# iebeid/ProtGram-DirectGCN

Hardware: AMD Instinct MI355X
Metric: edges/sec propagated, DirectGCN fwd on 4-gram graph, 1/2/4/8 MI355X (higher is better)
Workload: dtype f32; 1 GPU; directgcn_fwd_B(20,4); graph=complete n-gram de Bruijn B(20,4), num_nodes=160000, transitions=3200000, nnz_per_adjacency=6559580, feat_dim=128, layers=2, classes=20, propagation=precomputed-weights, entry=trainer COO (edge_index_*/edge_weight_* -> csr_from_coo), parallelism=single

## Files before the change

### include/pg_directgcn.h

```cpp
#ifndef PG_DIRECTGCN_H
#define PG_DIRECTGCN_H

#include <stdint.h>

#ifdef __cplusplus
extern "C" {
#endif

#define PG_ABI_VERSION 4

#define PG_OK 0
#define PG_ERR_ARG (-1)
#define PG_ERR_HIP (-2)
#define PG_ERR_UNSUPPORTED (-3)

typedef struct pg_edge3 {
    int32_t col;
    float w_in;
    float w_out;
    float w_und;
} pg_edge3_t;

typedef struct pg_edgeraw {
    int32_t col;
    float a_fwd;
    float a_bwd;
    float m_und;
} pg_edgeraw_t;

typedef struct pg_edge1 {
    int32_t col;
    float w;
} pg_edge1_t;


#define PG_FLAG_NO_XCD_REMAP (1u << 0)
#define PG_FLAG_EDGE_LDS (1u << 1)
#define PG_FLAG_UNROLL4 (1u << 2)
#define PG_FLAG_BCAST_RECORDS (1u << 7)
#define PG_FLAG_NGRAMT_WIDE (1u << 8)
#define PG_FLAG_NGRAMT_HALVES (1u << 4)
#define PG_FLAG_NGRAMT_NARROW (1u << 3)
#define PG_FLAG_DENSE_PREGATED (1u << 14)
#define PG_FLAG_DENSE_TILED (1u << 15)
#define PG_FLAG_DENSE_X3 (1u << 16)
#define PG_FLAG_WGRAD_BF16_TILED (1u << 11)
#define PG_FLAG_DGRAD_BF16_TILED (1u << 10)
#define PG_FLAG_DGRAD_BF16_RESIDENT (1u << 9)
#define PG_FLAG_WGRAD_F32MFMA (1u << 18)
#define PG_FLAG_DGRAD_F32MFMA (1u << 17)
#define PG_FLAG_NO_NGRAM (1u << 20)
#define PG_FLAG_NGRAM_BLOCK4 (1u << 21)
#define PG_FLAG_MID_NO_PAIRS (1u << 22)
#define PG_FLAG_MID_LOADER_SYNC (1u << 19)
#define PG_FLAG_DENSE_NO_IL (1u << 13)
#define PG_FLAG_DENSE_A_CACHED (1u << 12)
#define PG_FLAG_DENSE_LDS_EPILOGUE (1u << 29)
#define PG_FLAG_SCATTER_CPW_SHIFT 24
#define PG_FLAG_MID_TRANSPOSED (1u << 23)


const char* pg_last_error(void);
int pg_abi_version(void);

int pg_spmm3_f32(int64_t n_rows, const int64_t* rowptr, const int32_t* row_order, const pg_edge3_t* edges,
                 const float* X, int64_t ldx, int64_t F,
                 float* Z, int64_t ldz, uint32_t flags, void* stream);


int pg_spmm3_fusednorm_f32(int64_t n_rows, const int64_t* rowptr, const int32_t* row_order,
                           const pg_edgeraw_t* edges,
                           const float* node_norm, float eps,
                           const float* X, int64_t ldx, int64_t F,
                           float* Z, int64_t ldz, uint32_t flags, void* stream);

int pg_edges_normalize_f32(int64_t n_rows, const int64_t* rowptr, const pg_edgeraw_t* raw,
                           const float* node_norm, float eps, pg_edge3_t* out, void* stream);

int pg_spmm3t_f32(int64_t n_rows, const int64_t* rowptr, const int32_t* row_order, const pg_edge3_t* edges,
                  const float* G, int64_t ldg, int64_t F,
                  float* dX, int64_t lddx, int accumulate, uint32_t flags, void* stream);

int pg_spmm1_f32(int64_t n_rows, const int64_t* rowptr, const int32_t* row_order, const pg_edge1_t* edges,
                 const float* X, int64_t ldx, int64_t F,
                 float* Y, int64_t ldy, int accumulate, uint32_t flags, void* stream);

#define PG_GATES_VECTOR 0
#define PG_GATES_SCALAR 1

typedef struct pg_layer_args {
    int64_t M, F_in, F_out;
    const float* Z; int64_t ldz;
    const float* W_main_in; const float* W_main_out; const float* W_undirected; const float* W_shared;
    const float* b_main_in; const float* b_dir_shared_in;
    const float* b_main_out; const float* b_dir_shared_out;
    const float* b_undirected; const float* b_undirected_shared;
    int32_t gate_mode;
    const float* C_in; const float* C_out; const float* C_directed; const float* C_undirected; const float* C_all;
    const int64_t* rows;
    const float* constant; int64_t ld_const;
    const float* res_x; int64_t ld_res;
    const float* W_res; const float* b_res;
    int32_t act; float slope;
    float* Y; int64_t ldy;
    float drop_p; const int64_t* drop_seed;
} pg_layer_args_t;

int64_t pg_directgcn_packed_floats(int64_t F_in, int64_t F_out, int has_res_proj);

int pg_directgcn_pack_f32(const pg_layer_args_t* args, float* packed, void* stream);

int pg_directgcn_dense_f32(const pg_layer_args_t* args, const float* packed, uint32_t flags, void* stream);

int pg_directgcn_dense_ngram_rows_f32(const pg_layer_args_t* args, const float* packed, int64_t Kn1, int64_t m0,
                                      int32_t map_res, int32_t map_y, uint32_t flags, void* stream);

int pg_spmm3_gated_f32(int64_t n_rows, const int64_t* rowptr, const int32_t* row_order, const pg_edge3_t* edges,
                       const float* X, int64_t ldx, int64_t F, const pg_layer_args_t* gates,
                       float* Z, int64_t ldz, uint32_t flags, void* stream);

int64_t pg_ngram_plan_floats(int K, int n, int64_t n_rows);
int pg_ngram_plan_f32(int K, int n, int64_t n_rows, const int64_t* rowptr, const pg_edge3_t* edges, float* plan,
                      int64_t plan_floats, int* bad, void* stream);
int pg_spmm3_ngram_f32(int K, int n, int64_t n_rows, const float* plan, const float* X, int64_t ldx, int64_t F,
                       const pg_layer_args_t* gates, float* Z, int64_t ldz, uint32_t flags, void* stream);
int pg_spmm3t_ngram_f32(int K, int n, int64_t n_rows, const float* plan, const float* G, int64_t ldg, int64_t F,
                        float* dX, int64_t lddx, int accumulate, uint32_t flags, void* stream);
int pg_spmm3t_ngram_bf16(int K, int n, int64_t n_rows, const float* plan, const uint16_t* G, int64_t ldg, int64_t F,
                         uint16_t* dX, int64_t lddx, int accumulate, uint32_t flags, void* stream);
int pg_spmm3t_ngram_add_bf16(int K, int n, int64_t n_rows, const float* plan, const uint16_t* G, int64_t ldg,
                             int64_t F, const uint16_t* C, int64_t ldc, uint16_t* dX, int64_t lddx, uint32_t flags,
                             void* stream);

int64_t pg_ngram_mplan_floats(int K, int n, int64_t n_rows);
int pg_ngram_mplan_f32(int K, int n, int64_t n_rows, const int64_t* rowptr, const pg_edge3_t* edges, float* plan,
                       int64_t plan_floats, int* bad, void* stream);
int pg_spmm3_ngram_mid_f32(int K, int n, int64_t n_rows, const float* plan, const float* X, int64_t ldx, int64_t F,
                           const pg_layer_args_t* gates, float* Z, int64_t ldz, uint32_t flags, void* stream);
int pg_spmm3_ngram_mid_rows_f32(int K, int n, int64_t n_rows, const float* plan, const float* X, int64_t ldx, int64_t F,
                                int64_t m_begin, int64_t m_end, float* Z, int64_t ldz, uint32_t flags, void* stream);
int pg_spmm3_ngram_mid_bf16(int K, int n, int64_t n_rows, const float* plan, const uint16_t* X, int64_t ldx, int64_t F,
                            uint16_t* Z, int64_t ldz, uint32_t flags, void* stream);
int pg_spmm3_ngram_mid_rows_bf16(int K, int n, int64_t n_rows, const float* plan, const uint16_t* X, int64_t ldx,
                                 int64_t F, int64_t m_begin, int64_t m_end, uint16_t* Z, int64_t ldz, uint32_t flags,
                                 void* stream);
int pg_ngram_mplan_map_f32(int K, int n, int64_t n_nodes, const int64_t* rowptr, const pg_edge3_t* edges,
                           const int32_t* ginv, float* plan, int64_t plan_floats, uint8_t* resid, void* stream);
int pg_spmm3_ngram_mid_map_f32(int K, int n, const float* plan, const int32_t* gmap, const float* X, int64_t ldx,
                               int64_t F, float* Z, int64_t ldz, uint32_t flags, void* stream);
int pg_spmm3_resid_f32(int64_t n_list, const int64_t* rowptr, const int32_t* rows, const pg_edge3_t* edges,
                       const float* X, int64_t ldx, int64_t F, float* Z, int64_t ldz, uint32_t flags, void* stream);
int pg_spmm3t_ngram_mid_offdiag_f32(int K, int n, int64_t n_rows, const float* plan, const float* G, int64_t ldg,
                                    int64_t F, float* dX, int64_t lddx, int accumulate, uint32_t flags, void* stream);
int pg_spmm3t_ngram_mid_bf16(int K, int n, int64_t n_rows, const float* plan, const uint16_t* G, int64_t ldg, int64_t F,
                             uint16_t* dX, int64_t lddx, int accumulate, uint32_t flags, void* stream);

int pg_ngram_scatter_plan(int K, int n, const float* mplan, int64_t m0, int64_t n_mid, float* splan, void* stream);
int pg_spmm3t_ngram_scatter_f32(const float* splan, int64_t n_mid, const float* G, int64_t ldg, int64_t F, float* T,
                                int64_t ldt, uint32_t flags, void* stream);
int pg_spmm3t_ngram_scatter_bf16(const float* splan, int64_t n_mid, const uint16_t* G, int64_t ldg, int64_t F,
                                 float* T, int64_t ldt, uint32_t flags, void* stream);

int pg_rows_gather(const void* src, int64_t ld_src, const int64_t* idx, int64_t n, int64_t row_bytes, void* dst,
                   int64_t ld_dst, void* stream);
int pg_rows_scatter(const void* src, int64_t ld_src, const int64_t* idx, int64_t n, int64_t row_bytes, void* dst,
                    int64_t ld_dst, void* stream);
int pg_rows_gather_sum(const float* A, int64_t lda, const void* B, int64_t ldb, int b_bf16, const int64_t* rowptr,
                       const int32_t* idx, int64_t n_out, int64_t F, void* out, int64_t ldo, int out_bf16,
                       void* stream);

typedef struct pg_layer_grad_args {
    const float* dY; int64_t lddy;
    float* dpre; int64_t ldp;
    float* dZ; int64_t lddz;
    float* dres; int64_t lddres;
    float* dgate;
    float* gates;
    float* dW;
    float* work; int64_t work_floats;
    float* dpre_f32; int64_t ldp_f32;
} pg_layer_grad_args_t;

int64_t pg_directgcn_dense_bwd_workspace(const pg_layer_args_t* args);
int pg_directgcn_dense_bwd_f32(const pg_layer_args_t* args, const float* packed, const pg_layer_grad_args_t* grads,
                               uint32_t flags, void* stream);

int pg_directgcn_dense_bwd_span_f32(const pg_layer_args_t* args, const float* packed, const pg_layer_grad_args_t* grads,
                                    const float* wdiag, float* E, int64_t lde, int e_res, uint32_t flags, void* stream);


int pg_f32_to_bf16(int64_t n, const float* in, uint16_t* out, void* stream);

int pg_spmm3_bf16(int64_t n_rows, const int64_t* rowptr, const int32_t* row_order, const pg_edge3_t* edges,
                  const uint16_t* X, int64_t ldx, int64_t F, uint16_t* Z, int64_t ldz, uint32_t flags, void* stream);

int pg_spmm3t_bf16(int64_t n_rows, const int64_t* rowptr, const int32_t* row_order, const pg_edge3_t* edges,
                   const uint16_t* G, int64_t ldg, int64_t F, uint16_t* dX, int64_t lddx, uint32_t flags,
                   void* stream);

int pg_directgcn_dense_bf16(const pg_layer_args_t* args, const float* packed, const uint16_t* packed_bf16,
                            uint32_t flags, void* stream);

int pg_directgcn_dense_bwd_bf16(const pg_layer_args_t* args, const float* packed, const uint16_t* packed_bf16,
                                const pg_layer_grad_args_t* grads, uint32_t flags, void* stream);

int pg_directgcn_head_bf16(int64_t M, int64_t F, int64_t H, int64_t C, const uint16_t* h, int64_t ldh,
                           const float* W1, const float* b1, const float* W2, const float* b2, float eps,
                           float* logp, int64_t ldp, float* emb, int64_t lde, void* stream);

int pg_ngram_keys(int64_t nseq, const int64_t* offsets, const uint8_t* bytes, const int32_t* lut, int n,
                  int64_t K, int64_t* keys, int64_t* next_keys, void* stream);

int pg_ngram_letter_masks(int64_t n_nodes, const int64_t* node_keys, int n, int64_t K, const int32_t* code_bit,
                          uint32_t* masks, void* stream);

int pg_reach_hop_u32(int64_t n_rows, const int64_t* rowptr, const int64_t* col, const uint32_t* reach_in,
                     uint32_t* reach_out, int hop, int n_bits, uint8_t* dist, int64_t ldd, const uint8_t* target,
                     int64_t* labels, void* stream);

int pg_ngram_window_ids(int64_t nseq, const int64_t* offsets, const uint8_t* bytes, const int32_t* lut, int n,
                        int64_t K, const int64_t* node_keys, int64_t N, const int32_t* table, int32_t* ids,
                        void* stream);

int64_t pg_pool_distinct_max_nodes(void);
int pg_pool_rows_f32(const float* E, int64_t lde, int64_t N, int64_t F, const int64_t* rowptr, const int32_t* ids,
                     const int64_t* order, int64_t P, int distinct, float* out, int64_t ldo, int32_t* counts,
                     uint32_t flags, void* stream);

int64_t pg_pca_moments_workspace(int64_t P, int64_t F);
int pg_pca_moments_f64(const float* X, int64_t ldx, int64_t P, int64_t F, const int32_t* counts, const float* shift,
                       double* out, double* work, int64_t work_doubles, void* stream);

int pg_pca_project(const float* X, int64_t ldx, int64_t P, int64_t F, const int32_t* counts, const float* center,
                   const float* W, int64_t k, void* out, int64_t ldo, int out_dtype, void* stream);

typedef struct pg_tensor_desc {
    const float* x;
    float* y;
    int64_t numel;
} pg_tensor_desc_t;

int64_t pg_multi_chunks(int64_t numel);

int pg_multi_sqsum_f32(int ntens, const pg_tensor_desc_t* descs, const int64_t* chunk_ptr, int64_t nchunks,
                       float* partial, float* out, void* stream);

int pg_multi_axpy_f32(int ntens, const pg_tensor_desc_t* descs, const int64_t* chunk_ptr, int64_t nchunks,
                      float alpha, const float* alpha_scale, void* stream);

typedef struct pg_adam_desc {
    float* p;
    const void* g;
    float* m;
    float* v;
    int64_t numel;
    int64_t gtype;
} pg_adam_desc_t;

int pg_adam_f32(int ntens, const pg_adam_desc_t* descs, const int64_t* chunk_ptr, int64_t nchunks, double lr,
                double beta1, double beta2, double eps, double weight_decay, float* step, const float* grad_scale,
                const float* found_inf, float* sq_partial, const double* hyper, void* stream);

typedef struct pg_adam_rows_desc {
    float* p;
    const void* g;
    float* m;
    float* v;
    int64_t numel;
    int64_t gtype;
    const int32_t* pos;
    int64_t width;
} pg_adam_rows_desc_t;

int pg_adam_rows_f32(int ntens, const pg_adam_rows_desc_t* descs, const int64_t* chunk_ptr, int64_t nchunks, double lr,
                     double beta1, double beta2, double eps, double weight_decay, float* step, const float* grad_scale,
                     const float* found_inf, float* sq_partial, const double* hyper, void* stream);
int pg_multi_sum_f32(int64_t n, const float* x, float* out, void* stream);

int64_t pg_head_train_workspace(int64_t M, int64_t F, int64_t H, int64_t C);
int pg_head_train_f32(int64_t M, int64_t F, int64_t H, int64_t C, const float* h, int64_t ldh, const float* W1,
                      const float* b1, const float* W2, const float* b2, const int64_t* y, float loss_weight,
                      float drop_p, const int64_t* seed, const float* grad_scale, float* dh, int64_t lddh,
                      float* grads, float* loss, float* work, int64_t work_floats, void* stream);

int64_t pg_head_train_bf16_workspace(int64_t M, int64_t F, int64_t H, int64_t C);
int pg_head_train_bf16(int64_t M, int64_t F, int64_t H, int64_t C, const uint16_t* h, int64_t ldh, const float* W1,
                       const float* b1, const float* W2, const float* b2, const int64_t* y, float loss_weight,
                       float drop_p, const int64_t* seed, const float* grad_scale, uint16_t* dh, int64_t lddh,
                       float* grads, float* loss, float* work, int64_t work_floats, void* stream);

int64_t pg_gemm_at_b_workspace(int64_t M, int64_t P, int64_t N);
int pg_gemm_at_b_f32(int64_t M, int64_t P, int64_t N, const float* A, int64_t lda, const float* B, int64_t ldb,
                     float* out, float* work, int64_t work_floats, void* stream);

int pg_dense_grads_layout_f32(int64_t F_out, int64_t F_in, int32_t S, const float* dB, const float* dbsum, float* out,
                              void* stream);

int pg_directgcn_head_f32(int64_t M, int64_t F, int64_t H, int64_t C, const float* h, int64_t ldh,
                          const float* W1, const float* b1, const float* W2, const float* b2, float eps,
                          float* logp, int64_t ldp, float* emb, int64_t lde, void* stream);

#ifdef __cplusplus
}
#endif

#endif
```

### protgram-directgcn_amd/_lib.py

```python
from __future__ import annotations

import ctypes
import os

_HERE = os.path.dirname(os.path.abspath(__file__))
_LIB_PATH = os.environ.get("PG_DIRECTGCN_LIB", os.path.join(_HERE, "libpgdgcn.so"))

PG_OK = 0
PG_FLAG_NO_XCD_REMAP = 1 << 0
PG_FLAG_EDGE_LDS = 1 << 1
PG_FLAG_UNROLL4 = 1 << 2
PG_FLAG_BCAST_RECORDS = 1 << 7
PG_FLAG_NGRAMT_WIDE = 1 << 8
PG_FLAG_NGRAMT_NARROW = 1 << 3
PG_FLAG_NGRAMT_HALVES = 1 << 4
PG_FLAG_DENSE_PREGATED = 1 << 14
PG_FLAG_DENSE_TILED = 1 << 15
PG_FLAG_DENSE_X3 = 1 << 16
PG_FLAG_WGRAD_F32MFMA = 1 << 18
PG_FLAG_WGRAD_BF16_TILED = 1 << 11
PG_FLAG_DGRAD_BF16_TILED = 1 << 10
PG_FLAG_DGRAD_BF16_RESIDENT = 1 << 9
PG_FLAG_DGRAD_F32MFMA = 1 << 17
PG_FLAG_NO_NGRAM = 1 << 20
PG_FLAG_NGRAM_BLOCK4 = 1 << 21
PG_FLAG_MID_NO_PAIRS = 1 << 22
PG_FLAG_MID_LOADER_SYNC = 1 << 19
PG_FLAG_MID_TRANSPOSED = 1 << 23
PG_FLAG_SCATTER_CPW_SHIFT = 24
PG_FLAG_DENSE_A_CACHED = 1 << 12
PG_FLAG_DENSE_NO_IL = 1 << 13
PG_FLAG_DENSE_LDS_EPILOGUE = 1 << 29

c_i64, c_i32, c_u32, c_f32, c_vp = ctypes.c_int64, ctypes.c_int32, ctypes.c_uint32, ctypes.c_float, ctypes.c_void_p


PG_OK, PG_ERR_ARG, PG_ERR_HIP, PG_ERR_UNSUPPORTED = 0, -1, -2, -3


class NativeLibraryError(RuntimeError):
    pass


class LayerArgs(ctypes.Structure):
    _fields_ = [("M", c_i64), ("F_in", c_i64), ("F_out", c_i64),
                ("Z", c_vp), ("ldz", c_i64),
                ("W_main_in", c_vp), ("W_main_out", c_vp), ("W_undirected", c_vp), ("W_shared", c_vp),
                ("b_main_in", c_vp), ("b_dir_shared_in", c_vp),
                ("b_main_out", c_vp), ("b_dir_shared_out", c_vp),
                ("b_undirected", c_vp), ("b_undirected_shared", c_vp),
                ("gate_mode", c_i32),
                ("C_in", c_vp), ("C_out", c_vp), ("C_directed", c_vp), ("C_undirected", c_vp), ("C_all", c_vp),
                ("rows", c_vp),
                ("constant", c_vp), ("ld_const", c_i64),
                ("res_x", c_vp), ("ld_res", c_i64),
                ("W_res", c_vp), ("b_res", c_vp),
                ("act", c_i32), ("slope", c_f32),
                ("Y", c_vp), ("ldy", c_i64),
                ("drop_p", c_f32), ("drop_seed", c_vp)]


class LayerGradArgs(ctypes.Structure):
    _fields_ = [("dY", c_vp), ("lddy", c_i64), ("dpre", c_vp), ("ldp", c_i64), ("dZ", c_vp), ("lddz", c_i64),
                ("dres", c_vp), ("lddres", c_i64), ("dgate", c_vp), ("gates", c_vp), ("dW", c_vp),
                ("work", c_vp), ("work_floats", c_i64), ("dpre_f32", c_vp), ("ldp_f32", c_i64)]


SIGNATURES = {
    "pg_last_error": (ctypes.c_char_p, []),
    "pg_abi_version": (ctypes.c_int, []),
    "pg_spmm3_f32": (ctypes.c_int, [c_i64, c_vp, c_vp, c_vp, c_vp, c_i64, c_i64, c_vp, c_i64, c_u32, c_vp]),
    "pg_spmm3_gated_f32": (ctypes.c_int, [c_i64, c_vp, c_vp, c_vp, c_vp, c_i64, c_i64, ctypes.POINTER(LayerArgs), c_vp,
                                          c_i64, c_u32, c_vp]),
    "pg_spmm3_fusednorm_f32": (ctypes.c_int, [c_i64, c_vp, c_vp, c_vp, c_vp, c_f32, c_vp, c_i64, c_i64, c_vp, c_i64,
                                              c_u32, c_vp]),
    "pg_edges_normalize_f32": (ctypes.c_int, [c_i64, c_vp, c_vp, c_vp, c_f32, c_vp, c_vp]),
    "pg_ngram_plan_floats": (c_i64, [ctypes.c_int, ctypes.c_int, c_i64]),
    "pg_ngram_plan_f32": (ctypes.c_int, [ctypes.c_int, ctypes.c_int, c_i64, c_vp, c_vp, c_vp, c_i64, c_vp, c_vp]),
    "pg_spmm3_ngram_f32": (ctypes.c_int, [ctypes.c_int, ctypes.c_int, c_i64, c_vp, c_vp, c_i64, c_i64,
                                          ctypes.POINTER(LayerArgs), c_vp, c_i64, c_u32, c_vp]),
    "pg_ngram_mplan_floats": (c_i64, [ctypes.c_int, ctypes.c_int, c_i64]),
    "pg_ngram_mplan_f32": (ctypes.c_int, [ctypes.c_int, ctypes.c_int, c_i64, c_vp, c_vp, c_vp, c_i64, c_vp, c_vp]),
    "pg_spmm3_ngram_mid_f32": (ctypes.c_int, [ctypes.c_int, ctypes.c_int, c_i64, c_vp, c_vp, c_i64, c_i64,
                                              ctypes.POINTER(LayerArgs), c_vp, c_i64, c_u32, c_vp]),
    "pg_spmm3_ngram_mid_rows_f32": (ctypes.c_int, [ctypes.c_int, ctypes.c_int, c_i64, c_vp, c_vp, c_i64, c_i64, c_i64,
                                                   c_i64, c_vp, c_i64, c_u32, c_vp]),
    "pg_spmm3_ngram_mid_bf16": (ctypes.c_int, [ctypes.c_int, ctypes.c_int, c_i64, c_vp, c_vp, c_i64, c_i64, c_vp,
                                               c_i64, c_u32, c_vp]),
    "pg_spmm3_ngram_mid_rows_bf16": (ctypes.c_int, [ctypes.c_int, ctypes.c_int, c_i64, c_vp, c_vp, c_i64, c_i64, c_i64,
                                                    c_i64, c_vp, c_i64, c_u32, c_vp]),
    "pg_ngram_mplan_map_f32": (ctypes.c_int, [ctypes.c_int, ctypes.c_int, c_i64, c_vp, c_vp, c_vp, c_vp, c_i64, c_vp,
                                              c_vp]),
    "pg_spmm3_ngram_mid_map_f32": (ctypes.c_int, [ctypes.c_int, ctypes.c_int, c_vp, c_vp, c_vp, c_i64, c_i64, c_vp,
                                                  c_i64, c_u32, c_vp]),
    "pg_spmm3_resid_f32": (ctypes.c_int, [c_i64, c_vp, c_vp, c_vp, c_vp, c_i64, c_i64, c_vp, c_i64, c_u32, c_vp]),
    "pg_rows_gather": (ctypes.c_int, [c_vp, c_i64, c_vp, c_i64, c_i64, c_vp, c_i64, c_vp]),
    "pg_rows_scatter": (ctypes.c_int, [c_vp, c_i64, c_vp, c_i64, c_i64, c_vp, c_i64, c_vp]),
    "pg_rows_gather_sum": (ctypes.c_int, [c_vp, c_i64, c_vp, c_i64, ctypes.c_int, c_vp, c_vp, c_i64, c_i64, c_vp,
                                          c_i64, ctypes.c_int, c_vp]),
    "pg_ngram_scatter_plan": (ctypes.c_int, [ctypes.c_int, ctypes.c_int, c_vp, c_i64, c_i64, c_vp, c_vp]),
    "pg_spmm3t_ngram_scatter_f32": (ctypes.c_int, [c_vp, c_i64, c_vp, c_i64, c_i64, c_vp, c_i64, c_u32, c_vp]),
    "pg_spmm3t_ngram_scatter_bf16": (ctypes.c_int, [c_vp, c_i64, c_vp, c_i64, c_i64, c_vp, c_i64, c_u32, c_vp]),
    "pg_spmm3t_ngram_f32": (ctypes.c_int, [ctypes.c_int, ctypes.c_int, c_i64, c_vp, c_vp, c_i64, c_i64, c_vp, c_i64,
                                           ctypes.c_int, c_u32, c_vp]),
    "pg_spmm3t_ngram_mid_offdiag_f32": (ctypes.c_int, [ctypes.c_int, ctypes.c_int, c_i64, c_vp, c_vp, c_i64, c_i64,
                                                       c_vp, c_i64, ctypes.c_int, c_u32, c_vp]),
    "pg_spmm3t_ngram_mid_bf16": (ctypes.c_int, [ctypes.c_int, ctypes.c_int, c_i64, c_vp, c_vp, c_i64, c_i64, c_vp, c_i64,
                                                ctypes.c_int, c_u32, c_vp]),
    "pg_spmm3t_ngram_bf16": (ctypes.c_int, [ctypes.c_int, ctypes.c_int, c_i64, c_vp, c_vp, c_i64, c_i64, c_vp, c_i64,
                                            ctypes.c_int, c_u32, c_vp]),
    "pg_spmm3t_ngram_add_bf16": (ctypes.c_int, [ctypes.c_int, ctypes.c_int, c_i64, c_vp, c_vp, c_i64, c_i64, c_vp,
                                                c_i64, c_vp, c_i64, c_u32, c_vp]),
    "pg_spmm3t_f32": (ctypes.c_int, [c_i64, c_vp, c_vp, c_vp, c_vp, c_i64, c_i64, c_vp, c_i64, ctypes.c_int, c_u32,
                                     c_vp]),
    "pg_spmm1_f32": (ctypes.c_int, [c_i64, c_vp, c_vp, c_vp, c_vp, c_i64, c_i64, c_vp, c_i64, ctypes.c_int, c_u32,
                                    c_vp]),
    "pg_directgcn_packed_floats": (c_i64, [c_i64, c_i64, ctypes.c_int]),
    "pg_directgcn_pack_f32": (ctypes.c_int, [ctypes.POINTER(LayerArgs), c_vp, c_vp]),
    "pg_directgcn_dense_f32": (ctypes.c_int, [ctypes.POINTER(LayerArgs), c_vp, c_u32, c_vp]),
    "pg_directgcn_dense_ngram_rows_f32": (ctypes.c_int, [ctypes.POINTER(LayerArgs), c_vp, c_i64, c_i64, c_i32, c_i32,
                                                         c_u32, c_vp]),
    "pg_directgcn_dense_bwd_workspace": (c_i64, [ctypes.POINTER(LayerArgs)]),
    "pg_directgcn_dense_bwd_f32": (ctypes.c_int, [ctypes.POINTER(LayerArgs), c_vp, ctypes.POINTER(LayerGradArgs),
                                                  c_u32, c_vp]),
    "pg_directgcn_dense_bwd_span_f32": (ctypes.c_int, [ctypes.POINTER(LayerArgs), c_vp, ctypes.POINTER(LayerGradArgs),
                                                       c_vp, c_vp, c_i64, c_i32, c_u32, c_vp]),
    "pg_f32_to_bf16": (ctypes.c_int, [c_i64, c_vp, c_vp, c_vp]),
    "pg_spmm3_bf16": (ctypes.c_int, [c_i64, c_vp, c_vp, c_vp, c_vp, c_i64, c_i64, c_vp, c_i64, c_u32, c_vp]),
    "pg_spmm3t_bf16": (ctypes.c_int, [c_i64, c_vp, c_vp, c_vp, c_vp, c_i64, c_i64, c_vp, c_i64, c_u32, c_vp]),
    "pg_directgcn_dense_bf16": (ctypes.c_int, [ctypes.POINTER(LayerArgs), c_vp, c_vp, c_u32, c_vp]),
    "pg_directgcn_dense_bwd_bf16": (ctypes.c_int, [ctypes.POINTER(LayerArgs), c_vp, c_vp, ctypes.POINTER(LayerGradArgs),
                                                   c_u32, c_vp]),
    "pg_directgcn_head_bf16": (ctypes.c_int, [c_i64, c_i64, c_i64, c_i64, c_vp, c_i64, c_vp, c_vp, c_vp, c_vp, c_f32,
                                              c_vp, c_i64, c_vp, c_i64, c_vp]),
    "pg_ngram_keys": (ctypes.c_int, [c_i64, c_vp, c_vp, c_vp, ctypes.c_int, c_i64, c_vp, c_vp, c_vp]),
    "pg_ngram_window_ids": (ctypes.c_int, [c_i64, c_vp, c_vp, c_vp, ctypes.c_int, c_i64, c_vp, c_i64, c_vp, c_vp, c_vp]),
    "pg_ngram_letter_masks": (ctypes.c_int, [c_i64, c_vp, ctypes.c_int, c_i64, c_vp, c_vp, c_vp]),
    "pg_reach_hop_u32": (ctypes.c_int, [c_i64, c_vp, c_vp, c_vp, c_vp, ctypes.c_int, ctypes.c_int, c_vp, c_i64, c_vp,
                                        c_vp, c_vp]),
    "pg_pool_distinct_max_nodes": (c_i64, []),
    "pg_pool_rows_f32": (ctypes.c_int, [c_vp, c_i64, c_i64, c_i64, c_vp, c_vp, c_vp, c_i64, ctypes.c_int, c_vp, c_i64,
                                        c_vp, c_u32, c_vp]),
    "pg_pca_moments_workspace": (c_i64, [c_i64, c_i64]),
    "pg_pca_moments_f64": (ctypes.c_int, [c_vp, c_i64, c_i64, c_i64, c_vp, c_vp, c_vp, c_vp, c_i64, c_vp]),
    "pg_pca_project": (ctypes.c_int, [c_vp, c_i64, c_i64, c_i64, c_vp, c_vp, c_vp, c_i64, c_vp, c_i64, ctypes.c_int,
                                      c_vp]),
    "pg_multi_chunks": (c_i64, [c_i64]),
    "pg_multi_sqsum_f32": (ctypes.c_int, [ctypes.c_int, c_vp, c_vp, c_i64, c_vp, c_vp, c_vp]),
    "pg_multi_axpy_f32": (ctypes.c_int, [ctypes.c_int, c_vp, c_vp, c_i64, c_f32, c_vp, c_vp]),
    "pg_adam_f32": (ctypes.c_int, [ctypes.c_int, c_vp, c_vp, c_i64, ctypes.c_double, ctypes.c_double, ctypes.c_double,
                                   ctypes.c_double, ctypes.c_double, c_vp, c_vp, c_vp, c_vp, c_vp, c_vp]),
    "pg_adam_rows_f32": (ctypes.c_int, [ctypes.c_int, c_vp, c_vp, c_i64, ctypes.c_double, ctypes.c_double,
                                        ctypes.c_double, ctypes.c_double, ctypes.c_double, c_vp, c_vp, c_vp, c_vp, c_vp,
                                        c_vp]),
    "pg_multi_sum_f32": (ctypes.c_int, [c_i64, c_vp, c_vp, c_vp]),
    "pg_dense_grads_layout_f32": (ctypes.c_int, [c_i64, c_i64, ctypes.c_int32, c_vp, c_vp, c_vp, c_vp]),
    "pg_gemm_at_b_workspace": (c_i64, [c_i64, c_i64, c_i64]),
    "pg_gemm_at_b_f32": (ctypes.c_int, [c_i64, c_i64, c_i64, c_vp, c_i64, c_vp, c_i64, c_vp, c_vp, c_i64, c_vp]),
    "pg_directgcn_head_f32": (ctypes.c_int, [c_i64, c_i64, c_i64, c_i64, c_vp, c_i64, c_vp, c_vp, c_vp, c_vp, c_f32,
                                             c_vp, c_i64, c_vp, c_i64, c_vp]),
    "pg_head_train_workspace": (c_i64, [c_i64, c_i64, c_i64, c_i64]),
    "pg_head_train_f32": (ctypes.c_int, [c_i64, c_i64, c_i64, c_i64, c_vp, c_i64, c_vp, c_vp, c_vp, c_vp, c_vp, c_f32,
                                         c_f32, c_vp, c_vp, c_vp, c_i64, c_vp, c_vp, c_vp, c_i64, c_vp]),
    "pg_head_train_bf16_workspace": (c_i64, [c_i64, c_i64, c_i64, c_i64]),
    "pg_head_train_bf16": (ctypes.c_int, [c_i64, c_i64, c_i64, c_i64, c_vp, c_i64, c_vp, c_vp, c_vp, c_vp, c_vp, c_f32,
                                          c_f32, c_vp, c_vp, c_vp, c_i64, c_vp, c_vp, c_vp, c_i64, c_vp]),
}

_lib = None


def library_path() -> str:
    return _LIB_PATH


def load_library():
    global _lib
    if _lib is not None:
        return _lib
    if not os.path.exists(_LIB_PATH):
        raise NativeLibraryError(
            f"HIP library not found at {_LIB_PATH}; build it with `python -c 'import __graft_entry__ as g; g.build()'`"
            " (there is no CPU fallback)")
    try:
        lib = ctypes.CDLL(_LIB_PATH)
    except OSError as e:
        raise NativeLibraryError(f"failed to load {_LIB_PATH}: {e}") from e
    for name, (res, args) in SIGNATURES.items():
        fn = getattr(lib, name, None)
        if fn is None:
            raise NativeLibraryError(f"{_LIB_PATH} does not export {name}")
        fn.restype, fn.argtypes = res, args
    if lib.pg_abi_version() != 4:
        raise NativeLibraryError("ABI version mismatch")
    _lib = lib
    return lib


def check(rc: int, what: str):
    if rc != PG_OK:
        msg = load_library().pg_last_error().decode(errors="replace")
        raise RuntimeError(f"{what} failed ({rc}): {msg}")


def default_flags() -> int:
    v = os.environ.get("PG_SPMM_FLAGS")
    return int(v, 0) if v else 0
```

### protgram-directgcn_amd/csrc/pg_common.h

```cpp
#pragma once

#include <hip/hip_runtime.h>

#include <cstdarg>
#include <cstdint>
#include <cstdio>

#include "pg_directgcn.h"

namespace pg {

int set_error(int code, const char* fmt, ...);
void clear_error();

__device__ __forceinline__ float4 ld4(const float* p) { return *reinterpret_cast<const float4*>(p); }
__device__ __forceinline__ float fb(int v) { return __int_as_float(v); }

__device__ __forceinline__ int64_t xcd_logical_block(int64_t b, int64_t nb, bool remap) {
    if (!remap || nb < 16) return b;
    const int64_t q = nb >> 3, r = nb & 7;
    const int64_t x = b & 7, i = b >> 3;
    return x * q + (x < r ? x : r) + i;
}

__device__ __forceinline__ float sqrt_rn(float x) {
    if (!(x > 0.0f) || x == __builtin_inff()) return __builtin_sqrtf(x);
    const bool tiny = x < 0x1p-96f;
    const float xs = tiny ? x * 0x1p64f : x;
    float y = __builtin_sqrtf(xs);
    const int yi = __float_as_int(y);
    const float ym = __int_as_float(yi - 1), yp = __int_as_float(yi + 1);
    const float vm = __builtin_fmaf(-ym, y, xs), vp = __builtin_fmaf(-yp, y, xs);
    y = vm <= 0.0f ? ym : y;
    y = vp > 0.0f ? yp : y;
    return tiny ? y * 0x1p-32f : y;
}

__device__ __forceinline__ uint32_t drop_hash(uint64_t seed, uint32_t e) {
    uint32_t x = (e * 0x9E3779B1u + (uint32_t)seed) ^ (uint32_t)(seed >> 32);
    x ^= x >> 16;
    x *= 0x85EBCA6Bu;
    x ^= x >> 13;
    x *= 0xC2B2AE35u;
    x ^= x >> 16;
    return x;
}

__device__ __forceinline__ float act_grad(float d, float y, float slope, float ds) {
    if (ds == 0.f) return y > 0.f ? d : d * slope;
    const float e = d * ds;
    return y > 0.f ? e : (y < 0.f ? e * slope : 0.f);
}

inline int drop_params(const pg_layer_args_t* a, uint32_t& thr, float& scale, bool need_seed = true) {
    thr = 0;
    scale = 0.f;
    if (a->drop_p == 0.f) return PG_OK;
    if (!(a->drop_p > 0.f && a->drop_p < 1.f) || !a->act || (need_seed && !a->drop_seed))
        return set_error(PG_ERR_ARG, "fused dropout needs 0 <= drop_p < 1, act and drop_seed (drop_p = %g)",
                         (double)a->drop_p);
    thr = (uint32_t)((double)a->drop_p * 16777216.0 + 0.5);
    scale = (float)(1.0 / (1.0 - (double)a->drop_p));
    return PG_OK;
}

inline int check_launch(const char* what) {
    hipError_t e = hipGetLastError();
    if (e != hipSuccess) return set_error(PG_ERR_HIP, "%s: %s", what, hipGetErrorString(e));
    return PG_OK;
}

inline int cu_count() {
    int dev = 0, ncu = 256;
    if (hipGetDevice(&dev) != hipSuccess ||
        hipDeviceGetAttribute(&ncu, hipDeviceAttributeMultiprocessorCount, dev) != hipSuccess || ncu <= 0)
        ncu = 256;
    return ncu;
}

inline bool aligned16(const void* p) { return (reinterpret_cast<uintptr_t>(p) & 15u) == 0; }

}

#define PG_REQUIRE(cond, ...)                                         \
    do {                                                              \
        if (!(cond)) return ::pg::set_error(PG_ERR_ARG, __VA_ARGS__); \
    } while (0)
```

### protgram-directgcn_amd/csrc/pg_dense.hip

```cpp
#include "pg_common.h"
#include "pg_lds.h"
#include "pg_split3.h"

namespace {

typedef float f32x16 __attribute__((ext_vector_type(16)));
typedef float f32x4 __attribute__((ext_vector_type(4)));

constexpr int BK = 32;
constexpr int LDSW = 36;

struct DenseP {
    int64_t M;
    int F_in, F_out, K;
    const float* Z;
    int64_t ldz;
    const float* Bp;
    const float* bsum;
    int gate_mode;
    const float *C_in, *C_out, *C_dir, *C_und, *C_all;
    const int64_t* rows;
    const float* constant;
    int64_t ld_const;
    const float* res_x;
    int64_t ld_res;
    int proj_res;
    int vec_out;
    int act;
    float slope;
    float* Y;
    int64_t ldy;
    int remap;
    int pregated;
    int rawW;
    const float *Wq0, *Wq1, *Wq2, *Wsh;
    const float *bm0, *bs0, *bm1, *bs1, *bm2, *bs2;
    int64_t map_kn1, map_m0;
    int map_res, map_y;
    int nt_a;
    int exp;
    uint32_t drop_thr;
    float drop_s;
    const int64_t* drop_seed;
};

__device__ __forceinline__ float drop_apply(const DenseP& p, uint64_t seed, int64_t m, int j, float y) {
    const uint32_t e = (uint32_t)(m * p.F_out + j);
    return (pg::drop_hash(seed, e) >> 8) >= p.drop_thr ? y * p.drop_s : 0.f;
}
__device__ __forceinline__ uint64_t drop_seed_of(const DenseP& p) {
    return p.drop_s != 0.f ? (uint64_t)*p.drop_seed : 0ull;
}

#ifdef PG_DENSE_EXP
#define DEXP(bit) ((p.exp >> (bit)) & 1)
constexpr int DST_BLOCKS = 64, DST_IT = 48, DST_PT = 8;
__device__ unsigned long long* g_dense_stamps = nullptr;
#define DSTAMP_INIT unsigned long long* const dst_base_ = g_dense_stamps
#define DSTAMP(it, pt)                                                                                             \
    do {                                                                                                           \
        if (dst_base_ && lane == 0 && (wave == 0 || wave == 4) && blockIdx.x < DST_BLOCKS && (it) < DST_IT)        \
            dst_base_[((blockIdx.x * 2 + (wave >> 2)) * DST_IT + (it)) * DST_PT + (pt)] =                          \
                __builtin_amdgcn_s_memtime();                                                                      \
    } while (0)
#else
#define DEXP(bit) 0
#define DSTAMP_INIT \
    do {            \
    } while (0)
#define DSTAMP(it, pt) \
    do {               \
    } while (0)
#endif

__device__ __forceinline__ int64_t ngram_row(const DenseP& p, int64_t m) {
    const int r = (int)m;
    const int q = r / 400, w = r - 400 * q;
    const int a = w / 20, b = w - 20 * a;
    return (int64_t)a * p.map_kn1 + (p.map_m0 + q) * 20 + b;
}

using pg::ld4;
__device__ __forceinline__ float4 scale4(float4 a, float s) { return make_float4(a.x * s, a.y * s, a.z * s, a.w * s); }

__device__ __forceinline__ int seg_of(int k, int F) { return (k >= F) + (k >= 2 * F) + (k >= 3 * F); }

__device__ __forceinline__ float a_elem(const DenseP& p, const float* sg, int64_t m, int k) {
    const int q = seg_of(k, p.F_in);
    if (q < 3) return p.pregated ? p.Z[m * p.ldz + k] : p.Z[m * p.ldz + k] * sg[q];
    return p.res_x[m * p.ld_res + (k - 3 * p.F_in)];
}

template <int BM, int BN, int NW, bool VEC>
__global__ __launch_bounds__(64 * NW) void dense_kernel(DenseP p) {
    constexpr int NT = 64 * NW;
    const uint64_t dseed = drop_seed_of(p);
    constexpr int WN = (BM == 64 && NW == 8) ? 4 : (BN == 128 || BM == 64 || NW == 8) ? 2 : 1;
    constexpr int WM = NW / WN;
    static_assert(BM / WM >= 32 && BN / WN >= 32, "wave tile too small");
    constexpr int TM = BM / WM / 32;
    constexpr int TN = BN / WN / 32;
    constexpr int A_F4 = BM * BK / 4 / NT;
    constexpr int B_F4 = BN * BK / 4 / NT;

    constexpr int TLD = BN + 4;
    constexpr int MAIN_FLOATS = 2 * BM * LDSW + 2 * BN * LDSW;
    constexpr int SMEM_FLOATS = MAIN_FLOATS > BM * TLD ? MAIN_FLOATS : BM * TLD;
    __shared__ __attribute__((aligned(16))) float smem[SMEM_FLOATS];
    __shared__ __attribute__((aligned(16))) float Sg[BM * 4];
    __shared__ int64_t Crow[BM];
    static_assert(BM <= NT, "gate prologue assumes one thread per tile row");
    float (*As)[BM * LDSW] = reinterpret_cast<float (*)[BM * LDSW]>(smem);
    float (*Bs)[BN * LDSW] = reinterpret_cast<float (*)[BN * LDSW]>(smem + 2 * BM * LDSW);

    const int64_t n_mblk = (p.M + BM - 1) / BM;
    const int64_t lb = pg::xcd_logical_block(blockIdx.x, gridDim.x, p.remap != 0);
    const int64_t m0 = (lb % n_mblk) * BM;
    const int n0 = (int)(lb / n_mblk) * BN;
    const int tid = threadIdx.x;
    const int wave = tid >> 6, lane = tid & 63;
    const int wm = wave / WN, wn = wave % WN;
    const int li = lane & 31, lh = lane >> 5;

    if (tid < BM) {
        const int64_t m = m0 + tid;
        float s0 = 0.f, s1 = 0.f, s2 = 0.f;
        if (m < p.M) {
            const int64_t r = (p.gate_mode == PG_GATES_SCALAR) ? 0 : (p.rows ? p.rows[m] : m);
            const float ci = p.C_in[r], co = p.C_out[r], cd = p.C_dir[r], cu = p.C_und[r], ca = p.C_all[r];
            const float cad = ca * cd;
            s0 = cad * ci;
            s1 = cad * co;
            s2 = ca * cu;
        }
        Sg[tid * 4 + 0] = s0;
        Sg[tid * 4 + 1] = s1;
        Sg[tid * 4 + 2] = s2;
        Sg[tid * 4 + 3] = 1.f;
        Crow[tid] = m < p.M ? (p.rows ? p.rows[m] : m) : -1;
    }
    __syncthreads();

    f32x16 acc[TM][TN];
#pragma unroll
    for (int i = 0; i < TM; ++i)
#pragma unroll
        for (int j = 0; j < TN; ++j)
#pragma unroll
            for (int r = 0; r < 16; ++r) acc[i][j][r] = 0.f;

    float4 ra[A_F4], rb[B_F4];
    const int64_t mlast = p.M - 1;
    auto fetch_to = [&](int k0, float4 (&ra)[A_F4], float4 (&rb)[B_F4]) {
#pragma unroll
        for (int q = 0; q < A_F4; ++q) {
            const int idx = tid + NT * q;
            const int64_t m = min(m0 + (idx >> 3), mlast);
            const int k = k0 + 4 * (idx & 7);
            if (VEC) {
                const int kc = k < p.K ? k : 0;
                const int seg = seg_of(kc, p.F_in);
                const float* src = seg < 3 ? p.Z + m * p.ldz + kc : p.res_x + m * p.ld_res + (kc - 3 * p.F_in);
                ra[q] = ld4(src);
            } else {
                const float* sg = &Sg[(idx >> 3) * 4];
                float4 v = make_float4(0.f, 0.f, 0.f, 0.f);
                if (k + 0 < p.K) v.x = a_elem(p, sg, m, k + 0);
                if (k + 1 < p.K) v.y = a_elem(p, sg, m, k + 1);
                if (k + 2 < p.K) v.z = a_elem(p, sg, m, k + 2);
                if (k + 3 < p.K) v.w = a_elem(p, sg, m, k + 3);
                ra[q] = v;
            }
        }
#pragma unroll
        for (int q = 0; q < B_F4; ++q) {
            const int idx = tid + NT * q;
            const int n = min(n0 + (idx >> 3), p.F_out - 1);
            const int k = k0 + 4 * (idx & 7);
            const float* src = p.Bp + (int64_t)n * p.K;
            if (VEC) {
                rb[q] = ld4(src + (k < p.K ? k : 0));
            } else {
                float4 v = make_float4(0.f, 0.f, 0.f, 0.f);
                if (k + 0 < p.K) v.x = src[k + 0];
                if (k + 1 < p.K) v.y = src[k + 1];
                if (k + 2 < p.K) v.z = src[k + 2];
                if (k + 3 < p.K) v.w = src[k + 3];
                rb[q] = v;
            }
        }
    };
    auto fetch = [&](int k0) { fetch_to(k0, ra, rb); };
    auto stash_from = [&](int buf, int k0, const float4 (&ra)[A_F4], const float4 (&rb)[B_F4]) {
#pragma unroll
        for (int q = 0; q < A_F4; ++q) {
            const int idx = tid + NT * q;
            float4 v = ra[q];
            if (VEC) {
                const int k = k0 + 4 * (idx & 7);
                const int seg = seg_of(k, p.F_in);
                const float sc = k < p.K ? (p.pregated ? 1.f : Sg[(idx >> 3) * 4 + seg]) : 0.f;
                v = scale4(v, sc);
            }
            *reinterpret_cast<float4*>(&As[buf][(idx >> 3) * LDSW + 4 * (idx & 7)]) = v;
        }
#pragma unroll
        for (int q = 0; q < B_F4; ++q) {
            const int idx = tid + NT * q;
            float4 v = rb[q];
            if (VEC) {
                const int k = k0 + 4 * (idx & 7);
                if (k >= p.K) v = make_float4(0.f, 0.f, 0.f, 0.f);
            }
            *reinterpret_cast<float4*>(&Bs[buf][(idx >> 3) * LDSW + 4 * (idx & 7)]) = v;
        }
    };

    auto stash = [&](int buf, int k0) { stash_from(buf, k0, ra, rb); };
    auto mma = [&](int cur) {
        const float* Ab = As[cur];
        const float* Bb = Bs[cur];
#pragma unroll
        for (int g = 0; g < BK / 8; ++g) {
            float4 a[TM], b[TN];
#pragma unroll
            for (int i = 0; i < TM; ++i) a[i] = ld4(&Ab[(wm * TM * 32 + i * 32 + li) * LDSW + g * 8 + 4 * lh]);
#pragma unroll
            for (int j = 0; j < TN; ++j) b[j] = ld4(&Bb[(wn * TN * 32 + j * 32 + li) * LDSW + g * 8 + 4 * lh]);
#pragma unroll
            for (int i = 0; i < TM; ++i)
#pragma unroll
                for (int j = 0; j < TN; ++j) {
                    acc[i][j] = __builtin_amdgcn_mfma_f32_32x32x2f32(a[i].x, b[j].x, acc[i][j], 0, 0, 0);
                    acc[i][j] = __builtin_amdgcn_mfma_f32_32x32x2f32(a[i].y, b[j].y, acc[i][j], 0, 0, 0);
                    acc[i][j] = __builtin_amdgcn_mfma_f32_32x32x2f32(a[i].z, b[j].z, acc[i][j], 0, 0, 0);
                    acc[i][j] = __builtin_amdgcn_mfma_f32_32x32x2f32(a[i].w, b[j].w, acc[i][j], 0, 0, 0);
                }
        }
    };

    const int ntiles = (p.K + BK - 1) / BK;
    fetch(0);
    stash(0, 0);
    __syncthreads();
    for (int t = 0; t < ntiles; ++t) {
        const int cur = t & 1;
        if (t + 1 < ntiles) fetch((t + 1) * BK);
        mma(cur);
        if (t + 1 < ntiles) stash(cur ^ 1, (t + 1) * BK);
        __syncthreads();
    }

    float* T = smem;
#pragma unroll
    for (int i = 0; i < TM; ++i)
#pragma unroll
        for (int j = 0; j < TN; ++j)
#pragma unroll
            for (int r = 0; r < 16; ++r) {
                const int rl = wm * TM * 32 + i * 32 + (r & 3) + 8 * (r >> 2) + 4 * lh;
                T[rl * TLD + wn * TN * 32 + j * 32 + li] = acc[i][j][r];
            }
    __syncthreads();

    constexpr int C4 = BN / 4;
    constexpr int ITER = BM * C4 / NT;
    constexpr int BATCH = ITER < 4 ? ITER : 4;
    const int c4 = tid % C4;
    const int nb = n0 + 4 * c4;
    const bool has_const = p.constant && p.gate_mode == PG_GATES_VECTOR;
    const bool id_res = p.res_x && !p.proj_res;
    const bool vec_out = p.vec_out;
    float4 b[3], br = make_float4(0.f, 0.f, 0.f, 0.f);
    {
        auto ldb = [&](const float* v) {
            float4 o;
            o.x = nb + 0 < p.F_out ? v[nb + 0] : 0.f;
            o.y = nb + 1 < p.F_out ? v[nb + 1] : 0.f;
            o.z = nb + 2 < p.F_out ? v[nb + 2] : 0.f;
            o.w = nb + 3 < p.F_out ? v[nb + 3] : 0.f;
            return o;
        };
        b[0] = ldb(p.bsum);
        b[1] = ldb(p.bsum + p.F_out);
        b[2] = ldb(p.bsum + 2 * p.F_out);
        if (p.proj_res) br = ldb(p.bsum + 3 * p.F_out);
    }
    for (int it0 = 0; it0 < ITER; it0 += BATCH) {
        float4 cv[BATCH], rv[BATCH];
        int rl[BATCH];
        int64_t mm[BATCH];
        bool ok[BATCH];
#pragma unroll
        for (int u = 0; u < BATCH; ++u) {
            rl[u] = (tid + NT * (it0 + u)) / C4;
            mm[u] = m0 + rl[u];
            ok[u] = Crow[rl[u]] >= 0 && nb < p.F_out;
            cv[u] = make_float4(0.f, 0.f, 0.f, 0.f);
            rv[u] = make_float4(0.f, 0.f, 0.f, 0.f);
            if (ok[u] && vec_out) {
                if (has_const) cv[u] = ld4(p.constant + Crow[rl[u]] * p.ld_const + nb);
                if (id_res) rv[u] = ld4(p.res_x + mm[u] * p.ld_res + nb);
            }
        }
#pragma unroll
        for (int u = 0; u < BATCH; ++u) {
            if (!ok[u]) continue;
            const float* sg = &Sg[rl[u] * 4];
            float4 v = ld4(&T[rl[u] * TLD + 4 * c4]);
            float o[4] = {v.x, v.y, v.z, v.w};
            const float bb0[4] = {b[0].x, b[0].y, b[0].z, b[0].w};
            const float bb1[4] = {b[1].x, b[1].y, b[1].z, b[1].w};
            const float bb2[4] = {b[2].x, b[2].y, b[2].z, b[2].w};
            const float bbr[4] = {br.x, br.y, br.z, br.w};
            float cc[4] = {cv[u].x, cv[u].y, cv[u].z, cv[u].w};
            float rr[4] = {rv[u].x, rv[u].y, rv[u].z, rv[u].w};
            if (!vec_out) {
#pragma unroll
                for (int e = 0; e < 4; ++e) {
                    const int n = nb + e;
                    if (n < p.F_out) {
                        if (has_const) cc[e] = p.constant[Crow[rl[u]] * p.ld_const + n];
                        if (id_res) rr[e] = p.res_x[mm[u] * p.ld_res + n];
                    }
                }
            }
#pragma unroll
            for (int e = 0; e < 4; ++e) {
                float y = o[e] + (sg[0] * bb0[e] + sg[1] * bb1[e] + sg[2] * bb2[e]) + bbr[e] + cc[e] + rr[e];
                if (p.act) y = y > 0.f ? y : y * p.slope;
                if (p.drop_s != 0.f) y = drop_apply(p, dseed, mm[u], nb + e, y);
                o[e] = y;
            }
            if (vec_out) {
                *reinterpret_cast<float4*>(p.Y + mm[u] * p.ldy + nb) = make_float4(o[0], o[1], o[2], o[3]);
            } else {
#pragma unroll
                for (int e = 0; e < 4; ++e)
                    if (nb + e < p.F_out) p.Y[mm[u] * p.ldy + nb + e] = o[e];
            }
        }
    }
}

using pg::glds16;
using pg::glds16nt;
// ... 28 lines not shown
__device__ __forceinline__ void lds_st16(void* p, uint4 v) {
    const u32x4_t w = {v.x, v.y, v.z, v.w};
    asm volatile("ds_write_b128 %0, %1" ::"v"(lds_addr(p)), "v"(w) : "memory");
}
__device__ __forceinline__ void lds_ld4x4(const float* p0, const float* p1, const float* p2, const float* p3,
                                          float4 (&o)[4]) {
    f32x4 x0, x1, x2, x3;
    asm volatile(
        "ds_read_b128 %0, %4\n\tds_read_b128 %1, %5\n\tds_read_b128 %2, %6\n\tds_read_b128 %3, %7\n\t"
        "s_waitcnt lgkmcnt(0)"
        : "=&v"(x0), "=&v"(x1), "=&v"(x2), "=&v"(x3)
        : "v"(lds_addr(p0)), "v"(lds_addr(p1)), "v"(lds_addr(p2)), "v"(lds_addr(p3))
        : "memory");
    o[0] = make_float4(x0[0], x0[1], x0[2], x0[3]);
    o[1] = make_float4(x1[0], x1[1], x1[2], x1[3]);
    o[2] = make_float4(x2[0], x2[1], x2[2], x2[3]);
    o[3] = make_float4(x3[0], x3[1], x3[2], x3[3]);
}
template <int STRIDE_BYTES>
__device__ __forceinline__ void lds_epi(const float* p0, const float* p1, const float* p2, const float* g, float4& a,
                                        float4& b, float4& c, float (&gv)[5]) {
    f32x4 x0, x1, x2;
    asm volatile(
        "ds_read_b128 %0, %8\n\tds_read_b128 %1, %9\n\tds_read_b128 %2, %10\n\t"
        "ds_read_b32 %3, %11\n\tds_read_b32 %4, %11 offset:%c12\n\tds_read_b32 %5, %11 offset:%c13\n\t"
        "ds_read_b32 %6, %11 offset:%c14\n\tds_read_b32 %7, %11 offset:%c15\n\ts_waitcnt lgkmcnt(0)"
        : "=&v"(x0), "=&v"(x1), "=&v"(x2), "=&v"(gv[0]), "=&v"(gv[1]), "=&v"(gv[2]), "=&v"(gv[3]), "=&v"(gv[4])
        : "v"(lds_addr(p0)), "v"(lds_addr(p1)), "v"(lds_addr(p2)), "v"(lds_addr(g)), "n"(STRIDE_BYTES),
          "n"(2 * STRIDE_BYTES), "n"(3 * STRIDE_BYTES), "n"(4 * STRIDE_BYTES)
        : "memory");
    a = make_float4(x0[0], x0[1], x0[2], x0[3]);
    b = make_float4(x1[0], x1[1], x1[2], x1[3]);
    c = make_float4(x2[0], x2[1], x2[2], x2[3]);
}
template <int STRIDE_BYTES>
__device__ __forceinline__ void lds_gates5(const float* p, float (&g)[5]) {
    asm volatile(
        "ds_read_b32 %0, %5\n\tds_read_b32 %1, %5 offset:%c6\n\tds_read_b32 %2, %5 offset:%c7\n\t"
        "ds_read_b32 %3, %5 offset:%c8\n\tds_read_b32 %4, %5 offset:%c9\n\ts_waitcnt lgkmcnt(0)"
        : "=&v"(g[0]), "=&v"(g[1]), "=&v"(g[2]), "=&v"(g[3]), "=&v"(g[4])
        : "v"(lds_addr(p)), "n"(STRIDE_BYTES), "n"(2 * STRIDE_BYTES), "n"(3 * STRIDE_BYTES), "n"(4 * STRIDE_BYTES)
        : "memory");
}

__device__ __forceinline__ int a_unit(int s, int r, int g) { return 128 * s + 4 * r + (g ^ ((-(r >> 2)) & 3)); }

struct TileRange { int64_t ntl, lo, step; };
__device__ __forceinline__ TileRange tile_range(int64_t T) {
    const int nb = gridDim.x, b = blockIdx.x;
    TileRange t;
    if ((nb & 7) == 0 && nb >= 8) {
        const int x = b & 7, i = b >> 3, bpx = nb >> 3;
        const int64_t xlo = T * x / 8, xhi = T * (x + 1) / 8;
        t.ntl = (xhi - xlo - i + bpx - 1) / bpx;
        t.lo = xlo + i;
        t.step = bpx;
    } else {
        t.ntl = (T - b + nb - 1) / nb;
        t.lo = b;
        t.step = nb;
    }
    if (t.ntl < 0) t.ntl = 0;
    return t;
}

template <int NS>
__device__ __forceinline__ void w_splits(const float* src, uint4 (&w0)[NS], uint4 (&w1)[NS], uint4 (&w2)[NS]) {
#pragma unroll
    for (int s = 0; s < NS; ++s) {
        const float4 x0 = ld4(src + 32 * s), x1 = ld4(src + 32 * s + 16);
        const float v[8] = {x0.x, x0.y, x0.z, x0.w, x1.x, x1.y, x1.z, x1.w};
        split8(v, w0[s], w1[s], w2[s]);
    }
}

__device__ __forceinline__ void gate_scales(const float (&c)[5], float& s0, float& s1, float& s2) {
    const float cad = c[4] * c[2];
    s0 = cad * c[0];
    s1 = cad * c[1];
    s2 = c[4] * c[3];
}

__device__ __forceinline__ void gate_ptrs(const DenseP& p, const float* (&c)[5]) {
    c[0] = p.C_in, c[1] = p.C_out, c[2] = p.C_dir, c[3] = p.C_und, c[4] = p.C_all;
    asm volatile("" : "+s"(c[0]), "+s"(c[1]), "+s"(c[2]), "+s"(c[3]), "+s"(c[4]));
}

template <bool MAP, int BM>
__device__ __forceinline__ void cr_rows(const DenseP& p, bool has_const, bool id_res, int64_t tile, int r,
                                        const float*& cb, const float*& rb) {
    const int64_t m0 = tile * BM;
    const int rmax = (int)min((int64_t)(BM - 1), p.M - 1 - m0);
    const int rr = min(r, rmax);
    cb = has_const ? p.constant + m0 * p.ld_const + (rr * (int)p.ld_const) : p.Z + m0 * p.ldz;
    rb = !id_res            ? p.Z + m0 * p.ldz
         : MAP && p.map_res ? p.res_x + ngram_row(p, m0 + rr) * p.ld_res
                            : p.res_x + m0 * p.ld_res + (rr * (int)p.ld_res);
}

template <int F_IN, int KSEG, bool PRE>
__global__ __launch_bounds__(512) void dense_x3_kernel(DenseP p) {
    constexpr int K = F_IN * KSEG;
    const uint64_t dseed = drop_seed_of(p);
    constexpr int CH = K / 4;
    constexpr int NU = K / 8;
    constexpr int NS = K / 32;
    constexpr int BMW = 32;
    constexpr int NI = BMW * CH / 64 / 8;
    constexpr int NG = 3;
    constexpr int NCR = 4;
    (void)NCR;
    constexpr int NCV = (BMW * NU + 511) / 512;
    static_assert(CH % 16 == 0 && NU % 16 == 0 && (BMW * CH) % 512 == 0 && BMW * 128 / 4 == 1024, "tile shape");
    __shared__ __attribute__((aligned(16))) float Af[BMW * K];
    __shared__ __attribute__((aligned(16))) uint4 As[3][BMW * NU];
    __shared__ __attribute__((aligned(16))) float Cs[BMW * 128];
    __shared__ __attribute__((aligned(16))) float Rs[BMW * 128];
    __shared__ __attribute__((aligned(16))) float Gi[2][8][BMW];
    __shared__ __attribute__((aligned(16))) float Bs[4][128];
    constexpr int ELD = 128 + 4;
    static_assert(BMW * ELD * 4 <= 3 * BMW * NU * 16, "epilogue tile must fit in the split images");
    float* Es = reinterpret_cast<float*>(&As[0][0]);

    const int tid = threadIdx.x;
    const int wave = tid >> 6, lane = tid & 63;
    const int lc = lane & 15, kg = lane >> 4;
    const int col = 16 * wave + lc;
    const int64_t T = (p.M + BMW - 1) / BMW;
    Bs[tid >> 7][tid & 127] = (tid >> 7) < 3 || p.proj_res ? p.bsum[(tid >> 7) * p.F_out + (tid & 127)] : 0.f;
    const TileRange tr = tile_range(T);
    const int64_t ntl = tr.ntl, lo = tr.lo, step = tr.step;
    uint4 w0[NS], w1[NS], w2[NS];
    w_splits<NS>(p.Bp + (int64_t)col * K + 4 * kg, w0, w1, w2);
    const int ej = tid & 31, er = tid >> 5;
    const bool has_const = p.constant && p.gate_mode == PG_GATES_VECTOR;
    const bool id_res = p.res_x && !p.proj_res;

    auto issue_A = [&](int64_t tile, float* Ad) {
        const int64_t m0 = tile * BMW;
        const int rmax = (int)min((int64_t)(BMW - 1), p.M - 1 - m0);
        const float* zb = p.Z + m0 * p.ldz;
        const float* xb = KSEG > 3 ? p.res_x + m0 * p.ld_res : zb;
        const int ln = opaque(lane);
#pragma unroll
        for (int i = 0; i < NI; ++i) {
            const int idx = (wave * NI + i) * 64 + ln;
            const int r = idx / CH, pos = idx - r * CH;
            const int k = 4 * (pos ^ (r & 15));
            const int rr = min(r, rmax);
            const float* src = (KSEG == 3 || k < 3 * F_IN) ? zb + (rr * (int)p.ldz + k)
                                                          : xb + (rr * (int)p.ld_res + (k - 3 * F_IN));
            glds16(src, Ad + (wave * NI + i) * 256);
        }
    };
    auto issue_G = [&](int64_t tile, int gbuf) {
        const int ln = opaque(lane);
        const int64_t r = p.gate_mode == PG_GATES_SCALAR ? 0 : min(tile * BMW + (ln & 31), p.M - 1);
        const float* c[5];
        gate_ptrs(p, c);
        const bool hi = ln >= 32;
        glds4((hi ? c[1] : c[0]) + r, &Gi[gbuf][0][0]);
        glds4((hi ? c[3] : c[2]) + r, &Gi[gbuf][2][0]);
        glds4(c[4] + r, &Gi[gbuf][4][0]);
    };
    auto issue_CR = [&](int64_t tile) {
        const int ln = opaque(lane);
#pragma unroll
        for (int i = 0; i < 2; ++i) {
            const int piece = 2 * wave + i;
            const float *cb, *rb;
            cr_rows<false, BMW>(p, has_const, id_res, tile, 2 * piece + (ln >> 5), cb, rb);
            glds16(cb + 4 * (ln & 31), Cs + piece * 256);
            glds16(rb + 4 * (ln & 31), Rs + piece * 256);
        }
    };
    auto gates = [&](int gbuf, int r, float& s0, float& s1, float& s2) {
        float c[5];
        lds_gates5<BMW * 4>(&Gi[gbuf][0][r], c);
        gate_scales(c, s0, s1, s2);
    };
    auto tile_of = [&](int64_t kt) { return lo + min(kt, ntl - 1) * step; };

    auto convert = [&](const float* Af, int gb) {
#pragma unroll
        for (int i = 0; i < NCV; ++i) {
            const int j = tid + 512 * i;
            if (BMW * NU % 512 != 0 && j >= BMW * NU) break;
            const int r = j & (BMW - 1), u = j / BMW;
            const int s = u >> 2, g = u & 3;
            const int c0 = 8 * s + g;
            float4 x0, x1;
            lds_ld4x2(&Af[r * K + 4 * (c0 ^ (r & 15))], &Af[r * K + 4 * ((c0 + 4) ^ (r & 15))], x0, x1);
            float v[8] = {x0.x, x0.y, x0.z, x0.w, x1.x, x1.y, x1.z, x1.w};
            if (!PRE) {
                const int q = (32 * s) / F_IN;
                if (q < 3) {
                    float sg[3];
                    gates(gb, r, sg[0], sg[1], sg[2]);
                    const float sc = sg[q];
#pragma unroll
                    for (int e = 0; e < 8; ++e) v[e] = __fmul_rn(v[e], sc);
                }
            }
            uint4 s0, s1, s2;
            split8(v, s0, s1, s2);
            const int pos = a_unit(s, r, g);
            lds_st16(&As[0][pos], s0);
            lds_st16(&As[1][pos], s1);
            lds_st16(&As[2][pos], s2);
            __builtin_amdgcn_sched_barrier(0);
        }
    };
    constexpr int WAIT_W0 = NG + NI, WAIT_WN = NI;
    if (ntl > 0) {
        if (wave == 0) issue_G(tile_of(0), 0);
        issue_A(tile_of(0), Af);
    }
    bool prev_full = false;
    for (int64_t kt = 0; kt < ntl; ++kt) {
        const int buf = (int)(kt & 1);
        const int64_t m0 = (lo + kt * step) * BMW;
        if (prev_full) asm volatile("s_waitcnt vmcnt(2)" ::: "memory");
        else asm volatile("s_waitcnt vmcnt(0)" ::: "memory");
        lds_barrier();
        issue_CR(tile_of(kt));
        if (wave == 0) issue_G(tile_of(kt + 1), buf ^ 1);
        convert(Af, buf);
        lds_barrier();
        issue_A(tile_of(kt + 1), Af);
        f32x4 acc[2] = {f32x4{0.f, 0.f, 0.f, 0.f}, f32x4{0.f, 0.f, 0.f, 0.f}};
        const uint4* ab0 = &As[0][a_unit(0, lc, kg)];
        const uint4* ab2 = &As[2][a_unit(0, lc, kg)];
        uint4 op[2][6];
        auto ld_ops = [&](int s, uint4 (&o)[6]) {
            o[0] = ab0[128 * s];
            o[1] = ab0[BMW * NU + 128 * s];
            o[2] = ab2[128 * s];
            o[3] = ab0[64 + 128 * s];
            o[4] = ab0[BMW * NU + 64 + 128 * s];
            o[5] = ab2[64 + 128 * s];
        };
        ld_ops(0, op[0]);
#pragma unroll
        for (int s = 0; s < NS; ++s) {
            if (s + 1 < NS) ld_ops(s + 1, op[(s + 1) & 1]);
            const uint4 a00 = op[s & 1][0], a01 = op[s & 1][1], a02 = op[s & 1][2];
            const uint4 a10 = op[s & 1][3], a11 = op[s & 1][4], a12 = op[s & 1][5];
            acc[0] = mfma_bf(a02, w0[s], acc[0]);
            acc[1] = mfma_bf(a12, w0[s], acc[1]);
            acc[0] = mfma_bf(a01, w1[s], acc[0]);
            acc[1] = mfma_bf(a11, w1[s], acc[1]);
            acc[0] = mfma_bf(a00, w2[s], acc[0]);
            acc[1] = mfma_bf(a10, w2[s], acc[1]);
            acc[0] = mfma_bf(a01, w0[s], acc[0]);
            acc[1] = mfma_bf(a11, w0[s], acc[1]);
            acc[0] = mfma_bf(a00, w1[s], acc[0]);
            acc[1] = mfma_bf(a10, w1[s], acc[1]);
            acc[0] = mfma_bf(a00, w0[s], acc[0]);
            acc[1] = mfma_bf(a10, w0[s], acc[1]);
            __builtin_amdgcn_sched_barrier(0);
        }
        lds_barrier();
#pragma unroll
        for (int sb = 0; sb < 2; ++sb)
#pragma unroll
            for (int i = 0; i < 4; ++i) lds_stf(&Es[(16 * sb + 4 * kg + i) * ELD + col], acc[sb][i]);
        if (wave == 0) asm volatile("s_waitcnt vmcnt(%0)" ::"n"(WAIT_W0) : "memory");
        else asm volatile("s_waitcnt vmcnt(%0)" ::"n"(WAIT_WN) : "memory");
        lds_barrier();
#pragma unroll
        for (int h = 0; h < 2; ++h) {
            const int rl = er + 16 * h;
            if (m0 + rl >= p.M) continue;
            float4 v, cv, rv, bb[4];
            lds_ld4x2(&Cs[rl * 128 + 4 * ej], &Rs[rl * 128 + 4 * ej], cv, rv);
            lds_ld4x4(&Es[rl * ELD + 4 * ej], &Bs[0][4 * ej], &Bs[1][4 * ej], &Bs[2][4 * ej], bb);
            v = bb[0];
            const float4 b0 = bb[1], b1 = bb[2], b2 = bb[3];
            float4 br;
            lds_ld4x2(&Bs[3][4 * ej], &Bs[3][4 * ej], br, br);
            if (!has_const) cv = make_float4(0.f, 0.f, 0.f, 0.f);
            if (!id_res) rv = make_float4(0.f, 0.f, 0.f, 0.f);
            float s0, s1, s2;
            gates(buf, rl, s0, s1, s2);
            const float o[4] = {v.x, v.y, v.z, v.w}, C4[4] = {cv.x, cv.y, cv.z, cv.w}, R4[4] = {rv.x, rv.y, rv.z, rv.w};
            const float B0[4] = {b0.x, b0.y, b0.z, b0.w}, B1[4] = {b1.x, b1.y, b1.z, b1.w},
                        B2[4] = {b2.x, b2.y, b2.z, b2.w}, BR[4] = {br.x, br.y, br.z, br.w};
            float y[4];
#pragma unroll
            for (int e = 0; e < 4; ++e) {
                const float qv = epi_sum(o[e], s0, s1, s2, B0[e], B1[e], B2[e], BR[e], C4[e], R4[e]);
                y[e] = (p.act && !(qv > 0.f)) ? qv * p.slope : qv;
                if (p.drop_s != 0.f) y[e] = drop_apply(p, dseed, m0 + rl, 4 * ej + e, y[e]);
            }
            *reinterpret_cast<float4*>(p.Y + (m0 + rl) * p.ldy + 4 * ej) = make_float4(y[0], y[1], y[2], y[3]);
        }
        prev_full = m0 + BMW <= p.M;
    }
    asm volatile("s_waitcnt vmcnt(0)" ::: "memory");
}

__device__ __forceinline__ int a_unit16(int s, int r, int g) { return 64 * s + 4 * r + (g ^ ((-(r >> 2)) & 3)); }

template <bool PRE, bool IL, bool DROP, bool LDSE>
__global__ __launch_bounds__(512) void dense_x3p_kernel(DenseP p) {
    constexpr int F_IN = 128, K = 384;
    constexpr int CH = K / 4;
    constexpr int NU = K / 8;
    constexpr int NS = K / 32;
    constexpr int BM = 16;
    constexpr int NI = BM * CH / 64 / 8;
    constexpr int NG = 2;
    constexpr int NCR = 2;
    (void)NCR;
    [[maybe_unused]] constexpr int ELD = 128 + 4;
    static_assert(BM * CH % 512 == 0 && NI == 3, "tile shape");
    __shared__ __attribute__((aligned(16))) float Af0[BM * K];
    __shared__ __attribute__((aligned(16))) float Af1[BM * K];
    __shared__ __attribute__((aligned(16))) uint4 As[2][3][BM * NU];
    __shared__ __attribute__((aligned(16))) float Cs[LDSE ? BM * 128 : 4];
    __shared__ __attribute__((aligned(16))) float Rs[LDSE ? BM * 128 : 4];
    __shared__ __attribute__((aligned(16))) float Es[LDSE ? BM * ELD : 4];
    __shared__ __attribute__((aligned(16))) float Gi[4][8][BM];
    __shared__ __attribute__((aligned(16))) float Bs[4][128];

    const int tid = threadIdx.x;
    const int wave = tid >> 6, lane = tid & 63;
    const int lc = lane & 15, kg = lane >> 4;
    const int col = 16 * wave + lc;
    const bool mfma_first = wave < 4;
    const uint64_t dseed = DROP ? drop_seed_of(p) : 0ull;
    const int64_t T = (p.M + BM - 1) / BM;
    DSTAMP_INIT;
    {
        const int q = tid >> 7, n = tid & 127;
        float bv = 0.f;
        if (p.rawW) {
            if (q < 3) bv = q == 0 ? p.bm0[n] + p.bs0[n] : q == 1 ? p.bm1[n] + p.bs1[n] : p.bm2[n] + p.bs2[n];
        } else if (q < 3 || p.proj_res) {
            bv = p.bsum[q * p.F_out + n];
        }
        Bs[q][n] = bv;
    }
    const TileRange tr = tile_range(T);
    const int64_t ntl = tr.ntl, lo = tr.lo, step = tr.step;

    uint4 w0[NS], w1[NS], w2[NS];
    if (p.rawW) {
#pragma unroll
        for (int s = 0; s < NS; ++s) {
            const float* wq = s < 4 ? p.Wq0 : s < 8 ? p.Wq1 : p.Wq2;
            const int64_t o = (int64_t)col * F_IN + (32 * s) % F_IN + 4 * kg;
            const float4 a0 = ld4(wq + o), a1 = ld4(wq + o + 16), h0 = ld4(p.Wsh + o), h1 = ld4(p.Wsh + o + 16);
            const float v[8] = {a0.x + h0.x, a0.y + h0.y, a0.z + h0.z, a0.w + h0.w,
                                a1.x + h1.x, a1.y + h1.y, a1.z + h1.z, a1.w + h1.w};
            split8(v, w0[s], w1[s], w2[s]);
        }
    } else {
        w_splits<NS>(p.Bp + (int64_t)col * K + 4 * kg, w0, w1, w2);
    }
    const int ec = LDSE ? 4 * (tid & 31) : 16 * wave + 4 * kg, er = LDSE ? tid >> 5 : lc;
    const bool has_const = p.constant && p.gate_mode == PG_GATES_VECTOR;
    const bool id_res = p.res_x && !p.proj_res;
    auto tile_of = [&](int64_t kt) { return lo + max((int64_t)0, min(kt, ntl - 1)) * step; };

    auto issue_A_piece = [&](int64_t tile, float* Ad, int i) {
        if (DEXP(3)) return;
        const int64_t m0 = tile * BM;
        const int rmax = (int)min((int64_t)(BM - 1), p.M - 1 - m0);
        const float* zb = p.Z + m0 * p.ldz;
        const int ln = opaque(lane);
        const int idx = (wave * NI + i) * 64 + ln;
        const int r = idx / CH, pos = idx - r * CH;
        const int k = 4 * (pos ^ r);
        const int rr = min(r, rmax);
        if (p.nt_a) glds16nt(zb + (rr * (int)p.ldz + k), Ad + (wave * NI + i) * 256);
        else glds16(zb + (rr * (int)p.ldz + k), Ad + (wave * NI + i) * 256);
    };
    auto issue_A = [&](int64_t tile, float* Ad) {
#pragma unroll
        for (int i = 0; i < NI; ++i) issue_A_piece(tile, Ad, i);
    };
    auto issue_G = [&](int64_t tile, int slot) {
        const int ln = opaque(lane);
        const int64_t r = p.gate_mode == PG_GATES_SCALAR ? 0 : min(tile * BM + (ln & 15), p.M - 1);
        const float* c[5];
        gate_ptrs(p, c);
        const int q = ln >> 4;
        const float* cq = q == 0 ? c[0] : q == 1 ? c[1] : q == 2 ? c[2] : c[3];
        glds4(cq + r, &Gi[slot][0][0]);
        glds4(c[4] + r, &Gi[slot][4][0]);
    };
    [[maybe_unused]] f32x4 cv = {0.f, 0.f, 0.f, 0.f}, rv = cv;
    [[maybe_unused]] auto load_CR = [&](int64_t tile) {
        if (DEXP(4)) return;
        const float *cb, *rb;
        cr_rows<true, BM>(p, has_const, id_res, tile, er, cb, rb);
        if (p.nt_a)
            asm volatile("global_load_dwordx4 %0, %2, off nt\n\tglobal_load_dwordx4 %1, %3, off"
                         : "=&v"(cv), "=&v"(rv)
                         : "v"(cb + ec), "v"(rb + ec)
                         : "memory");
        else
            asm volatile("global_load_dwordx4 %0, %2, off\n\tglobal_load_dwordx4 %1, %3, off"
                         : "=&v"(cv), "=&v"(rv)
                         : "v"(cb + ec), "v"(rb + ec)
                         : "memory");
    };
    [[maybe_unused]] auto wait_CR = [&]() {
        if (wave == 0) asm volatile("s_waitcnt vmcnt(%2)" : "+v"(cv), "+v"(rv) : "n"(NI + NG) : "memory");
        else asm volatile("s_waitcnt vmcnt(%2)" : "+v"(cv), "+v"(rv) : "n"(NI) : "memory");
    };
    [[maybe_unused]] auto issue_CR = [&](int64_t tile) {
        if (DEXP(4)) return;
        const int ln = opaque(lane);
        const float *cb, *rb;
        cr_rows<true, BM>(p, has_const, id_res, tile, 2 * wave + (ln >> 5), cb, rb);
        if (p.nt_a) glds16nt(cb + 4 * (ln & 31), Cs + wave * 256);
        else glds16(cb + 4 * (ln & 31), Cs + wave * 256);
        glds16(rb + 4 * (ln & 31), Rs + wave * 256);
    };
    auto split_tile = [&](const float* Af, int ab, int gslot) {
        if (DEXP(1)) return;
        const int r = tid & 15;
        const bool two = tid + 512 < BM * NU;
        const int u0 = tid >> 4, u1 = u0 + 32;
        const int c00 = 8 * (u0 >> 2) + (u0 & 3), c10 = 8 * (u1 >> 2) + (u1 & 3);
        float4 x[4];
        if (two) lds_ld4x4(&Af[r * K + 4 * (c00 ^ r)], &Af[r * K + 4 * ((c00 + 4) ^ r)], &Af[r * K + 4 * (c10 ^ r)],
                           &Af[r * K + 4 * ((c10 + 4) ^ r)], x);
        else lds_ld4x2(&Af[r * K + 4 * (c00 ^ r)], &Af[r * K + 4 * ((c00 + 4) ^ r)], x[0], x[1]);
        float sg[3] = {1.f, 1.f, 1.f}, gc[5];
        if (!PRE) {
            lds_gates5<BM * 4>(&Gi[gslot][0][r], gc);
            gate_scales(gc, sg[0], sg[1], sg[2]);
        }
#pragma unroll
        for (int i = 0; i < 2; ++i) {
            if (i == 1 && !two) break;
            const int u = i ? u1 : u0;
            const int s = u >> 2, g = u & 3;
            const float4 a = x[2 * i], c = x[2 * i + 1];
            float v[8] = {a.x, a.y, a.z, a.w, c.x, c.y, c.z, c.w};
            if (!PRE) {
                const float sc = sg[(32 * s) / F_IN];
#pragma unroll
                for (int e = 0; e < 8; ++e) v[e] = __fmul_rn(v[e], sc);
            }
            uint4 s0, s1, s2;
            split8(v, s0, s1, s2);
            const int pos = a_unit16(s, r, g);
            lds_st16(&As[ab][0][pos], s0);
            lds_st16(&As[ab][1][pos], s1);
            lds_st16(&As[ab][2][pos], s2);
        }
    };
    f32x4 acc = {0.f, 0.f, 0.f, 0.f};
    auto mfma_tile = [&](int ab, int64_t a_tile, float* a_dst, int g_slot, bool issue) {
        const uint4* a0 = &As[ab][0][a_unit16(0, lc, kg)];
        const uint4* a1 = &As[ab][1][a_unit16(0, lc, kg)];
        const uint4* a2 = &As[ab][2][a_unit16(0, lc, kg)];
        uint4 op[2][3];
        acc = f32x4{0.f, 0.f, 0.f, 0.f};
        if (DEXP(0)) {
            if (IL && issue) {
                issue_A(a_tile, a_dst);
                if (wave == 0) issue_G(a_tile, g_slot);
            }
            return;
        }
        op[0][0] = a0[0];
        op[0][1] = a1[0];
        op[0][2] = a2[0];
#pragma unroll
        for (int s = 0; s < NS; ++s) {
            if (s + 1 < NS) {
                op[(s + 1) & 1][0] = a0[64 * (s + 1)];
                op[(s + 1) & 1][1] = a1[64 * (s + 1)];
                op[(s + 1) & 1][2] = a2[64 * (s + 1)];
            }
            const uint4 x0 = op[s & 1][0], x1 = op[s & 1][1], x2 = op[s & 1][2];
            if constexpr (LDSE) {
                acc = mfma_bf(x2, w0[s], acc);
                acc = mfma_bf(x1, w1[s], acc);
                acc = mfma_bf(x0, w2[s], acc);
                acc = mfma_bf(x1, w0[s], acc);
                acc = mfma_bf(x0, w1[s], acc);
                acc = mfma_bf(x0, w0[s], acc);
            } else {
                acc = mfma_bf(w0[s], x2, acc);
                acc = mfma_bf(w1[s], x1, acc);
                acc = mfma_bf(w2[s], x0, acc);
                acc = mfma_bf(w0[s], x1, acc);
                acc = mfma_bf(w1[s], x0, acc);
                acc = mfma_bf(w0[s], x0, acc);
            }
            if constexpr (IL) {
                if (issue && (s == 2 || s == 5 || s == 8)) issue_A_piece(a_tile, a_dst, s / 3);
                if (issue && s == 10 && wave == 0) issue_G(a_tile, g_slot);
            }
            __builtin_amdgcn_sched_barrier(0);
        }
    };

    if (ntl > 0) {
        issue_A(tile_of(0), Af0);
        if (wave == 0) issue_G(tile_of(0), 0);
        issue_A(tile_of(1), Af1);
        if (wave == 0) issue_G(tile_of(1), 1);
        if (wave == 0) asm volatile("s_waitcnt vmcnt(%0)" ::"n"(NI + NG) : "memory");
        else asm volatile("s_waitcnt vmcnt(%0)" ::"n"(NI) : "memory");
        lds_barrier();
        split_tile(Af0, 0, 0);
    }
    float4 bq[4];
    if (ntl > 0) lds_ld4x4(&Bs[0][ec], &Bs[1][ec], &Bs[2][ec], &Bs[3][ec], bq);
    auto epilogue = [&](int64_t m0, float4 ov, float4 cq, float4 rq, const float (&c)[5]) {
        if (!has_const) cq = make_float4(0.f, 0.f, 0.f, 0.f);
        if (!id_res) rq = make_float4(0.f, 0.f, 0.f, 0.f);
        float s0, s1, s2;
        gate_scales(c, s0, s1, s2);
        const float o[4] = {ov.x, ov.y, ov.z, ov.w}, C4[4] = {cq.x, cq.y, cq.z, cq.w}, R4[4] = {rq.x, rq.y, rq.z, rq.w};
        const float B0[4] = {bq[0].x, bq[0].y, bq[0].z, bq[0].w}, B1[4] = {bq[1].x, bq[1].y, bq[1].z, bq[1].w},
                    B2[4] = {bq[2].x, bq[2].y, bq[2].z, bq[2].w}, BR[4] = {bq[3].x, bq[3].y, bq[3].z, bq[3].w};
        float y[4];
#pragma unroll
        for (int e = 0; e < 4; ++e) {
            const float qv = epi_sum(o[e], s0, s1, s2, B0[e], B1[e], B2[e], BR[e], C4[e], R4[e]);
            y[e] = (p.act && !(qv > 0.f)) ? qv * p.slope : qv;
            if (DROP) y[e] = drop_apply(p, dseed, m0 + er, ec + e, y[e]);
        }
        const int64_t yr = p.map_y ? ngram_row(p, m0 + er) : m0 + er;
        *reinterpret_cast<float4*>(p.Y + yr * p.ldy + ec) = make_float4(y[0], y[1], y[2], y[3]);
    };
    if constexpr (!LDSE) {
        bool y_pending = false;
        for (int64_t i = 0; i < ntl; ++i) {
            const int ab = (int)(i & 1);
            [[maybe_unused]] const int si = (int)i;
            DSTAMP(si, 0);
            if (y_pending) asm volatile("s_waitcnt vmcnt(1)" ::: "memory");
            else asm volatile("s_waitcnt vmcnt(0)" ::: "memory");
            lds_barrier();
            DSTAMP(si, 1);
            const int64_t m0 = tile_of(i) * BM;
            load_CR(tile_of(i));
            __builtin_amdgcn_sched_barrier(0);
            const int64_t a_tile = tile_of(i + 2);
            float* const a_dst = ab ? Af1 : Af0;
            const int g_slot = (int)((i + 2) & 3);
            const bool do_split = i + 1 < ntl;
            if (!IL) {
                issue_A(a_tile, a_dst);
                if (wave == 0) issue_G(a_tile, g_slot);
            }
            DSTAMP(si, 2);
            auto mfma_epi = [&](int pt) {
                mfma_tile(ab, a_tile, a_dst, g_slot, IL);
                DSTAMP(si, pt);
                wait_CR();
                DSTAMP(si, pt + 1);
                float c[5];
                lds_gates5<BM * 4>(&Gi[(int)(i & 3)][0][er], c);
                if (!DEXP(2) && m0 + er < p.M) {
                    epilogue(m0, make_float4(acc[0], acc[1], acc[2], acc[3]), make_float4(cv[0], cv[1], cv[2], cv[3]),
                             make_float4(rv[0], rv[1], rv[2], rv[3]), c);
                }
                DSTAMP(si, pt + 2);
            };
            if (mfma_first) {
                mfma_epi(3);
                if (do_split) split_tile(ab ? Af0 : Af1, ab ^ 1, (int)((i + 1) & 3));
                DSTAMP(si, 6);
            } else {
                if (do_split) split_tile(ab ? Af0 : Af1, ab ^ 1, (int)((i + 1) & 3));
                DSTAMP(si, 3);
                mfma_epi(4);
            }
            y_pending = !DEXP(2) && m0 + BM <= p.M;
        }
    } else {
        bool y_pending = false;
        for (int64_t i = 0; i <= ntl && ntl > 0; ++i) {
            const int ab = (int)(i & 1);
            [[maybe_unused]] const int si = (int)i;
            DSTAMP(si, 0);
            if (y_pending) asm volatile("s_waitcnt vmcnt(1)" ::: "memory");
            else asm volatile("s_waitcnt vmcnt(0)" ::: "memory");
            lds_barrier();
            DSTAMP(si, 1);
            if (i >= 1) {
#pragma unroll
                for (int e = 0; e < 4; ++e) lds_stf(&Es[(4 * kg + e) * ELD + col], acc[e]);
            }
            issue_CR(tile_of(i - 1));
            const int64_t a_tile = tile_of(i + 2);
            float* const a_dst = ab ? Af1 : Af0;
            const int g_slot = (int)((i + 2) & 3);
            const bool do_mfma = i < ntl, do_split = i + 1 < ntl;
            if (!IL || !do_mfma) {
                issue_A(a_tile, a_dst);
                if (wave == 0) issue_G(a_tile, g_slot);
            }
            DSTAMP(si, 2);
            if (mfma_first) {
                if (do_mfma) mfma_tile(ab, a_tile, a_dst, g_slot, IL);
                DSTAMP(si, 3);
                if (do_split) split_tile(ab ? Af0 : Af1, ab ^ 1, (int)((i + 1) & 3));
            } else {
                if (do_split) split_tile(ab ? Af0 : Af1, ab ^ 1, (int)((i + 1) & 3));
                DSTAMP(si, 3);
                if (do_mfma) mfma_tile(ab, a_tile, a_dst, g_slot, IL);
            }
            DSTAMP(si, 4);
            if (wave == 0) asm volatile("s_waitcnt vmcnt(%0)" ::"n"(NI + NG) : "memory");
            else asm volatile("s_waitcnt vmcnt(%0)" ::"n"(NI) : "memory");
            DSTAMP(si, 5);
            lds_barrier();
            DSTAMP(si, 6);
            y_pending = false;
            if (i >= 1) {
                const int64_t m0 = tile_of(i - 1) * BM;
                const int gs = (int)((i - 1) & 3);
                if (m0 + er < p.M) {
                    float4 cq, rq, ov;
                    float c[5];
                    lds_epi<BM * 4>(&Cs[er * 128 + ec], &Rs[er * 128 + ec], &Es[er * ELD + ec], &Gi[gs][0][er], cq, rq, ov, c);
                    if (!DEXP(2)) {
                        epilogue(m0, ov, cq, rq, c);
                        y_pending = true;
                    }
                }
            }
            DSTAMP(si, 7);
        }
    }
    asm volatile("s_waitcnt vmcnt(0)" ::: "memory");
}

__global__ __launch_bounds__(256) void pack_kernel(int F_in, int F_out, int K, const float* W0, const float* W1,
                                                   const float* W2, const float* Ws, const float* Wr,
                                                   const float* bm0, const float* bs0, const float* bm1,
                                                   const float* bs1, const float* bm2, const float* bs2,
                                                   const float* br, float* out) {
    const int64_t total = (int64_t)F_out * K;
    for (int64_t i = (int64_t)blockIdx.x * 256 + threadIdx.x; i < total + 4 * F_out; i += (int64_t)gridDim.x * 256) {
        if (i < total) {
            const int n = (int)(i / K), k = (int)(i % K);
            const int q = seg_of(k, F_in), kk = k - q * F_in;
            const int64_t w = (int64_t)n * F_in + kk;
            float v;
            if (q == 0) v = W0[w] + Ws[w];
            else if (q == 1) v = W1[w] + Ws[w];
            else if (q == 2) v = W2[w] + Ws[w];
            else v = Wr[w];
            out[i] = v;
        } else {
            const int j = (int)(i - total), q = j / F_out, n = j % F_out;
            float v;
            if (q == 0) v = bm0[n] + bs0[n];
            else if (q == 1) v = bm1[n] + bs1[n];
            else if (q == 2) v = bm2[n] + bs2[n];
            else v = br ? br[n] : 0.f;
            out[i] = v;
        }
    }
}

}

extern "C" {

int64_t pg_directgcn_packed_floats(int64_t F_in, int64_t F_out, int has_res_proj) {
    return F_out * (has_res_proj ? 4 : 3) * F_in + 4 * F_out;
}

int pg_directgcn_pack_f32(const pg_layer_args_t* a, float* packed, void* stream) {
    PG_REQUIRE(a != nullptr && packed != nullptr, "null args");
    PG_REQUIRE(a->F_in > 0 && a->F_out > 0 && a->F_in < (1 << 20) && a->F_out < (1 << 20), "bad F_in/F_out");
    PG_REQUIRE(a->W_main_in && a->W_main_out && a->W_undirected && a->W_shared, "null weight");
    PG_REQUIRE(a->b_main_in && a->b_dir_shared_in && a->b_main_out && a->b_dir_shared_out && a->b_undirected &&
                   a->b_undirected_shared,
               "null bias");
    const int K = (int)((a->W_res ? 4 : 3) * a->F_in);
    const int64_t total = a->F_out * K + 4 * a->F_out;
    const int64_t nb = (total + 255) / 256 < 1024 ? (total + 255) / 256 : 1024;
    hipLaunchKernelGGL(pack_kernel, dim3((unsigned)nb), dim3(256), 0, (hipStream_t)stream, (int)a->F_in,
                       (int)a->F_out, K, a->W_main_in, a->W_main_out, a->W_undirected, a->W_shared, a->W_res,
                       a->b_main_in, a->b_dir_shared_in, a->b_main_out, a->b_dir_shared_out, a->b_undirected,
                       a->b_undirected_shared, a->b_res, packed);
    return pg::check_launch("pg_directgcn_pack_f32");
}

static int dense_launch(const pg_layer_args_t* a, const float* packed, uint32_t flags, const int64_t* ngmap,
                        void* stream) {
    PG_REQUIRE(a != nullptr, "null args");
    PG_REQUIRE(a->M >= 0 && a->F_in > 0 && a->F_out > 0 && a->F_in < (1 << 20) && a->F_out < (1 << 20),
               "bad shape M=%lld F_in=%lld F_out=%lld", (long long)a->M, (long long)a->F_in, (long long)a->F_out);
    if (a->M == 0) return PG_OK;
    PG_REQUIRE(a->Z && a->ldz >= 3 * a->F_in, "Z must be [M, >=3*F_in]");
    PG_REQUIRE(a->C_in && a->C_out && a->C_directed && a->C_undirected && a->C_all, "null gate");
    PG_REQUIRE(a->gate_mode == PG_GATES_VECTOR || a->gate_mode == PG_GATES_SCALAR, "bad gate_mode");
    PG_REQUIRE(!a->constant || a->ld_const >= a->F_out, "ld_const < F_out");
    PG_REQUIRE(!a->W_res || a->res_x, "W_res needs res_x");
    PG_REQUIRE(!a->res_x || a->W_res || a->F_in == a->F_out, "identity residual needs F_in == F_out");
    PG_REQUIRE(!a->res_x || a->ld_res >= a->F_in, "ld_res < F_in");
    PG_REQUIRE(a->Y && a->ldy >= a->F_out, "bad output");
    DenseP p{};
    p.M = a->M;
    p.F_in = (int)a->F_in;
    p.F_out = (int)a->F_out;
    p.K = (int)((a->W_res ? 4 : 3) * a->F_in);
    p.Z = a->Z;
    p.ldz = a->ldz;
    p.Bp = packed;
    p.bsum = packed ? packed + (int64_t)p.F_out * p.K : nullptr;
    if (!packed) {
        PG_REQUIRE(a->W_main_in && a->W_main_out && a->W_undirected && a->W_shared && a->b_main_in &&
                       a->b_dir_shared_in && a->b_main_out && a->b_dir_shared_out && a->b_undirected &&
                       a->b_undirected_shared,
                   "packed == NULL needs the raw weights and biases in the args");
        p.rawW = 1;
        p.Wq0 = a->W_main_in;
        p.Wq1 = a->W_main_out;
        p.Wq2 = a->W_undirected;
        p.Wsh = a->W_shared;
        p.bm0 = a->b_main_in;
        p.bs0 = a->b_dir_shared_in;
        p.bm1 = a->b_main_out;
        p.bs1 = a->b_dir_shared_out;
        p.bm2 = a->b_undirected;
        p.bs2 = a->b_undirected_shared;
    }
    p.gate_mode = a->gate_mode;
    p.C_in = a->C_in;
    p.C_out = a->C_out;
    p.C_dir = a->C_directed;
    p.C_und = a->C_undirected;
    p.C_all = a->C_all;
    p.rows = a->rows;
    p.constant = a->constant;
    p.ld_const = a->ld_const;
    p.res_x = a->res_x;
    p.ld_res = a->ld_res;
    p.proj_res = a->W_res ? 1 : 0;
    p.act = a->act;
    p.slope = a->slope;
    p.Y = a->Y;
    p.ldy = a->ldy;
    p.remap = (flags & PG_FLAG_NO_XCD_REMAP) ? 0 : 1;
    p.pregated = (flags & PG_FLAG_DENSE_PREGATED) ? 1 : 0;
    p.nt_a = (flags & PG_FLAG_DENSE_A_CACHED) ? 0 : 1;
    if (const int rc = pg::drop_params(a, p.drop_thr, p.drop_s)) return rc;
    p.drop_seed = a->drop_seed;
    PG_REQUIRE(p.drop_s == 0.f || a->M * a->F_out <= (int64_t(1) << 32), "fused dropout: M * F_out > 2^32");
#ifdef PG_DENSE_EXP
    p.exp = (int)((flags >> 24) & 31u);
#endif
    if (ngmap) {
        p.map_kn1 = ngmap[0];
        p.map_m0 = ngmap[1];
        p.map_res = ngmap[2] ? 1 : 0;
        p.map_y = ngmap[3] ? 1 : 0;
    }
    p.vec_out = (a->F_out % 4 == 0) && (a->ldy % 4 == 0) && pg::aligned16(a->Y) &&
                (!a->constant || (a->ld_const % 4 == 0 && pg::aligned16(a->constant))) &&
                (!a->res_x || a->W_res || (a->ld_res % 4 == 0 && pg::aligned16(a->res_x)));
    bool vec = (a->F_in % 4 == 0) && (a->ldz % 4 == 0) && pg::aligned16(a->Z) && pg::aligned16(packed);
    if (a->res_x) vec = vec && pg::aligned16(a->res_x) && (a->ld_res % 4 == 0);
    const bool wide = a->F_out > 64;
    const int64_t BN = wide ? 128 : 64;
    const int64_t nb = ((a->M + 127) / 128) * ((a->F_out + BN - 1) / BN);
    hipStream_t s = (hipStream_t)stream;
    const bool ws_shape_ok = a->F_out == 128 && vec && p.vec_out &&
                             (!a->res_x || (a->ld_res % 4 == 0 && pg::aligned16(a->res_x)));
    if (!(flags & PG_FLAG_DENSE_TILED) && ws_shape_ok && a->ldz < (1 << 24) && a->rows == nullptr &&
        (!a->res_x || a->ld_res < (1 << 24)) &&
        ((a->F_in == 128 && !a->W_res) || (a->F_in == 64 && a->W_res))) {
        if (ngmap && a->F_in != 128)
            return pg::set_error(PG_ERR_UNSUPPORTED, "pg_directgcn_dense_ngram_rows_f32: F_in = F_out = 128 only");
        const int ncu = pg::cu_count();
        if (a->F_in == 128) {
            if (p.rawW && !(pg::aligned16(a->W_main_in) && pg::aligned16(a->W_main_out) &&
                            pg::aligned16(a->W_undirected) && pg::aligned16(a->W_shared)))
                return pg::set_error(PG_ERR_UNSUPPORTED, "pg_directgcn_dense_f32: unpacked weights must be 16-B aligned");
            const int64_t T16 = (a->M + 15) / 16;
            const unsigned g16 = (unsigned)(T16 < ncu ? T16 : ncu);
            const bool il = (flags & PG_FLAG_DENSE_NO_IL) == 0;
            const bool ldse = (flags & PG_FLAG_DENSE_LDS_EPILOGUE) != 0;
            const bool drop = p.drop_s != 0.f;
            void (*kern)(DenseP);
#define PG_X3P_PICK(LDSE)                                                                                  \
    kern = drop ? (p.pregated ? dense_x3p_kernel<true, true, true, LDSE> : dense_x3p_kernel<false, true, true, LDSE>) \
           : p.pregated ? (il ? dense_x3p_kernel<true, true, false, LDSE> : dense_x3p_kernel<true, false, false, LDSE>) \
                        : (il ? dense_x3p_kernel<false, true, false, LDSE> : dense_x3p_kernel<false, false, false, LDSE>)
            if (ldse) PG_X3P_PICK(true);
            else PG_X3P_PICK(false);
#undef PG_X3P_PICK
            hipLaunchKernelGGL(kern, dim3(g16), dim3(512), 0, s, p);
        } else {
            if (p.rawW)
                return pg::set_error(PG_ERR_UNSUPPORTED, "pg_directgcn_dense_f32: unpacked weights need the pipelined "
                                                         "split-bf16 kernel (F_in = F_out = 128, no row map)");
            const int64_t T = (a->M + 31) / 32;
            const unsigned g = (unsigned)(T < ncu ? T : ncu);
            if (p.pregated) hipLaunchKernelGGL((dense_x3_kernel<64, 4, true>), dim3(g), dim3(512), 0, s, p);
            else hipLaunchKernelGGL((dense_x3_kernel<64, 4, false>), dim3(g), dim3(512), 0, s, p);
        }
        return pg::check_launch("pg_directgcn_dense_f32");
    }
    if (ngmap)
        return pg::set_error(PG_ERR_UNSUPPORTED, "pg_directgcn_dense_ngram_rows_f32: needs the pipelined split-bf16 "
                                                 "kernel's shape (F_in = F_out = 128, no W_res, no row map, aligned)");
    if (p.rawW)
        return pg::set_error(PG_ERR_UNSUPPORTED, "pg_directgcn_dense_f32: unpacked weights need the pipelined "
                                                 "split-bf16 kernel (F_in = F_out = 128, no row map)");
    if (vec) {
        if (wide) hipLaunchKernelGGL((dense_kernel<128, 128, 8, true>), dim3((unsigned)nb), dim3(512), 0, s, p);
        else hipLaunchKernelGGL((dense_kernel<128, 64, 8, true>), dim3((unsigned)nb), dim3(512), 0, s, p);
    } else {
        if (wide) hipLaunchKernelGGL((dense_kernel<128, 128, 8, false>), dim3((unsigned)nb), dim3(512), 0, s, p);
        else hipLaunchKernelGGL((dense_kernel<128, 64, 8, false>), dim3((unsigned)nb), dim3(512), 0, s, p);
    }
    return pg::check_launch("pg_directgcn_dense_f32");
}

int pg_directgcn_dense_f32(const pg_layer_args_t* a, const float* packed, uint32_t flags, void* stream) {
    return dense_launch(a, packed, flags, nullptr, stream);
}

#ifdef PG_DENSE_EXP
int pg_dense_set_stamps(unsigned long long* buf) {
    return hipMemcpyToSymbol(HIP_SYMBOL(g_dense_stamps), &buf, sizeof(buf)) == hipSuccess ? PG_OK : PG_ERR_HIP;
}
#endif

int pg_directgcn_dense_ngram_rows_f32(const pg_layer_args_t* a, const float* packed, int64_t Kn1, int64_t m0,
                                      int32_t map_res, int32_t map_y, uint32_t flags, void* stream) {
    PG_REQUIRE(a != nullptr, "null args");
    int64_t pw = 20;
    while (pw < Kn1 && pw <= (int64_t(1) << 56)) pw *= 20;
    PG_REQUIRE(Kn1 >= 20 && pw == Kn1 && m0 >= 0 && m0 < Kn1,
               "bad n-gram map (Kn1 = %lld must be a power of K = 20; m0 = %lld)", (long long)Kn1, (long long)m0);
    PG_REQUIRE(a->M % 400 == 0 && a->M < (int64_t(1) << 31), "rows must be whole middles (M = %lld)", (long long)a->M);
    PG_REQUIRE(!map_res || a->res_x, "map_res needs res_x");
    PG_REQUIRE(m0 + a->M / 400 <= Kn1 / 20, "middles [%lld, %lld) past the graph's %lld", (long long)m0,
               (long long)(m0 + a->M / 400), (long long)(Kn1 / 20));
    const int64_t map[4] = {Kn1, m0, map_res, map_y};
    return dense_launch(a, packed, flags, map, stream);
}

}
```

### protgram-directgcn_amd/csrc/pg_head.hip

```cpp
#include "pg_common.h"
#include "pg_split3.h"

namespace {

typedef float f32x16 __attribute__((ext_vector_type(16)));
typedef float f32x4 __attribute__((ext_vector_type(4)));

constexpr int HB = 64;

struct HeadP {
    int64_t M;
    int F, H, C;
    const float* h;
    const uint16_t* hb;
    int64_t ldh;
    const float *W1, *b1, *W2, *b2;
    float eps;
    float* logp;
    int64_t ldp;
    float* emb;
    int64_t lde;
};

using pg::ld4;

template <int FMAX, int HMAX, int CMAX>
__global__ __launch_bounds__(256) void head_kernel(HeadP p) {
    constexpr int HLD = FMAX + 4, ZLD = HMAX + 4, LLD = CMAX + 1;
    static_assert(HB * LLD <= HB * HLD, "logits alias the h tile");
    constexpr int PF = HB * FMAX / 4 / 256;
    __shared__ __attribute__((aligned(16))) float Hs[HB * HLD];
    __shared__ __attribute__((aligned(16))) float Zs[HB * ZLD];
    float* Ls = Hs;
    const int tid = threadIdx.x, wave = tid >> 6, lane = tid & 63;
    const int li = lane & 31, lh = lane >> 5;
    const int F4 = p.F >> 2;
    const int64_t ntiles = (p.M + HB - 1) / HB;

    float4 hv[PF];
    auto load = [&](int64_t t) {
#pragma unroll
        for (int q = 0; q < PF; ++q) {
            const int idx = tid + 256 * q;
            const int r = idx / (FMAX / 4), c4 = idx % (FMAX / 4);
            const int64_t m = t * HB + r;
            if (m < p.M && c4 < F4) {
                if (p.hb) {
                    const uint2 w = *reinterpret_cast<const uint2*>(p.hb + m * p.ldh + 4 * c4);
                    hv[q] = make_float4(__uint_as_float(w.x << 16), __uint_as_float(w.x & 0xffff0000u),
                                        __uint_as_float(w.y << 16), __uint_as_float(w.y & 0xffff0000u));
                } else {
                    hv[q] = ld4(p.h + m * p.ldh + 4 * c4);
                }
            } else {
                hv[q] = make_float4(0.f, 0.f, 0.f, 0.f);
            }
        }
    };
    int64_t t = blockIdx.x;
    if (t < ntiles) load(t);
    for (; t < ntiles; t += gridDim.x) {
        const int64_t m0 = t * HB;
#pragma unroll
        for (int q = 0; q < PF; ++q) {
            const int idx = tid + 256 * q;
            const int r = idx / (FMAX / 4), c4 = idx % (FMAX / 4);
            *reinterpret_cast<float4*>(&Hs[r * HLD + 4 * c4]) = hv[q];
        }
        __syncthreads();
        if (t + gridDim.x < ntiles) load(t + gridDim.x);

        {
            const int g = lane >> 4, tt = lane & 15;
            for (int r = wave * 4 + g; r < HB; r += 16) {
                float ss = 0.f;
                for (int c4 = tt; c4 < F4; c4 += 16) {
                    const float4 v = ld4(&Hs[r * HLD + 4 * c4]);
                    ss += v.x * v.x + v.y * v.y + v.z * v.z + v.w * v.w;
                }
#pragma unroll
                for (int o = 8; o > 0; o >>= 1) ss += __shfl_xor(ss, o, 16);
                const int64_t m = m0 + r;
                if (m < p.M) {
                    const float inv = 1.0f / (sqrtf(ss) + p.eps);
                    for (int c4 = tt; c4 < F4; c4 += 16) {
                        float4 v = ld4(&Hs[r * HLD + 4 * c4]);
                        v = make_float4(v.x * inv, v.y * inv, v.z * inv, v.w * inv);
                        *reinterpret_cast<float4*>(p.emb + m * p.lde + 4 * c4) = v;
                    }
                }
            }
        }

        {
            const int ntile_n = (p.H + 31) / 32;
            for (int tile = wave; tile < 2 * ntile_n; tile += 4) {
                const int tm = tile / ntile_n, tn = tile % ntile_n;
                const int j = tn * 32 + li;
                const bool jok = j < p.H;
                const float* w1row = p.W1 + (int64_t)(jok ? j : 0) * p.F;
                constexpr int KG = FMAX / 8;
                float4 bf[KG];
#pragma unroll
                for (int g = 0; g < KG; ++g) {
                    const int k = g * 8 + 4 * lh;
                    bf[g] = (jok && k < p.F) ? ld4(w1row + k) : make_float4(0.f, 0.f, 0.f, 0.f);
                }
                f32x16 acc;
#pragma unroll
                for (int r = 0; r < 16; ++r) acc[r] = 0.f;
#pragma unroll
                for (int g = 0; g < KG; ++g) {
                    const int k = g * 8 + 4 * lh;
                    const float4 a = k < p.F ? ld4(&Hs[(tm * 32 + li) * HLD + k]) : make_float4(0.f, 0.f, 0.f, 0.f);
                    const float4 b = bf[g];
                    acc = __builtin_amdgcn_mfma_f32_32x32x2f32(a.x, b.x, acc, 0, 0, 0);
                    acc = __builtin_amdgcn_mfma_f32_32x32x2f32(a.y, b.y, acc, 0, 0, 0);
                    acc = __builtin_amdgcn_mfma_f32_32x32x2f32(a.z, b.z, acc, 0, 0, 0);
                    acc = __builtin_amdgcn_mfma_f32_32x32x2f32(a.w, b.w, acc, 0, 0, 0);
                }
                const float bj = jok ? p.b1[j] : 0.f;
#pragma unroll
                for (int r = 0; r < 16; ++r) {
                    const int row = tm * 32 + (r & 3) + 8 * (r >> 2) + 4 * lh;
                    const float z = acc[r] + bj;
                    if (j < ZLD - 4) Zs[row * ZLD + j] = jok ? (z > 0.f ? z : 0.f) : 0.f;
                }
            }
        }
        __syncthreads();

        {
            const int ntile_n = (p.C + 31) / 32;
            for (int tile = wave; tile < 2 * ntile_n; tile += 4) {
                const int tm = tile / ntile_n, tn = tile % ntile_n;
                const int c = tn * 32 + li;
                const bool cok = c < p.C;
                const float* w2row = p.W2 + (int64_t)(cok ? c : 0) * p.H;
                constexpr int KG = HMAX / 8;
                float4 bf[KG];
#pragma unroll
                for (int g = 0; g < KG; ++g) {
                    const int k = g * 8 + 4 * lh;
                    bf[g] = (cok && k < p.H) ? ld4(w2row + k) : make_float4(0.f, 0.f, 0.f, 0.f);
                }
                f32x16 acc;
#pragma unroll
                for (int r = 0; r < 16; ++r) acc[r] = 0.f;
#pragma unroll
                for (int g = 0; g < KG; ++g) {
                    const int k = g * 8 + 4 * lh;
                    const float4 a = k < p.H ? ld4(&Zs[(tm * 32 + li) * ZLD + k]) : make_float4(0.f, 0.f, 0.f, 0.f);
                    const float4 b = bf[g];
                    acc = __builtin_amdgcn_mfma_f32_32x32x2f32(a.x, b.x, acc, 0, 0, 0);
                    acc = __builtin_amdgcn_mfma_f32_32x32x2f32(a.y, b.y, acc, 0, 0, 0);
                    acc = __builtin_amdgcn_mfma_f32_32x32x2f32(a.z, b.z, acc, 0, 0, 0);
                    acc = __builtin_amdgcn_mfma_f32_32x32x2f32(a.w, b.w, acc, 0, 0, 0);
                }
                const float bc = cok ? p.b2[c] : 0.f;
#pragma unroll
                for (int r = 0; r < 16; ++r) {
                    const int row = tm * 32 + (r & 3) + 8 * (r >> 2) + 4 * lh;
                    if (cok) Ls[row * LLD + c] = acc[r] + bc;
                }
            }
        }
        __syncthreads();

        {
            const int r = tid >> 2, tt = tid & 3;
            const int64_t m = m0 + r;
            float mx = -INFINITY;
            for (int c = tt; c < p.C; c += 4) mx = fmaxf(mx, Ls[r * LLD + c]);
            mx = fmaxf(mx, __shfl_xor(mx, 1, 4));
            mx = fmaxf(mx, __shfl_xor(mx, 2, 4));
            float se = 0.f;
            for (int c = tt; c < p.C; c += 4) se += expf(Ls[r * LLD + c] - mx);
            se += __shfl_xor(se, 1, 4);
            se += __shfl_xor(se, 2, 4);
            const float lse = mx + logf(se);
            if (m < p.M)
                for (int c = tt; c < p.C; c += 4) p.logp[m * p.ldp + c] = Ls[r * LLD + c] - lse;
        }
        __syncthreads();
    }
}

__global__ __launch_bounds__(256) __attribute__((amdgpu_waves_per_eu(4, 8))) void head_f128_kernel(HeadP p) {
    constexpr int BM = 32, F = 128, H = 64, CP = 32;
    constexpr int HLD = F + 8, ZLD = H + 8, LLD = CP + 1;
    __shared__ __attribute__((aligned(16))) float Hs[BM * HLD];
    __shared__ __attribute__((aligned(16))) float Zs[BM * ZLD];
    __shared__ __attribute__((aligned(16))) float Ls[BM * LLD];
    const int tid = threadIdx.x, wave = tid >> 6, lane = tid & 63;
    const int li = lane & 15, q = lane >> 4;
    const int64_t m0 = (int64_t)blockIdx.x * BM;
    float4 hv[4];
#pragma unroll
    for (int k = 0; k < 4; ++k) {
        const int r = (tid >> 5) + 8 * k;
        const int64_t m = m0 + r;
        if (m >= p.M) {
            hv[k] = make_float4(0.f, 0.f, 0.f, 0.f);
        } else if (p.hb) {
            const uint2 w = *reinterpret_cast<const uint2*>(p.hb + m * p.ldh + 4 * (tid & 31));
            hv[k] = make_float4(__uint_as_float(w.x << 16), __uint_as_float(w.x & 0xffff0000u),
                                __uint_as_float(w.y << 16), __uint_as_float(w.y & 0xffff0000u));
        } else {
            hv[k] = ld4(p.h + m * p.ldh + 4 * (tid & 31));
        }
    }
    float4 w1f[8], w2f[4];
    {
        const float* w1row = p.W1 + (int64_t)(16 * wave + li) * F + 4 * q;
#pragma unroll
        for (int m = 0; m < 8; ++m) w1f[m] = ld4(w1row + 16 * m);
        const int c = 16 * (wave >> 1) + li;
        const bool cok = c < p.C;
        const float* w2row = p.W2 + (int64_t)(cok ? c : 0) * H + 4 * q;
#pragma unroll
        for (int m = 0; m < 4; ++m) w2f[m] = cok ? ld4(w2row + 16 * m) : make_float4(0.f, 0.f, 0.f, 0.f);
    }
    const float b1v = p.b1[16 * wave + li];
    const int c2 = 16 * (wave >> 1) + li;
    const float b2v = c2 < p.C ? p.b2[c2] : 0.f;
#pragma unroll
    for (int k = 0; k < 4; ++k) *reinterpret_cast<float4*>(&Hs[((tid >> 5) + 8 * k) * HLD + 4 * (tid & 31)]) = hv[k];
    __syncthreads();
    {
        const int r = tid >> 3, part = tid & 7;
        float4 v[4];
        float ss = 0.f;
#pragma unroll
        for (int k = 0; k < 4; ++k) {
            v[k] = ld4(&Hs[r * HLD + 16 * part + 4 * k]);
            ss += v[k].x * v[k].x + v[k].y * v[k].y + v[k].z * v[k].z + v[k].w * v[k].w;
        }
        ss += __shfl_xor(ss, 1, 8);
        ss += __shfl_xor(ss, 2, 8);
        ss += __shfl_xor(ss, 4, 8);
        const int64_t m = m0 + r;
        if (m < p.M) {
            const float inv = 1.0f / (sqrtf(ss) + p.eps);
#pragma unroll
            for (int k = 0; k < 4; ++k)
                *reinterpret_cast<float4*>(p.emb + m * p.lde + 16 * part + 4 * k) =
                    make_float4(v[k].x * inv, v[k].y * inv, v[k].z * inv, v[k].w * inv);
        }
    }
    {
        f32x4 acc[2] = {f32x4{0.f, 0.f, 0.f, 0.f}, f32x4{0.f, 0.f, 0.f, 0.f}};
#pragma unroll
        for (int m = 0; m < 8; ++m) {
#pragma unroll
            for (int rb = 0; rb < 2; ++rb) {
                const float4 a = ld4(&Hs[(16 * rb + li) * HLD + 4 * q + 16 * m]);
                acc[rb] = __builtin_amdgcn_mfma_f32_16x16x4f32(a.x, w1f[m].x, acc[rb], 0, 0, 0);
                acc[rb] = __builtin_amdgcn_mfma_f32_16x16x4f32(a.y, w1f[m].y, acc[rb], 0, 0, 0);
                acc[rb] = __builtin_amdgcn_mfma_f32_16x16x4f32(a.z, w1f[m].z, acc[rb], 0, 0, 0);
                acc[rb] = __builtin_amdgcn_mfma_f32_16x16x4f32(a.w, w1f[m].w, acc[rb], 0, 0, 0);
            }
        }
#pragma unroll
        for (int rb = 0; rb < 2; ++rb)
#pragma unroll
            for (int i = 0; i < 4; ++i) {
                const float z = acc[rb][i] + b1v;
                Zs[(16 * rb + 4 * q + i) * ZLD + 16 * wave + li] = z > 0.f ? z : 0.f;
            }
    }
    __syncthreads();
    {
        const int rb = wave & 1;
        f32x4 acc = {0.f, 0.f, 0.f, 0.f};
#pragma unroll
        for (int m = 0; m < 4; ++m) {
            const float4 a = ld4(&Zs[(16 * rb + li) * ZLD + 4 * q + 16 * m]);
            acc = __builtin_amdgcn_mfma_f32_16x16x4f32(a.x, w2f[m].x, acc, 0, 0, 0);
            acc = __builtin_amdgcn_mfma_f32_16x16x4f32(a.y, w2f[m].y, acc, 0, 0, 0);
            acc = __builtin_amdgcn_mfma_f32_16x16x4f32(a.z, w2f[m].z, acc, 0, 0, 0);
            acc = __builtin_amdgcn_mfma_f32_16x16x4f32(a.w, w2f[m].w, acc, 0, 0, 0);
        }
#pragma unroll
        for (int i = 0; i < 4; ++i) Ls[(16 * rb + 4 * q + i) * LLD + c2] = acc[i] + b2v;
    }
    __syncthreads();
    {
        const int r = tid >> 3, part = tid & 7;
        const int64_t m = m0 + r;
        float mx = -INFINITY;
        for (int c = part; c < p.C; c += 8) mx = fmaxf(mx, Ls[r * LLD + c]);
        mx = fmaxf(mx, __shfl_xor(mx, 1, 8));
        mx = fmaxf(mx, __shfl_xor(mx, 2, 8));
        mx = fmaxf(mx, __shfl_xor(mx, 4, 8));
        float se = 0.f;
        for (int c = part; c < p.C; c += 8) se += expf(Ls[r * LLD + c] - mx);
        se += __shfl_xor(se, 1, 8);
        se += __shfl_xor(se, 2, 8);
        se += __shfl_xor(se, 4, 8);
        const float lse = mx + logf(se);
        if (m < p.M)
            for (int c = part; c < p.C; c += 8) p.logp[m * p.ldp + c] = Ls[r * LLD + c] - lse;
    }
}

__global__ __launch_bounds__(256) __attribute__((amdgpu_waves_per_eu(4, 8))) void head_x3_kernel(HeadP p) {
    constexpr int BM = 32, F = 128, H = 64, CP = 32;
    constexpr int ZLD = H + 8, LLD = CP + 1;
    constexpr int NU = F / 8;
    __shared__ __attribute__((aligned(16))) uint4 As[3][BM * NU];
    __shared__ __attribute__((aligned(16))) float Ls[BM * LLD];
    float* Zs = reinterpret_cast<float*>(&As[0][0]);
    static_assert(BM * ZLD * 4 <= 3 * BM * NU * 16, "Zs fits the split images");
    const int tid = threadIdx.x, wave = tid >> 6, lane = tid & 63;
    const int li = lane & 15, q = lane >> 4;
    const int64_t m0 = (int64_t)blockIdx.x * BM;
    const int c4 = tid & 31;
    float4 hv[4];
#pragma unroll
    for (int k = 0; k < 4; ++k) {
        const int64_t m = m0 + (tid >> 5) + 8 * k;
        if (m >= p.M) {
            hv[k] = make_float4(0.f, 0.f, 0.f, 0.f);
        } else if (p.hb) {
            const uint2 w = *reinterpret_cast<const uint2*>(p.hb + m * p.ldh + 4 * c4);
            hv[k] = make_float4(__uint_as_float(w.x << 16), __uint_as_float(w.x & 0xffff0000u),
                                __uint_as_float(w.y << 16), __uint_as_float(w.y & 0xffff0000u));
        } else {
            hv[k] = ld4(p.h + m * p.ldh + 4 * c4);
        }
    }
    uint4 w0[4], w1[4], w2[4];
    {
        const float* w1row = p.W1 + (int64_t)(16 * wave + li) * F + 8 * q;
#pragma unroll
        for (int s = 0; s < 4; ++s) {
            const float4 x0 = ld4(w1row + 32 * s), x1 = ld4(w1row + 32 * s + 4);
            const float v[8] = {x0.x, x0.y, x0.z, x0.w, x1.x, x1.y, x1.z, x1.w};
            pgx3::split8(v, w0[s], w1[s], w2[s]);
        }
    }
    float4 w2f[4];
    {
        const int c = 16 * (wave >> 1) + li;
        const float* w2row = p.W2 + (int64_t)(c < p.C ? c : 0) * H + 4 * q;
#pragma unroll
        for (int m = 0; m < 4; ++m) w2f[m] = ld4(w2row + 16 * m);
    }
    const float b1v = p.b1[16 * wave + li];
    const int c2 = 16 * (wave >> 1) + li;
    const float b2v = c2 < p.C ? p.b2[c2] : 0.f;
#pragma unroll
    for (int k = 0; k < 4; ++k) {
        const int r = (tid >> 5) + 8 * k;
        const float4 v = hv[k];
        float ss = v.x * v.x + v.y * v.y + v.z * v.z + v.w * v.w;
#pragma unroll
        for (int o = 1; o < 32; o <<= 1) ss += __shfl_xor(ss, o, 32);
        const int64_t m = m0 + r;
        if (m < p.M) {
            const float inv = 1.0f / (sqrtf(ss) + p.eps);
            *reinterpret_cast<float4*>(p.emb + m * p.lde + 4 * c4) = make_float4(v.x * inv, v.y * inv, v.z * inv, v.w * inv);
        }
        uint32_t s0[2], s1[2], s2[2];
        {
            float fa, fb;
            float a = v.x, b = v.y;
            s0[0] = pgx3::bf2(a, b, fa, fb); a -= fa; b -= fb;
            s1[0] = pgx3::bf2(a, b, fa, fb); a -= fa; b -= fb;
            s2[0] = pgx3::bf2(a, b, fa, fb);
            a = v.z; b = v.w;
            s0[1] = pgx3::bf2(a, b, fa, fb); a -= fa; b -= fb;
            s1[1] = pgx3::bf2(a, b, fa, fb); a -= fa; b -= fb;
            s2[1] = pgx3::bf2(a, b, fa, fb);
        }
        const int u = c4 >> 1;
        uint2* d0 = reinterpret_cast<uint2*>(&As[0][r * NU + (u ^ (r & 15))]) + (c4 & 1);
        uint2* d1 = reinterpret_cast<uint2*>(&As[1][r * NU + (u ^ (r & 15))]) + (c4 & 1);
        uint2* d2 = reinterpret_cast<uint2*>(&As[2][r * NU + (u ^ (r & 15))]) + (c4 & 1);
        *d0 = make_uint2(s0[0], s0[1]);
        *d1 = make_uint2(s1[0], s1[1]);
        *d2 = make_uint2(s2[0], s2[1]);
    }
    __syncthreads();
    f32x4 acc[2] = {f32x4{0.f, 0.f, 0.f, 0.f}, f32x4{0.f, 0.f, 0.f, 0.f}};
#pragma unroll
    for (int s = 0; s < 4; ++s) {
#pragma unroll
        for (int rb = 0; rb < 2; ++rb) {
            const int r = 16 * rb + li, u = 4 * s + q;
            const int pos = r * NU + (u ^ (r & 15));
            acc[rb] = pgx3::mfma_x3(As[0][pos], As[1][pos], As[2][pos], w0[s], w1[s], w2[s], acc[rb]);
        }
    }
    __syncthreads();
#pragma unroll
    for (int rb = 0; rb < 2; ++rb)
#pragma unroll
        for (int i = 0; i < 4; ++i) {
            const float z = acc[rb][i] + b1v;
            Zs[(16 * rb + 4 * q + i) * ZLD + 16 * wave + li] = z > 0.f ? z : 0.f;
        }
    __syncthreads();
    {
        const int rb = wave & 1;
        f32x4 a = {0.f, 0.f, 0.f, 0.f};
#pragma unroll
        for (int m = 0; m < 4; ++m) {
            const float4 x = ld4(&Zs[(16 * rb + li) * ZLD + 4 * q + 16 * m]);
            a = __builtin_amdgcn_mfma_f32_16x16x4f32(x.x, w2f[m].x, a, 0, 0, 0);
            a = __builtin_amdgcn_mfma_f32_16x16x4f32(x.y, w2f[m].y, a, 0, 0, 0);
            a = __builtin_amdgcn_mfma_f32_16x16x4f32(x.z, w2f[m].z, a, 0, 0, 0);
            a = __builtin_amdgcn_mfma_f32_16x16x4f32(x.w, w2f[m].w, a, 0, 0, 0);
        }
#pragma unroll
        for (int i = 0; i < 4; ++i) Ls[(16 * rb + 4 * q + i) * LLD + c2] = a[i] + b2v;
    }
    __syncthreads();
    {
        const int r = tid >> 3, part = tid & 7;
        const int64_t m = m0 + r;
        float mx = -INFINITY;
        for (int c = part; c < p.C; c += 8) mx = fmaxf(mx, Ls[r * LLD + c]);
        mx = fmaxf(mx, __shfl_xor(mx, 1, 8));
        mx = fmaxf(mx, __shfl_xor(mx, 2, 8));
        mx = fmaxf(mx, __shfl_xor(mx, 4, 8));
        float se = 0.f;
        for (int c = part; c < p.C; c += 8) se += expf(Ls[r * LLD + c] - mx);
        se += __shfl_xor(se, 1, 8);
        se += __shfl_xor(se, 2, 8);
        se += __shfl_xor(se, 4, 8);
        const float lse = mx + logf(se);
        if (m < p.M)
            for (int c = part; c < p.C; c += 8) p.logp[m * p.ldp + c] = Ls[r * LLD + c] - lse;
    }
}

__global__ __launch_bounds__(256) void head_generic_kernel(HeadP p) {
    extern __shared__ float sm[];
    const int wave = threadIdx.x >> 6, lane = threadIdx.x & 63;
    const int64_t m = (int64_t)blockIdx.x * 4 + wave;
    float* hs = sm + wave * (p.F + p.H + p.C);
    float* zs = hs + p.F;
    float* ls = zs + p.H;
    if (m >= p.M) return;
    float ss = 0.f;
    for (int f = lane; f < p.F; f += 64) {
        const float v = p.h[m * p.ldh + f];
        hs[f] = v;
        ss += v * v;
    }
    for (int o = 32; o > 0; o >>= 1) ss += __shfl_xor(ss, o);
    const float inv = 1.0f / (sqrtf(ss) + p.eps);
    for (int f = lane; f < p.F; f += 64) p.emb[m * p.lde + f] = hs[f] * inv;
    __builtin_amdgcn_wave_barrier();
    for (int j = lane; j < p.H; j += 64) {
        float z = p.b1[j];
        for (int f = 0; f < p.F; ++f) z += p.W1[(int64_t)j * p.F + f] * hs[f];
        zs[j] = z > 0.f ? z : 0.f;
    }
    __builtin_amdgcn_wave_barrier();
    float mx = -INFINITY;
    for (int c = lane; c < p.C; c += 64) {
        float l = p.b2[c];
        for (int k = 0; k < p.H; ++k) l += p.W2[(int64_t)c * p.H + k] * zs[k];
        ls[c] = l;
        mx = fmaxf(mx, l);
    }
    for (int o = 32; o > 0; o >>= 1) mx = fmaxf(mx, __shfl_xor(mx, o));
    __builtin_amdgcn_wave_barrier();
    float se = 0.f;
    for (int c = lane; c < p.C; c += 64) se += expf(ls[c] - mx);
    for (int o = 32; o > 0; o >>= 1) se += __shfl_xor(se, o);
    const float lse = mx + logf(se);
    for (int c = lane; c < p.C; c += 64) p.logp[m * p.ldp + c] = ls[c] - lse;
}

}

namespace {
int head_launch(int64_t M, int64_t F, int64_t H, int64_t C, const float* h, const uint16_t* hb, int64_t ldh,
                const float* W1, const float* b1, const float* W2, const float* b2, float eps, float* logp, int64_t ldp,
                float* emb, int64_t lde, void* stream) {
    PG_REQUIRE(M >= 0 && F > 0 && H > 0 && C > 0 && F < (1 << 16) && H < (1 << 16) && C < (1 << 16), "bad shape");
    if (M == 0) return PG_OK;
    PG_REQUIRE((h || hb) && W1 && b1 && W2 && b2 && logp && emb, "null pointer");
    PG_REQUIRE(ldh >= F && lde >= F && ldp >= C, "bad leading dimension");
    HeadP p{M, (int)F, (int)H, (int)C, h, hb, ldh, W1, b1, W2, b2, eps, logp, ldp, emb, lde};
    hipStream_t s = (hipStream_t)stream;
    const bool in_ok = hb ? ((reinterpret_cast<uintptr_t>(hb) & 7) == 0) : pg::aligned16(h);
    const bool vec = F % 4 == 0 && H % 4 == 0 && ldh % 4 == 0 && lde % 4 == 0 && in_ok &&
                     pg::aligned16(emb) && pg::aligned16(W1) && pg::aligned16(W2);
    if (hb && !(vec && F <= 256 && H <= 128 && C <= 64))
        return pg::set_error(PG_ERR_UNSUPPORTED, "pg_directgcn_head_bf16: needs F <= 256, H <= 128, C <= 64, "
                                                 "F, H, ldh multiples of 4");
    const int64_t ntiles = (M + HB - 1) / HB;
    auto grid_of = [&](int64_t per_cu) {
        const int64_t slots = 256 * per_cu;
        const int64_t per_block = (ntiles + slots - 1) / slots;
        return (unsigned)((ntiles + per_block - 1) / per_block);
    };
    if (vec && F == 128 && H == 64 && C <= 32 && ldh % 4 == 0 && lde % 4 == 0) {
#ifdef PG_HEAD_FP32
        hipLaunchKernelGGL(head_f128_kernel, dim3((unsigned)((M + 31) / 32)), dim3(256), 0, s, p);
#else
        hipLaunchKernelGGL(head_x3_kernel, dim3((unsigned)((M + 31) / 32)), dim3(256), 0, s, p);
#endif
    } else if (vec && F <= 128 && H <= 64 && C <= 32) {
        hipLaunchKernelGGL((head_kernel<128, 64, 32>), dim3(grid_of(2)), dim3(256), 0, s, p);
    } else if (vec && F <= 256 && H <= 128 && C <= 64) {
        hipLaunchKernelGGL((head_kernel<256, 128, 64>), dim3(grid_of(1)), dim3(256), 0, s, p);
    } else {
        const size_t shm = 4 * (size_t)(F + H + C) * sizeof(float);
        PG_REQUIRE(shm <= 160 * 1024, "head too wide for the generic kernel");
        hipLaunchKernelGGL(head_generic_kernel, dim3((unsigned)((M + 3) / 4)), dim3(256), shm, s, p);
    }
    return pg::check_launch("pg_directgcn_head_f32");
}
}

extern "C" int pg_directgcn_head_f32(int64_t M, int64_t F, int64_t H, int64_t C, const float* h, int64_t ldh,
                                     const float* W1, const float* b1, const float* W2, const float* b2, float eps,
                                     float* logp, int64_t ldp, float* emb, int64_t lde, void* stream) {
    return head_launch(M, F, H, C, h, nullptr, ldh, W1, b1, W2, b2, eps, logp, ldp, emb, lde, stream);
}

extern "C" int pg_directgcn_head_bf16(int64_t M, int64_t F, int64_t H, int64_t C, const uint16_t* h, int64_t ldh,
                                      const float* W1, const float* b1, const float* W2, const float* b2, float eps,
                                      float* logp, int64_t ldp, float* emb, int64_t lde, void* stream) {
    return head_launch(M, F, H, C, nullptr, h, ldh, W1, b1, W2, b2, eps, logp, ldp, emb, lde, stream);
}
```

### protgram-directgcn_amd/layer.py

```python
from __future__ import annotations

import weakref
from typing import List, Optional, Tuple

import torch
import torch.nn as nn
import torch.nn.functional as F

from . import ops
from .graph import csr_from_coo, _single, _key

_ROWS_OK: dict = {}


def _check_rows(rows: torch.Tensor, limit: int):
    k = _key(rows, n=limit)
    hit = _ROWS_OK.get(k)
    if hit is not None and hit() is rows:
        return
    if rows.numel():
        lo, hi = int(rows.min()), int(rows.max())
        if lo < 0 or hi >= limit:
            raise IndexError(f"original_indices in [{lo}, {hi}] outside [0, {limit})")
    ops.rows_distinct(rows)
    if len(_ROWS_OK) > 1024:
        _ROWS_OK.clear()
    _ROWS_OK[k] = weakref.ref(rows)


class DirectGCNLayer(nn.Module):

    def __init__(self, in_channels: int, out_channels: int, num_nodes: int, use_vector_coeffs: bool = True):
        super().__init__()
        self.aggr = "add"
        self.in_channels = in_channels
        self.out_channels = out_channels
        self.num_nodes = num_nodes
        self.use_vector_coeffs = use_vector_coeffs
        self.lin_main_in = nn.Linear(in_channels, out_channels, bias=False)
        self.lin_main_out = nn.Linear(in_channels, out_channels, bias=False)
        self.lin_undirected = nn.Linear(in_channels, out_channels, bias=False)
        self.bias_main_in = nn.Parameter(torch.empty(out_channels))
        self.bias_main_out = nn.Parameter(torch.empty(out_channels))
        self.bias_undirected = nn.Parameter(torch.empty(out_channels))
        self.lin_shared = nn.Linear(in_channels, out_channels, bias=False)
        self.bias_directed_shared_in = nn.Parameter(torch.empty(out_channels))
        self.bias_directed_shared_out = nn.Parameter(torch.empty(out_channels))
        self.bias_undirected_shared = nn.Parameter(torch.empty(out_channels))
        if self.use_vector_coeffs and self.num_nodes > 0:
            self.C_in_vec = nn.Parameter(torch.empty(num_nodes, 1))
            self.C_out_vec = nn.Parameter(torch.empty(num_nodes, 1))
            self.C_directed_vec = nn.Parameter(torch.empty(num_nodes, 1))
            self.C_undirected_vec = nn.Parameter(torch.empty(num_nodes, 1))
            self.C_all_vec = nn.Parameter(torch.empty(num_nodes, 1))
        else:
            self.use_vector_coeffs = False
            self.C_in = nn.Parameter(torch.empty(1))
            self.C_out = nn.Parameter(torch.empty(1))
            self.C_directed = nn.Parameter(torch.empty(1))
            self.C_undirected = nn.Parameter(torch.empty(1))
            self.C_all = nn.Parameter(torch.empty(1))
        if self.num_nodes > 0:
            self.constant = nn.Parameter(torch.empty(num_nodes, out_channels))
        else:
            self.constant = None
        self.reset_parameters()

    def reset_parameters(self):
        for lin in [self.lin_main_in, self.lin_main_out, self.lin_shared, self.lin_undirected]:
            nn.init.xavier_uniform_(lin.weight)
        for bias in [self.bias_main_in, self.bias_main_out, self.bias_directed_shared_in,
                     self.bias_directed_shared_out, self.bias_undirected, self.bias_undirected_shared]:
            nn.init.zeros_(bias)
        if self.use_vector_coeffs:
            for c in (self.C_in_vec, self.C_out_vec, self.C_directed_vec, self.C_undirected_vec, self.C_all_vec):
                nn.init.ones_(c)
        else:
            for c in (self.C_in, self.C_out, self.C_directed, self.C_undirected, self.C_all):
                nn.init.ones_(c)
        if self.constant is not None:
            nn.init.xavier_uniform_(self.constant)

    def message(self, x_j: torch.Tensor, edge_weight: Optional[torch.Tensor]) -> torch.Tensor:
        if edge_weight is None:
            return x_j
        return edge_weight.view(-1, 1) * x_j

    def propagate(self, edge_index: torch.Tensor, x: torch.Tensor, edge_weight: Optional[torch.Tensor] = None):
        ops._require_gpu(x, edge_index)
        k = ("p1",) + _key(edge_index, edge_weight, n=x.size(0))
        hit = _P1_CACHE.get(k)
        if hit is None:
            a = _single(edge_index, edge_weight, x.size(0))
            if len(_P1_CACHE) > 16:
                _P1_CACHE.clear()
            _P1_CACHE[k] = ((edge_index, edge_weight), a)
        else:
            a = hit[1]
        return ops.Propagate1.apply(x, a)

    def _dense_params(self):
        if self.use_vector_coeffs:
            C = (self.C_in_vec, self.C_out_vec, self.C_directed_vec, self.C_undirected_vec, self.C_all_vec)
        else:
            C = (self.C_in, self.C_out, self.C_directed, self.C_undirected, self.C_all)
        return (self.lin_main_in.weight, self.lin_main_out.weight, self.lin_undirected.weight, self.lin_shared.weight,
                self.bias_main_in, self.bias_directed_shared_in, self.bias_main_out, self.bias_directed_shared_out,
                self.bias_undirected, self.bias_undirected_shared, *C)

    def fused_forward(self, x, graph, original_indices=None, res_x=None, W_res=None, b_res=None, act=False,
                      fused_norm: bool = False, drop=None):
        if drop is not None and not act:
            raise ValueError("fused dropout needs the activation")
        M = x.size(0)
        rows = None
        if self.use_vector_coeffs:
            if original_indices is not None:
                rows = original_indices.to(device=x.device, dtype=torch.int64)
                if rows.numel() != M:
                    raise ValueError("original_indices must have one entry per row of x")
                _check_rows(rows, self.num_nodes)
            elif self.num_nodes != M:
                raise RuntimeError(f"vector coefficients hold {self.num_nodes} nodes but x has {M} rows "
                                   "(pass original_indices for subgraphs)")
        if graph.n_rows != M:
            raise ValueError("graph rows != x rows")
        constant = self.constant if self.use_vector_coeffs else None
        gate_mode = 0 if self.use_vector_coeffs else 1
        params = self._dense_params()
        if (ops.PREGATED_INFERENCE and rows is None and not fused_norm
                and not (torch.is_grad_enabled() and (x.requires_grad or any(p.requires_grad for p in params)))):
            prm = dict(zip(ops._DENSE_KEYS, params))
            Z = ops.spmm3_gated(graph, x, prm, gate_mode)
            if Z is not None:
                return ops.layer_dense(Z, prm, gate_mode, constant=constant, res_x=res_x, W_res=W_res, b_res=b_res,
                                       act=act, pregated=True, drop=drop)
        if (ops.SPAN_BACKWARD and torch.is_grad_enabled() and x.requires_grad
                and ops.PropagateDense.supports(graph, x, self.out_channels, res_x, W_res, rows, fused_norm)):
            return ops.PropagateDense.apply(x, graph, res_x is not None, constant, gate_mode, act, ops.LEAKY_SLOPE,
                                            drop, *params)
        Z = ops.Propagate3.apply(x, graph, fused_norm)
        return ops.LayerDense.apply(Z, res_x, constant, W_res, b_res, rows, gate_mode, act, ops.LEAKY_SLOPE, drop,
                                    *params)

    def forward(self, x: torch.Tensor,
                edge_index_in: torch.Tensor, edge_weight_in: Optional[torch.Tensor],
                edge_index_out: torch.Tensor, edge_weight_out: Optional[torch.Tensor],
                edge_index_undirected: torch.Tensor, edge_weight_undirected: Optional[torch.Tensor],
                original_indices: Optional[torch.Tensor] = None) -> torch.Tensor:
        ops._require_gpu(x, edge_index_in, edge_index_out, edge_index_undirected)
        g = csr_from_coo(x.size(0), edge_index_in, edge_weight_in, edge_index_out, edge_weight_out,
                         edge_index_undirected, edge_weight_undirected)
        return self.fused_forward(x, g, original_indices)


_P1_CACHE: dict = {}


class Bf16InputCache:

    def __init__(self):
        self._ref, self._version, self.buffer = None, None, None

    def __call__(self, x: torch.Tensor) -> torch.Tensor:
        xb = self.buffer
        if xb is not None and self._ref() is x and self._version == x._version:
            return xb
        if xb is not None and xb.shape == x.shape and xb.device == x.device:
            xb.copy_(x)
        else:
            xb = x.to(torch.bfloat16)
        self._ref, self._version, self.buffer = weakref.ref(x), x._version, xb
        return xb


class ProtGramDirectGCN(nn.Module):

    def __init__(self, layer_dims: List[int], num_graph_nodes: Optional[int],
                 task_num_output_classes: int, n_gram_len: int,
                 one_gram_dim: int, max_pe_len: int, dropout: float,
                 use_vector_coeffs: bool, l2_eps: float = 1e-12):
        super().__init__()
        self.n_gram_len = n_gram_len
        self.one_gram_dim = one_gram_dim
        self.dropout = dropout
        self.l2_eps = l2_eps
        self.pe_layer = None
        if one_gram_dim > 0 and max_pe_len > 0:
            self.pe_layer = nn.Embedding(max_pe_len, one_gram_dim)
        self.convs = nn.ModuleList()
        self.res_projs = nn.ModuleList()
        if not layer_dims or len(layer_dims) < 2:
            raise ValueError("layer_dims must contain at least input and output dimensions (length >= 2).")
        for i in range(len(layer_dims) - 1):
            in_dim, out_dim = layer_dims[i], layer_dims[i + 1]
            current_num_nodes = num_graph_nodes if num_graph_nodes is not None else 0
            effective = use_vector_coeffs and current_num_nodes > 0
            self.convs.append(DirectGCNLayer(in_dim, out_dim, current_num_nodes, effective))
            self.res_projs.append(nn.Linear(in_dim, out_dim) if in_dim != out_dim else nn.Identity())
        final_dim = layer_dims[-1]
        hidden = final_dim // 2 if final_dim > 1 else 1
        self.decoder_fc = nn.Sequential(nn.Linear(final_dim, hidden), nn.ReLU(), nn.Dropout(p=0.5),
                                        nn.Linear(hidden, task_num_output_classes))
        self.fused_norm = False
        self.compute_dtype = torch.float32
        self._xb = Bf16InputCache()

    def _apply_pe(self, x: torch.Tensor) -> torch.Tensor:
        if self.pe_layer is None:
            return x
        if self.n_gram_len > 0 and self.one_gram_dim > 0 and x.shape[1] == self.n_gram_len * self.one_gram_dim:
            pos = min(self.n_gram_len, self.pe_layer.num_embeddings)
            xr = x.view(-1, self.n_gram_len, self.one_gram_dim)
            if pos > 0:
                pe = self.pe_layer(torch.arange(0, pos, device=x.device, dtype=torch.long))
                pad = pe.new_zeros(self.n_gram_len - pos, self.one_gram_dim)
                xr = xr + torch.cat([pe, pad], 0).unsqueeze(0)
            return xr.reshape(-1, self.n_gram_len * self.one_gram_dim)
        return x

    def graph_of(self, data):
        g = getattr(data, "graph", None)
        if g is not None:
            x = getattr(data, "x", None)
            if x is not None and g.device != x.device:
                g = g.to(x.device)
                data.graph = g
            return g
        x = data.x
        return csr_from_coo(x.size(0), data.edge_index_in, getattr(data, "edge_weight_in", None),
                            data.edge_index_out, getattr(data, "edge_weight_out", None),
                            data.edge_index_undirected_norm, getattr(data, "edge_weight_undirected_norm", None))

    def forward(self, data) -> Tuple[torch.Tensor, torch.Tensor]:
        return self.head(self.body(data))

    def body(self, data) -> torch.Tensor:
        x = getattr(data, "x", None)
        ei_in = getattr(data, "edge_index_in", None)
        ei_out = getattr(data, "edge_index_out", None)
        ei_undir = getattr(data, "edge_index_undirected_norm", None)
        original_indices = getattr(data, "original_indices", None)
        has_graph = getattr(data, "graph", None) is not None
        if x is None or (not has_graph and (ei_in is None or ei_out is None or ei_undir is None)):
            raise ValueError("ProtGramDirectGCN requires 'x', 'edge_index_in', 'edge_index_out', and "
                             "'edge_index_undirected_norm' in the Data object.")
        ops._require_gpu(x)
        g = self.graph_of(data)
        h = self._apply_pe(x)
        if self.compute_dtype == torch.bfloat16:
            h = self.bf16_input(h) if (h is x and h.dtype != torch.bfloat16 and not h.requires_grad) else h.to(
                torch.bfloat16)
        elif self.compute_dtype != torch.float32:
            raise ValueError("compute_dtype must be torch.float32 or torch.bfloat16")
        p = float(self.dropout) if self.training else 0.0
        seeds = None
        if ops.FUSED_DROPOUT and 0.0 < p < 1.0:
            seeds = torch.randint(0, 1 << 62, (len(self.convs),), device=x.device, dtype=torch.int64)
        for i, (conv, res) in enumerate(zip(self.convs, self.res_projs)):
            drop = (p, seeds[i:i + 1]) if seeds is not None else None
            if isinstance(res, nn.Linear):
                h = conv.fused_forward(h, g, original_indices, res_x=h, W_res=res.weight, b_res=res.bias, act=True,
                                       fused_norm=self.fused_norm, drop=drop)
            else:
                h = conv.fused_forward(h, g, original_indices, res_x=h, act=True, fused_norm=self.fused_norm,
                                       drop=drop)
            if drop is None:
                h = F.dropout(h, p=self.dropout, training=self.training)
        return h

    def bf16_input(self, x: torch.Tensor) -> torch.Tensor:
        return self._xb(x)

    def head_train_args(self):
        dec = self.decoder_fc
        if not (len(dec) == 4 and isinstance(dec[0], nn.Linear) and isinstance(dec[1], nn.ReLU) and
                isinstance(dec[2], nn.Dropout) and isinstance(dec[3], nn.Linear)):
            return None
        return dec[0].weight, dec[0].bias, dec[3].weight, dec[3].bias, dec[2].p if self.training else 0.0

    def head(self, h, need_emb: bool = True):
        dec = self.decoder_fc
        if not self.training and not torch.is_grad_enabled() and h.is_cuda:
            return ops.head(h, dec[0].weight, dec[0].bias, dec[3].weight, dec[3].bias, self.l2_eps)
        h = h.float()
        if h.is_cuda and len(dec) == 4 and isinstance(dec[0], nn.Linear) and isinstance(dec[3], nn.Linear):
            a = dec[2](dec[1](ops.row_linear(h, dec[0].weight, dec[0].bias)))
            logits = ops.row_linear(a, dec[3].weight, dec[3].bias)
        else:
            logits = dec(h)
        if not need_emb:
            return F.log_softmax(logits, dim=-1), None
        emb = h / (torch.norm(h, p=2, dim=1, keepdim=True) + self.l2_eps)
        return F.log_softmax(logits, dim=-1), emb
```

### protgram-directgcn_amd/ops.py

```python
from __future__ import annotations

import contextlib
import ctypes
import functools
import weakref
from typing import Optional

import torch

from . import _lib
from ._lib import PG_FLAG_NGRAM_BLOCK4, PG_FLAG_NO_NGRAM, LayerArgs, check, default_flags, load_library
from .graph import CSRGraph, ShapedAdjacency

LEAKY_SLOPE = 0.01

FUSED_DROPOUT = True

SPAN_BACKWARD = True
BF16_BACKWARD = True
PREGATED_INFERENCE = True

SPMM_EVENTS: Optional[list] = None
DENSE_EVENTS: Optional[list] = None
HEAD_EVENTS: Optional[list] = None


def _ev_start(x, kind: str = "SPMM"):
    if globals()[kind + "_EVENTS"] is None:
        return None
    e0 = torch.cuda.Event(enable_timing=True)
    e0.record(torch.cuda.current_stream(x.device))
    return e0


def _ev_end(x, e0, kind: str = "SPMM"):
    lst = globals()[kind + "_EVENTS"]
    if e0 is not None and lst is not None:
        e1 = torch.cuda.Event(enable_timing=True)
        e1.record(torch.cuda.current_stream(x.device))
        lst.append((e0, e1))


def _require_graph_on(g, x):
    for t in g.tensors():
        if t.device != x.device:
            raise RuntimeError(f"graph tensors on {t.device} but features on {x.device}: move the graph "
                               "(CSRGraph.to) -- the kernels read both")


def _require_gpu(*ts):
    for t in ts:
        if t is None:
            continue
        if not t.is_cuda:
            raise RuntimeError("protgram_directgcn_amd runs on the MI355X only: got a CPU tensor "
                               "(move the model and data to 'cuda'; there is no CPU fallback)")
        if t.dtype not in (torch.float32, torch.bfloat16, torch.int32, torch.int64):
            raise TypeError(f"unsupported dtype {t.dtype}")


_DEFER_CONST_GRAD = False
_DEFERRED_GRADS: dict = {}


@contextlib.contextmanager
def deferring_const_grads(enabled: bool):
    global _DEFER_CONST_GRAD
    prev, _DEFER_CONST_GRAD = _DEFER_CONST_GRAD, bool(enabled)
    try:
        yield
    finally:
        _DEFER_CONST_GRAD = prev
        _DEFERRED_GRADS.clear()


def deferred_grad(p: torch.Tensor):
    return _DEFERRED_GRADS.get(p.data_ptr()) if _DEFERRED_GRADS else None


_ROWS_DISTINCT: dict = {}


def rows_info(rows: torch.Tensor) -> tuple:
    k = (rows.data_ptr(), rows._version, tuple(rows.shape), rows.dtype, str(rows.device))
    hit = _ROWS_DISTINCT.get(k)
    if hit is not None and hit[0]() is rows:
        return hit[1]
    if rows.numel():
        info = (int(torch.unique(rows).numel()) == rows.numel(), int(rows.min()), int(rows.max()))
    else:
        info = (True, 0, -1)
    if len(_ROWS_DISTINCT) > 1024:
        _ROWS_DISTINCT.clear()
    _ROWS_DISTINCT[k] = (weakref.ref(rows), info)
    return info


def rows_distinct(rows: torch.Tensor) -> bool:
    return rows_info(rows)[0]


def _rows_fileable(p, rows) -> bool:
    return (_DEFER_CONST_GRAD and rows is not None and p is not None and p.dtype == torch.float32 and p.dim() == 2
            and p.size(1) > 0 and p.is_contiguous() and p.is_leaf and p.requires_grad and rows.dim() == 1
            and rows.dtype == torch.int64 and rows.device == p.device and rows_distinct(rows))


def _file_rows(p, grad: torch.Tensor, rows) -> bool:
    if not _rows_fileable(p, rows):
        return False
    if not (grad.dtype in (torch.float32, torch.bfloat16) and grad.dim() == 2 and grad.size(1) == p.size(1)
            and grad.size(0) == rows.numel() and grad.device == p.device):
        return False
    if p.data_ptr() in _DEFERRED_GRADS:
        raise RuntimeError("a deferred gradient was filed twice for one parameter")
    _DEFERRED_GRADS[p.data_ptr()] = (grad.contiguous(), rows)
    return True


def _defer_const(constant, need: bool, M: int, rows) -> bool:
    return (_DEFER_CONST_GRAD and need and constant is not None and constant.dtype == torch.float32 and rows is None
            and constant.dim() == 2 and constant.size(0) == M and constant.is_contiguous()
            and constant.is_leaf and constant.requires_grad)


def _file_deferred(constant, dpre) -> bool:
    if not (_is_bf16(dpre) and dpre.is_contiguous() and dpre.shape == constant.shape):
        return False
    if constant.data_ptr() in _DEFERRED_GRADS:
        raise RuntimeError("a deferred gradient was filed twice for one parameter")
    _DEFERRED_GRADS[constant.data_ptr()] = dpre
    return True


def _p(t: Optional[torch.Tensor]):
    return None if t is None else ctypes.c_void_p(t.data_ptr())


def _stream(t: torch.Tensor):
    return ctypes.c_void_p(torch.cuda.current_stream(t.device).cuda_stream)


def _f32c(t: torch.Tensor) -> torch.Tensor:
    return t.contiguous() if t.dtype == torch.float32 else t.float().contiguous()


def _bf16c(t: torch.Tensor) -> torch.Tensor:
    return t.contiguous() if t.dtype == torch.bfloat16 else t.to(torch.bfloat16).contiguous()


def _is_bf16(t) -> bool:
    return t is not None and t.dtype == torch.bfloat16


def _ngram_ok(g: CSRGraph, x: torch.Tensor, fl: int, widths=(64, 128), dtype=torch.float32) -> bool:
    return (g.ngram is not None and not (fl & PG_FLAG_NO_NGRAM) and x.dtype == dtype
            and x.size(0) == g.n_rows and x.size(1) in widths)


def _mid_ok(g: CSRGraph, x: torch.Tensor, fl: int) -> bool:
    return (g.ngram is not None and g.ngram.mplan is not None and not (fl & (PG_FLAG_NO_NGRAM | PG_FLAG_NGRAM_BLOCK4))
            and x.dtype in (torch.float32, torch.bfloat16) and x.size(0) == g.n_rows and x.size(1) % 16 == 0)


def _ngram_fwd(lib, g, x, a, Z, fl, s):
    ng, N, F = g.ngram, g.n_rows, x.size(1)
    if _mid_ok(g, x, fl):
        rc = lib.pg_spmm3_ngram_mid_f32(ng.K, ng.n, N, _p(ng.mplan), _p(x), x.stride(0), F, a, _p(Z), Z.stride(0), fl, s)
        if rc != _lib.PG_ERR_UNSUPPORTED:
            return rc
    if _ngram_ok(g, x, fl, (64, 128, 256)):
        return lib.pg_spmm3_ngram_f32(ng.K, ng.n, N, _p(ng.plan), _p(x), x.stride(0), F, a, _p(Z), Z.stride(0), fl, s)
    return _lib.PG_ERR_UNSUPPORTED


def _map_ok(g: CSRGraph, x: torch.Tensor, fl: int) -> bool:
    return (g.ngram_map is not None and not (fl & PG_FLAG_NO_NGRAM) and x.dtype == torch.float32
            and x.size(0) == g.n_rows and x.size(1) % 16 == 0)


def _map_fwd(lib, g, x, Z, fl, s):
    m, F = g.ngram_map, x.size(1)
    rc = lib.pg_spmm3_ngram_mid_map_f32(m.K, m.n, _p(m.mplan), _p(m.gmap), _p(x), x.stride(0), F, _p(Z), Z.stride(0),
                                        fl, s)
    if rc:
        return rc
    if m.res_rows.numel():
        check(lib.pg_spmm3_resid_f32(m.res_rows.numel(), _p(m.res_rowptr), _p(m.res_rows), _p(m.res_edges), _p(x),
                                     x.stride(0), F, _p(Z), Z.stride(0), fl, s), "pg_spmm3_resid_f32")
    return 0


def spmm3(g: CSRGraph, x: torch.Tensor, out: Optional[torch.Tensor] = None, fused: bool = False,
          flags: Optional[int] = None) -> torch.Tensor:
    lib = load_library()
    if _is_bf16(x):
        return _spmm3_bf16(lib, g, x, out, fused, flags)
    x = _f32c(x)
    _require_gpu(x)
    _require_graph_on(g, x)
    N, F = g.n_rows, x.size(1)
    if x.size(0) < N:
        raise ValueError("x has fewer rows than the graph")
    Z = out if out is not None else torch.empty(N, 3 * F, device=x.device, dtype=torch.float32)
    fl = default_flags() if flags is None else flags
    s = _stream(x)
    ev = _ev_start(x)
    if g.shared and not fused and g.ngram is not None:
        rc = _ngram_fwd(lib, g, x, None, Z, fl, s)
        if rc != _lib.PG_ERR_UNSUPPORTED:
            check(rc, "pg_spmm3_ngram_(mid_)f32")
            _ev_end(x, ev)
            return Z
    if g.shared and not fused and _map_ok(g, x, fl):
        rc = _map_fwd(lib, g, x, Z, fl, s)
        if rc != _lib.PG_ERR_UNSUPPORTED:
            check(rc, "pg_spmm3_ngram_mid_map_f32")
            _ev_end(x, ev)
            return Z
    if g.shared:
        if fused:
            if g.raw is None:
                raise ValueError("graph has no raw-count records (build it with build_propagation_csr)")
            check(lib.pg_spmm3_fusednorm_f32(N, _p(g.rowptr), _p(g.row_order), _p(g.raw), _p(g.node_norm), g.eps, _p(x),
                                             x.stride(0), F, _p(Z), Z.stride(0), fl, s), "pg_spmm3_fusednorm_f32")
        else:
            check(lib.pg_spmm3_f32(N, _p(g.rowptr), _p(g.row_order), _p(g.edges3), _p(x), x.stride(0), F, _p(Z),
                                   Z.stride(0), fl, s), "pg_spmm3_f32")
    else:
        for k, a in enumerate(g.adj):
            check(lib.pg_spmm1_f32(N, _p(a.rowptr), None, _p(a.edges), _p(x), x.stride(0), F, _p(Z[:, k * F:]),
                                   Z.stride(0), 0, fl, s), "pg_spmm1_f32")
    _ev_end(x, ev)
    return Z


def spmm3_middles(g: CSRGraph, x: torch.Tensor, m_begin: int, m_end: int, flags: Optional[int] = None,
                  out: Optional[torch.Tensor] = None) -> torch.Tensor:
    lib = load_library()
    bf = _is_bf16(x)
    x = _bf16c(x) if bf else _f32c(x)
    _require_gpu(x)
    _require_graph_on(g, x)
    fl = default_flags() if flags is None else flags
    if not _mid_ok(g, x, fl):
        raise ValueError("spmm3_middles needs a graph with a middle plan and fp32 x with F % 16 == 0")
    ng, N, F = g.ngram, g.n_rows, x.size(1)
    K2 = ng.K * ng.K
    rows = (m_end - m_begin) * K2
    Z = out if out is not None else torch.empty(rows, 3 * F, device=x.device, dtype=x.dtype)
    if Z.shape != (rows, 3 * F) or Z.stride(1) != 1 or Z.dtype != x.dtype:
        raise ValueError("out must be [(m_end - m_begin) K^2, 3F] of x's dtype with unit column stride")
    ev = _ev_start(x)
    fn = lib.pg_spmm3_ngram_mid_rows_bf16 if bf else lib.pg_spmm3_ngram_mid_rows_f32
    check(fn(ng.K, ng.n, N, _p(ng.mplan), _p(x), x.stride(0), F, m_begin, m_end, _p(Z), Z.stride(0), fl, _stream(x)),
          "pg_spmm3_ngram_mid_rows_" + ("bf16" if bf else "f32"))
    _ev_end(x, ev)
    return Z


_IDX_OK: dict = {}


def _check_index(idx: torch.Tensor, n: int, distinct: bool, what: str):
    k = (idx.data_ptr(), idx._version, idx.numel(), str(idx.device), int(n), bool(distinct))
    hit = _IDX_OK.get(k)
    if hit is not None and hit() is idx:
        return
    if idx.numel():
        lo, hi = int(idx.min()), int(idx.max())
        if lo < 0 or hi >= n:
            raise IndexError(f"{what}: row indices in [{lo}, {hi}] outside [0, {n})")
        if distinct and int(torch.unique(idx).numel()) != idx.numel():
            raise ValueError(f"{what}: indices must be distinct (each destination row written once)")
    if len(_IDX_OK) > 256:
        _IDX_OK.clear()
    _IDX_OK[k] = weakref.ref(idx)


def rows_gather(src: torch.Tensor, idx: torch.Tensor, out: Optional[torch.Tensor] = None,
                check_idx: bool = True) -> torch.Tensor:
    lib = load_library()
    _require_gpu(src)
    if src.dim() != 2 or src.stride(1) != 1:
        raise ValueError("rows_gather needs a 2-D source with unit column stride")
    idx = idx.to(device=src.device, dtype=torch.int64).contiguous()
    if check_idx:
        _check_index(idx, src.size(0), False, "rows_gather")
    out = out if out is not None else torch.empty(idx.numel(), src.size(1), device=src.device, dtype=src.dtype)
    if out.shape != (idx.numel(), src.size(1)) or out.dtype != src.dtype or out.stride(1) != 1:
        raise ValueError("rows_gather: out must be [len(idx), src.size(1)] of src's dtype")
    es = src.element_size()
    check(lib.pg_rows_gather(_p(src), src.stride(0) * es, _p(idx), idx.numel(), src.size(1) * es, _p(out),
                             out.stride(0) * es, _stream(src)), "pg_rows_gather")
    return out


def rows_scatter(src: torch.Tensor, idx: torch.Tensor, dst: torch.Tensor, check_idx: bool = True) -> torch.Tensor:
    lib = load_library()
    _require_gpu(src)
    if src.dim() != 2 or dst.dim() != 2 or src.size(1) != dst.size(1) or src.dtype != dst.dtype:
        raise ValueError("rows_scatter: src and dst must be 2-D of the same width and dtype")
    if src.stride(1) != 1 or dst.stride(1) != 1 or idx.numel() != src.size(0):
        raise ValueError("rows_scatter: unit column strides and one index per source row")
    idx = idx.to(device=src.device, dtype=torch.int64).contiguous()
    if check_idx:
        _check_index(idx, dst.size(0), True, "rows_scatter")
    es = src.element_size()
    check(lib.pg_rows_scatter(_p(src), src.stride(0) * es, _p(idx), idx.numel(), src.size(1) * es, _p(dst),
                              dst.stride(0) * es, _stream(src)), "pg_rows_scatter")
    return dst


def rows_gather_sum(A: Optional[torch.Tensor], rowptr: torch.Tensor, idx: torch.Tensor, n_out: int, F: int,
                    B: Optional[torch.Tensor] = None, out_dtype=torch.float32) -> torch.Tensor:
    lib = load_library()
    ref = A if A is not None else B
    _require_gpu(ref)
    for t in (A, B):
        if t is not None and (t.dim() != 2 or t.stride(1) != 1 or t.size(1) < F):
            raise ValueError("rows_gather_sum: 2-D sources with unit column stride and >= F columns")
    if A is not None and A.dtype != torch.float32:
        raise ValueError("rows_gather_sum: A must be fp32")
# ... 100 lines not shown
        rc = _ngram_fwd(lib, g, x, ctypes.byref(a), Z, fl, _stream(x))
        if rc != _lib.PG_ERR_UNSUPPORTED:
            check(rc, "pg_spmm3_ngram_(mid_)f32")
            _ev_end(x, ev)
            del keep
            return Z
    check(lib.pg_spmm3_gated_f32(N, _p(g.rowptr), _p(g.row_order), _p(g.edges3), _p(x), x.stride(0), F,
                                 ctypes.byref(a), _p(Z), Z.stride(0), fl, _stream(x)), "pg_spmm3_gated_f32")
    _ev_end(x, ev)
    del keep
    return Z


def spmm3t_ngram_acc_bf16(g: CSRGraph, G: torch.Tensor, dX: torch.Tensor, flags: Optional[int] = None,
                          src: Optional[torch.Tensor] = None):
    fl = default_flags() if flags is None else flags
    if not (_is_bf16(G) and _is_bf16(dX) and G.is_contiguous() and dX.is_contiguous() and g.shared and g.symmetric
            and G.size(0) == g.n_rows and dX.size(1) * 3 == G.size(1)
            and _ngram_ok(g, dX, fl, (64, 128, 256), torch.bfloat16)):
        return None
    if src is not None and not (_is_bf16(src) and src.is_contiguous() and src.shape == dX.shape):
        return None
    _require_gpu(G, dX)
    _require_graph_on(g, G)
    lib, ng, F = load_library(), g.ngram, dX.size(1)
    if src is not None:
        rc = lib.pg_spmm3t_ngram_add_bf16(ng.K, ng.n, g.n_rows, _p(ng.plan), _p(G), G.stride(0), F, _p(src),
                                          src.stride(0), _p(dX), dX.stride(0), fl, _stream(G))
        name = "pg_spmm3t_ngram_add_bf16"
    else:
        rc = lib.pg_spmm3t_ngram_bf16(ng.K, ng.n, g.n_rows, _p(ng.plan), _p(G), G.stride(0), F, _p(dX), dX.stride(0),
                                      1, fl, _stream(G))
        name = "pg_spmm3t_ngram_bf16"
    if rc == _lib.PG_ERR_UNSUPPORTED:
        return None
    check(rc, name)
    return dX


def spmm3_t(g: CSRGraph, G: torch.Tensor, flags: Optional[int] = None) -> torch.Tensor:
    lib = load_library()
    if _is_bf16(G):
        G = _bf16c(G)
        _require_gpu(G)
        _require_graph_on(g, G)
        N, F = (g.n_cols if g.n_cols is not None else g.n_rows), G.size(1) // 3
        if g.shared:
            dX = torch.empty(N, F, device=G.device, dtype=torch.bfloat16)
            ro = g.row_order if g.symmetric else None
            fl = default_flags() if flags is None else flags
            if g.symmetric and G.size(0) == g.n_rows and (fl & _lib.PG_FLAG_MID_TRANSPOSED) and _mid_ok(g, dX, fl):
                ng = g.ngram
                rc = lib.pg_spmm3t_ngram_mid_bf16(ng.K, ng.n, N, _p(ng.mplan), _p(G), G.stride(0), F, _p(dX),
                                                  dX.stride(0), 0, fl, _stream(G))
                if rc != _lib.PG_ERR_UNSUPPORTED:
                    check(rc, "pg_spmm3t_ngram_mid_bf16")
                    return dX
            if g.symmetric and G.size(0) == g.n_rows and _ngram_ok(g, dX, fl, (64, 128, 256), torch.bfloat16):
                ng = g.ngram
                rc = lib.pg_spmm3t_ngram_bf16(ng.K, ng.n, N, _p(ng.plan), _p(G), G.stride(0), F, _p(dX), dX.stride(0), 0,
                                              fl, _stream(G))
                if rc != _lib.PG_ERR_UNSUPPORTED:
                    check(rc, "pg_spmm3t_ngram_bf16")
                    return dX
            rc = lib.pg_spmm3t_bf16(N, _p(g.rowptr_t), _p(ro), _p(g.edges3_t), _p(G), G.stride(0), F, _p(dX),
                                    dX.stride(0), fl, _stream(G))
            if rc != _lib.PG_ERR_UNSUPPORTED:
                check(rc, "pg_spmm3t_bf16")
                return dX
        return spmm3_t(g, G.float(), flags).to(torch.bfloat16)
    G = _f32c(G)
    _require_gpu(G)
    _require_graph_on(g, G)
    N, F = (g.n_cols if g.n_cols is not None else g.n_rows), G.size(1) // 3
    dX = torch.empty(N, F, device=G.device, dtype=torch.float32)
    fl = default_flags() if flags is None else flags
    s = _stream(G)
    if g.shared and g.symmetric and G.size(0) == g.n_rows and (fl & _lib.PG_FLAG_MID_TRANSPOSED) and _mid_ok(g, dX, fl):
        rc = _offdiag(lib, g, G, dX, False, fl, s)
        if rc != _lib.PG_ERR_UNSUPPORTED:
            check(rc, "pg_spmm3t_ngram_mid_offdiag_f32")
            d3 = g.ngram.diag3()
            dX += (G[:, :3 * F].view(N, 3, F) * d3.unsqueeze(2)).sum(1)
            return dX
    if g.shared and g.symmetric and G.size(0) == g.n_rows and _ngram_ok(g, dX, fl, (64, 128, 256)):
        ng = g.ngram
        rc = lib.pg_spmm3t_ngram_f32(ng.K, ng.n, N, _p(ng.plan), _p(G), G.stride(0), F, _p(dX), dX.stride(0), 0, fl, s)
        if rc != _lib.PG_ERR_UNSUPPORTED:
            check(rc, "pg_spmm3t_ngram_f32")
            return dX
    if g.shared:
        ro = g.row_order if g.symmetric else None
        check(lib.pg_spmm3t_f32(N, _p(g.rowptr_t), _p(ro), _p(g.edges3_t), _p(G), G.stride(0), F, _p(dX), dX.stride(0), 0,
                                fl, s), "pg_spmm3t_f32")
    else:
        for k, a in enumerate(g.adj):
            check(lib.pg_spmm1_f32(N, _p(a.rowptr_t), None, _p(a.edges_t), _p(G[:, k * F:]), G.stride(0), F, _p(dX),
                                   dX.stride(0), 1 if k else 0, fl, s), "pg_spmm1_f32")
    return dX


def _offdiag(lib, g: CSRGraph, G, dX, accumulate: bool, fl: int, s) -> int:
    ng = g.ngram
    return lib.pg_spmm3t_ngram_mid_offdiag_f32(ng.K, ng.n, g.n_rows, _p(ng.mplan), _p(G), G.stride(0), G.size(1) // 3,
                                               _p(dX), dX.stride(0), 1 if accumulate else 0, fl, s)


def spmm3t_offdiag(g: CSRGraph, G: torch.Tensor, out: Optional[torch.Tensor] = None, flags: Optional[int] = None):
    lib = load_library()
    if _is_bf16(G) or not (g.shared and g.symmetric and g.ngram is not None and g.ngram.mplan is not None):
        return None
    G = _f32c(G)
    _require_gpu(G)
    _require_graph_on(g, G)
    N, F = g.n_rows, G.size(1) // 3
    if G.size(0) != N or F % 16:
        return None
    acc = out is not None
    dX = out if acc else torch.empty(N, F, device=G.device, dtype=torch.float32)
    if dX.dtype != torch.float32 or dX.shape != (N, F) or dX.stride(1) != 1:
        raise ValueError("spmm3t_offdiag: out must be fp32 [N, F] with unit column stride")
    fl = default_flags() if flags is None else flags
    rc = _offdiag(lib, g, G, dX, acc, fl, _stream(G))
    if rc == _lib.PG_ERR_UNSUPPORTED:
        return None
    check(rc, "pg_spmm3t_ngram_mid_offdiag_f32")
    return dX


def spmm3t_rows(rowptr_t: torch.Tensor, edges3_t: torch.Tensor, rows: torch.Tensor, G: torch.Tensor, n_out: int,
                flags: Optional[int] = None) -> torch.Tensor:
    lib = load_library()
    bf = _is_bf16(G)
    G = _bf16c(G) if bf else _f32c(G)
    _require_gpu(G, rowptr_t, edges3_t, rows)
    if rows.dtype != torch.int32 or rowptr_t.numel() != n_out + 1:
        raise ValueError("spmm3t_rows: int32 rows and a rowptr of n_out + 1 entries")
    F = G.size(1) // 3
    dX = torch.empty(n_out, F, device=G.device, dtype=G.dtype)
    fl = default_flags() if flags is None else flags
    if bf:
        check(lib.pg_spmm3t_bf16(rows.numel(), _p(rowptr_t), _p(rows), _p(edges3_t), _p(G), G.stride(0), F, _p(dX),
                                 dX.stride(0), fl, _stream(G)), "pg_spmm3t_bf16")
    else:
        check(lib.pg_spmm3t_f32(rows.numel(), _p(rowptr_t), _p(rows), _p(edges3_t), _p(G), G.stride(0), F, _p(dX),
                                dX.stride(0), 0, fl, _stream(G)), "pg_spmm3t_f32")
    return dX


def spmm1(a: ShapedAdjacency, x: torch.Tensor, transpose: bool = False, flags: Optional[int] = None) -> torch.Tensor:
    lib = load_library()
    x = _f32c(x)
    _require_gpu(x)
    if a.rowptr.device != x.device:
        raise RuntimeError(f"adjacency on {a.rowptr.device} but features on {x.device}")
    N = a.rowptr.numel() - 1
    Y = torch.empty(N, x.size(1), device=x.device, dtype=torch.float32)
    rp, e = (a.rowptr_t, a.edges_t) if transpose else (a.rowptr, a.edges)
    fl = default_flags() if flags is None else flags
    check(lib.pg_spmm1_f32(N, _p(rp), None, _p(e), _p(x), x.stride(0), x.size(1), _p(Y), Y.stride(0), 0, fl,
                           _stream(x)), "pg_spmm1_f32")
    return Y


def edges_normalize(rc, eps: float) -> torch.Tensor:
    lib = load_library()
    _require_gpu(rc.raw)
    out = torch.empty_like(rc.raw)
    check(lib.pg_edges_normalize_f32(rc.n, _p(rc.rowptr), _p(rc.raw), _p(rc.node_norm), eps, _p(out),
                                     _stream(rc.raw)), "pg_edges_normalize_f32")
    return out


def pack_weights(prm: dict, W_res=None, b_res=None) -> torch.Tensor:
    srcs = [prm[k] for k in _PACK_KEYS] + [W_res, b_res]
    lib = load_library()
    F_out, F_in = prm["W_main_in"].shape
    n = lib.pg_directgcn_packed_floats(F_in, F_out, 1 if W_res is not None else 0)
    out = torch.empty(n, device=prm["W_main_in"].device, dtype=torch.float32)
    keep = [_f32c(t.detach()) if t is not None else None for t in srcs]
    a = LayerArgs()
    a.F_in, a.F_out = F_in, F_out
    (a.W_main_in, a.W_main_out, a.W_undirected, a.W_shared, a.b_main_in, a.b_dir_shared_in, a.b_main_out,
     a.b_dir_shared_out, a.b_undirected, a.b_undirected_shared, a.W_res, a.b_res) = [_p(t) for t in keep]
    check(lib.pg_directgcn_pack_f32(ctypes.byref(a), _p(out), _stream(out)), "pg_directgcn_pack_f32")
    return out


def pack_weights_bf16(prm: dict, W_res=None, b_res=None):
    packed = pack_weights(prm, W_res, b_res)
    lib = load_library()
    F_out, F_in = prm["W_main_in"].shape
    n = F_out * (4 if W_res is not None else 3) * F_in
    out = torch.empty(n, device=packed.device, dtype=torch.bfloat16)
    check(lib.pg_f32_to_bf16(n, _p(packed), _p(out), _stream(packed)), "pg_f32_to_bf16")
    return packed, out


def clear_caches():
    from .graph import clear_cache
    clear_cache()


_PACK_KEYS = ("W_main_in", "W_main_out", "W_undirected", "W_shared", "b_main_in", "b_dir_shared_in",
              "b_main_out", "b_dir_shared_out", "b_undirected", "b_undirected_shared")


def _layer_args(Z, prm: dict, gate_mode: int, rows=None, constant=None, res_x=None, W_res=None,
                act: bool = False, slope: float = LEAKY_SLOPE, Y=None, M: Optional[int] = None, drop=None):
    if Z is None:
        M, F_in = int(M), prm["W_main_in"].size(1)
    else:
        M, F_in = Z.size(0), Z.size(1) // 3
    F_out = prm["W_main_in"].size(0)
    keep = []

    def c(t):
        if t is None:
            return None
        t = _f32c(t.detach()) if t.dtype != torch.int64 else t.contiguous()
        keep.append(t)
        return _p(t)

    a = LayerArgs()
    a.M, a.F_in, a.F_out = M, F_in, F_out
    b16 = Z is not None and _is_bf16(Z)
    if Z is not None:
        Zc = _bf16c(Z.detach()) if b16 else _f32c(Z.detach())
        keep.append(Zc)
        a.Z, a.ldz = _p(Zc), Zc.stride(0)
    a.gate_mode = gate_mode
    a.C_in, a.C_out, a.C_directed = c(prm["C_in"]), c(prm["C_out"]), c(prm["C_directed"])
    a.C_undirected, a.C_all = c(prm["C_undirected"]), c(prm["C_all"])
    a.rows = c(rows)
    if constant is not None:
        a.constant, a.ld_const = c(constant), constant.size(1)
    if res_x is not None:
        rx = _bf16c(res_x.detach()) if b16 else _f32c(res_x.detach())
        keep.append(rx)
        a.res_x, a.ld_res = _p(rx), rx.stride(0)
    a.W_res = c(W_res)
    a.act, a.slope = int(bool(act)), float(slope)
    if drop is not None and drop[0] > 0:
        a.drop_p = float(drop[0])
        if drop[1] is not None:
            if drop[1].dtype != torch.int64 or not drop[1].is_cuda or drop[1].numel() < 1:
                raise ValueError("the dropout seed must be a device int64 tensor")
            keep.append(drop[1])
            a.drop_seed = _p(drop[1])
    if Y is not None:
        Yc = Y.detach().contiguous()
        keep.append(Yc)
        a.Y, a.ldy = _p(Yc), Yc.stride(0)
    return a, keep


def layer_dense(Z, prm: dict, gate_mode: int, rows=None, constant=None, res_x=None, W_res=None, b_res=None,
                act: bool = False, slope: float = LEAKY_SLOPE, flags: Optional[int] = None,
                out: Optional[torch.Tensor] = None, pregated: bool = False, packs: Optional[list] = None,
                drop=None) -> torch.Tensor:
    lib = load_library()
    _require_gpu(Z)
    if _is_bf16(Z):
        Y = _layer_dense_bf16(Z, prm, gate_mode, rows, constant, res_x, W_res, b_res, act, slope, flags, packs, drop)
        if Y is None:
            Y = layer_dense(Z.float(), prm, gate_mode, rows, constant, None if res_x is None else res_x.float(),
                            W_res, b_res, act, slope, flags, drop=drop).to(torch.bfloat16)
        if out is not None:
            out.copy_(Y)
            return out
        return Y
    M = Z.size(0)
    F_out = prm["W_main_in"].size(0)
    if out is not None:
        if out.shape != (M, F_out) or out.dtype != torch.float32 or out.stride(1) != 1 or out.device != Z.device:
            raise ValueError("out must be a row-major fp32 [M, F_out] tensor on Z's device")
        Y = out
    else:
        Y = torch.empty(M, F_out, device=Z.device, dtype=torch.float32)
    a, keep = _layer_args(Z, prm, gate_mode, rows, constant, res_x, W_res, act, slope, drop=drop)
    a.Y, a.ldy = _p(Y), Y.stride(0)
    fl = default_flags() if flags is None else flags
    if pregated:
        fl |= _lib.PG_FLAG_DENSE_PREGATED
    if W_res is None and rows is None:
        raw = [_f32c(prm[k].detach()) for k in _PACK_KEYS]
        (a.W_main_in, a.W_main_out, a.W_undirected, a.W_shared, a.b_main_in, a.b_dir_shared_in, a.b_main_out,
         a.b_dir_shared_out, a.b_undirected, a.b_undirected_shared) = [_p(t) for t in raw]
        ev = _ev_start(Z, "DENSE")
        rc = lib.pg_directgcn_dense_f32(ctypes.byref(a), None, fl, _stream(Z))
        if rc != _lib.PG_ERR_UNSUPPORTED:
            check(rc, "pg_directgcn_dense_f32")
            _ev_end(Z, ev, "DENSE")
            del keep, raw
            return Y
    packed = pack_weights(prm, W_res, b_res)
    ev = _ev_start(Z, "DENSE")
    check(lib.pg_directgcn_dense_f32(ctypes.byref(a), _p(packed), fl, _stream(Z)), "pg_directgcn_dense_f32")
    _ev_end(Z, ev, "DENSE")
    del keep
    return Y


def layer_dense_ngram_rows(Z, prm: dict, gate_mode: int, Kn1: int, m0: int, constant=None, res_x=None,
                           map_res: bool = False, out: Optional[torch.Tensor] = None, map_out: bool = False,
                           act: bool = False, slope: float = LEAKY_SLOPE, flags: Optional[int] = None):
    lib = load_library()
    _require_gpu(Z)
    if _is_bf16(Z) or Z.dtype != torch.float32:
        return None
    M = Z.size(0)
    F_out = prm["W_main_in"].size(0)
    if map_out:
        if out is None or out.dtype != torch.float32 or out.stride(1) != 1 or out.size(1) != F_out:
            raise ValueError("map_out needs a row-major fp32 out [n_rows, F_out] in the global row layout")
        Y = out
    elif out is not None:
        if out.shape != (M, F_out) or out.dtype != torch.float32 or out.stride(1) != 1 or out.device != Z.device:
            raise ValueError("out must be a row-major fp32 [M, F_out] tensor on Z's device")
        Y = out
    else:
        Y = torch.empty(M, F_out, device=Z.device, dtype=torch.float32)
    if map_res and (res_x is None or res_x.dtype != torch.float32):
        return None
    a, keep = _layer_args(Z, prm, gate_mode, None, constant, res_x, None, act, slope)
    a.Y, a.ldy = _p(Y), Y.stride(0)
    raw = [_f32c(prm[k].detach()) for k in _PACK_KEYS]
    (a.W_main_in, a.W_main_out, a.W_undirected, a.W_shared, a.b_main_in, a.b_dir_shared_in, a.b_main_out,
     a.b_dir_shared_out, a.b_undirected, a.b_undirected_shared) = [_p(t) for t in raw]
    fl = default_flags() if flags is None else flags
    ev = _ev_start(Z, "DENSE")
    rc = lib.pg_directgcn_dense_ngram_rows_f32(ctypes.byref(a), None, int(Kn1), int(m0), int(bool(map_res)),
                                               int(bool(map_out)), fl, _stream(Z))
    del keep, raw
    if rc == _lib.PG_ERR_UNSUPPORTED:
        return None
    check(rc, "pg_directgcn_dense_ngram_rows_f32")
    _ev_end(Z, ev, "DENSE")
    return Y


def _layer_dense_bf16(Z, prm, gate_mode, rows, constant, res_x, W_res, b_res, act, slope, flags, packs=None,
                      drop=None):
    lib = load_library()
    packed, p16 = pack_weights_bf16(prm, W_res, b_res)
    if packs is not None:
        packs[:] = [packed, p16]
    M = Z.size(0)
    F_out = prm["W_main_in"].size(0)
    Y = torch.empty(M, F_out, device=Z.device, dtype=torch.bfloat16)
    a, keep = _layer_args(Z, prm, gate_mode, rows, constant, res_x, W_res, act, slope, drop=drop)
    a.Y, a.ldy = _p(Y), Y.stride(0)
    fl = default_flags() if flags is None else flags
    ev = _ev_start(Z, "DENSE")
    rc = lib.pg_directgcn_dense_bf16(ctypes.byref(a), _p(packed), _p(p16), fl, _stream(Z))
    del keep
    if rc == _lib.PG_ERR_UNSUPPORTED:
        return None
    check(rc, "pg_directgcn_dense_bf16")
    _ev_end(Z, ev, "DENSE")
    return Y


def layer_dense_backward(dY, Z, Y, prm: dict, gate_mode: int, rows=None, res_x=None, W_res=None, b_res=None,
                         act: bool = False, slope: float = LEAKY_SLOPE, flags: Optional[int] = None,
                         need_dZ: bool = True, packs: Optional[list] = None, span: Optional[tuple] = None,
                         drop_p: float = 0.0, dpre_f32: bool = False):
    lib = load_library()
    _require_gpu(dY, Z, Y)
    M, F_in = Z.size(0), Z.size(1) // 3
    F_out = prm["W_main_in"].size(0)
    bf = _is_bf16(Z)
    if bf and (F_in % 8 or F_out % 8):
        return None
    if bf:
        packed, p16 = packs if packs else pack_weights_bf16(prm, W_res, b_res)
        Y = _bf16c(Y)
    else:
        packed = pack_weights(prm, W_res, b_res)
    a, keep = _layer_args(Z, prm, gate_mode, rows, None, res_x, W_res, act, slope, Y=Y,
                          drop=(drop_p, None) if drop_p else None)
    dev = Z.device
    K = (4 if W_res is not None else 3) * F_in
    act_dt = torch.bfloat16 if bf else torch.float32
    dYc = _bf16c(dY) if bf else _f32c(dY)
    dpre = torch.empty(M, F_out, device=dev, dtype=act_dt)
    dZ = torch.empty(M, 3 * F_in, device=dev, dtype=act_dt) if need_dZ else None
    dres = torch.empty(M, F_in, device=dev, dtype=act_dt) if W_res is not None else None
    dgate = torch.empty(5, M, device=dev)
    gates = torch.empty(M, 4, device=dev)
    dW = torch.empty(F_out * K + 4 * F_out, device=dev)
    nwork = lib.pg_directgcn_dense_bwd_workspace(ctypes.byref(a))
    if nwork < 0:
        raise RuntimeError("pg_directgcn_dense_bwd_workspace: bad arguments")
    work = torch.empty(max(int(nwork), 4), device=dev)
    g = _lib.LayerGradArgs()
    g.dY, g.lddy = _p(dYc), dYc.stride(0)
    g.dpre, g.ldp = _p(dpre), dpre.stride(0)
    if dZ is not None:
        g.dZ, g.lddz = _p(dZ), dZ.stride(0)
    if dres is not None:
        g.dres, g.lddres = _p(dres), dres.stride(0)
    g.dgate, g.gates, g.dW = _p(dgate), _p(gates), _p(dW)
    g.work, g.work_floats = _p(work), work.numel()
    dpre32 = None
    if bf and dpre_f32:
        dpre32 = torch.empty(M, F_out, device=dev, dtype=torch.float32)
        g.dpre_f32, g.ldp_f32 = _p(dpre32), dpre32.stride(0)
    fl = default_flags() if flags is None else flags
    E = None
    if span is not None:
        if bf or dZ is None:
            return None
        wdiag, e_res = span
        wdiag = _f32c(wdiag)
        E = torch.empty(M, F_in, device=dev, dtype=torch.float32)
        rc = lib.pg_directgcn_dense_bwd_span_f32(ctypes.byref(a), _p(packed), ctypes.byref(g), _p(wdiag), _p(E),
                                                 E.stride(0), int(bool(e_res)), fl, _stream(Z))
        name = "pg_directgcn_dense_bwd_span_f32"
    elif bf:
        rc = lib.pg_directgcn_dense_bwd_bf16(ctypes.byref(a), _p(packed), _p(p16), ctypes.byref(g), fl, _stream(Z))
        name = "pg_directgcn_dense_bwd_bf16"
    else:
        rc = lib.pg_directgcn_dense_bwd_f32(ctypes.byref(a), _p(packed), ctypes.byref(g), fl, _stream(Z))
        name = "pg_directgcn_dense_bwd_f32"
    if rc == _lib.PG_ERR_UNSUPPORTED:
        return None
    check(rc, name)
    del keep
    return {"dpre": dpre, "dZ": dZ, "dres": dres, "dgate": dgate, "E": E, "dpre_f32": dpre32,
            "dB": dW[:F_out * K].view(F_out, K), "dbsum": dW[F_out * K:].view(4, F_out)}


def head(h: torch.Tensor, W1, b1, W2, b2, eps: float):
    lib = load_library()
    _require_gpu(h)
    M, F = h.shape
    H, C = W1.size(0), W2.size(0)
    W1, b1, W2, b2 = (_f32c(t.detach()) for t in (W1, b1, W2, b2))
    logp = torch.empty(M, C, device=h.device, dtype=torch.float32)
    emb = torch.empty(M, F, device=h.device, dtype=torch.float32)
    if _is_bf16(h):
        hb = _bf16c(h.detach())
        ev = _ev_start(hb, "HEAD")
        rc = lib.pg_directgcn_head_bf16(M, F, H, C, _p(hb), hb.stride(0), _p(W1), _p(b1), _p(W2), _p(b2), float(eps),
                                        _p(logp), logp.stride(0), _p(emb), emb.stride(0), _stream(hb))
        if rc != _lib.PG_ERR_UNSUPPORTED:
            check(rc, "pg_directgcn_head_bf16")
            _ev_end(hb, ev, "HEAD")
            return logp, emb
    h = _f32c(h.detach())
    ev = _ev_start(h, "HEAD")
    check(lib.pg_directgcn_head_f32(M, F, H, C, _p(h), h.stride(0), _p(W1), _p(b1), _p(W2), _p(b2), float(eps),
                                    _p(logp), logp.stride(0), _p(emb), emb.stride(0), _stream(h)),
          "pg_directgcn_head_f32")
    _ev_end(h, ev, "HEAD")
    return logp, emb


_LABELS_OK: dict = {}


def _check_labels(y: torch.Tensor, C: int):
    key = (y.data_ptr(), y.numel(), y._version, C)
    if key in _LABELS_OK or y.numel() == 0 or torch.cuda.is_current_stream_capturing():
        return
    lo, hi = torch.aminmax(y)
    if int(lo) < 0 or int(hi) >= C:
        raise IndexError(f"head_train: label out of range [0, {C}): min {int(lo)}, max {int(hi)}")
    if len(_LABELS_OK) > 64:
        _LABELS_OK.clear()
    _LABELS_OK[key] = True


def head_train(h: torch.Tensor, W1, b1, W2, b2, y: torch.Tensor, weight: float = 1.0, drop_p: float = 0.0,
               seed: Optional[torch.Tensor] = None, scale: Optional[torch.Tensor] = None):
    lib = load_library()
    _require_gpu(h, y)
    M, Fd = h.shape
    H, C = W1.size(0), W2.size(0)
    nwork = int(lib.pg_head_train_workspace(M, Fd, H, C))
    if nwork < 0:
        return None
    h = _f32c(h)
    W1, b1, W2, b2 = (_f32c(t.detach()) for t in (W1, b1, W2, b2))
    y = y.contiguous().to(torch.int64)
    dev = h.device
    dh = torch.empty(M, Fd, device=dev, dtype=torch.float32)
    grads = torch.empty(H * Fd + H + C * H + C, device=dev, dtype=torch.float32)
    loss = torch.empty((), device=dev, dtype=torch.float32)
    work = torch.empty(max(nwork, 4), device=dev, dtype=torch.float32)
    if drop_p > 0 and seed is None:
        raise ValueError("head_train: dropout needs a seed tensor")
    _check_labels(y, C)
    rc = lib.pg_head_train_f32(M, Fd, H, C, _p(h), h.stride(0), _p(W1), _p(b1), _p(W2), _p(b2), _p(y),
                               float(weight) / max(M, 1), float(drop_p), _p(seed), _p(scale), _p(dh), dh.stride(0),
                               _p(grads), _p(loss), _p(work), work.numel(), _stream(h))
    if rc == _lib.PG_ERR_UNSUPPORTED:
        return None
    check(rc, "pg_head_train_f32")
    o1, o2, o3 = H * Fd, H * Fd + H, H * Fd + H + C * H
    return loss, dh, (grads[:o1].view(H, Fd), grads[o1:o2], grads[o2:o3].view(C, H), grads[o3:])


def head_train_bf16(h: torch.Tensor, W1, b1, W2, b2, y: torch.Tensor, weight: float = 1.0, drop_p: float = 0.0,
                    seed: Optional[torch.Tensor] = None, scale: Optional[torch.Tensor] = None):
    lib = load_library()
    _require_gpu(h, y)
    if not _is_bf16(h) or h.dim() != 2:
        return None
    M, Fd = h.shape
    H, C = W1.size(0), W2.size(0)
    nwork = int(lib.pg_head_train_bf16_workspace(M, Fd, H, C))
    if nwork < 0:
        return None
    h = _bf16c(h)
    W1, b1, W2, b2 = (_f32c(t.detach()) for t in (W1, b1, W2, b2))
    y = y.contiguous().to(torch.int64)
    dev = h.device
    dh = torch.empty(M, Fd, device=dev, dtype=torch.bfloat16)
    grads = torch.empty(H * Fd + H + C * H + C, device=dev, dtype=torch.float32)
    loss = torch.empty((), device=dev, dtype=torch.float32)
    work = torch.empty(max(nwork, 4), device=dev, dtype=torch.float32)
    if drop_p > 0 and seed is None:
        raise ValueError("head_train_bf16: dropout needs a seed tensor")
    _check_labels(y, C)
    rc = lib.pg_head_train_bf16(M, Fd, H, C, _p(h), h.stride(0), _p(W1), _p(b1), _p(W2), _p(b2), _p(y),
                                float(weight) / max(M, 1), float(drop_p), _p(seed), _p(scale), _p(dh), dh.stride(0),
                                _p(grads), _p(loss), _p(work), work.numel(), _stream(h))
    if rc == _lib.PG_ERR_UNSUPPORTED:
        return None
    check(rc, "pg_head_train_bf16")
    o1, o2, o3 = H * Fd, H * Fd + H, H * Fd + H + C * H
    return loss, dh, (grads[:o1].view(H, Fd), grads[o1:o2], grads[o2:o3].view(C, H), grads[o3:])


def gemm_at_b(A: torch.Tensor, B: torch.Tensor):
    lib = load_library()
    _require_gpu(A, B)
    A, B = _f32c(A), _f32c(B)
    M, P = A.shape
    N = B.size(1)
    if P % 4 or N % 4:
        return None
    out = torch.empty(P * N + P, device=A.device, dtype=torch.float32)
    nwork = int(lib.pg_gemm_at_b_workspace(M, P, N))
    work = torch.empty(max(nwork, 4), device=A.device, dtype=torch.float32)
    rc = lib.pg_gemm_at_b_f32(M, P, N, _p(A), A.stride(0), _p(B), B.stride(0), _p(out), _p(work), work.numel(),
                              _stream(A))
    if rc == _lib.PG_ERR_UNSUPPORTED:
        return None
    check(rc, "pg_gemm_at_b_f32")
    return out[:P * N].view(P, N), out[P * N:]




def _fwd32(fn):
    @functools.wraps(fn)
    def forward(ctx, *args):
        if torch.is_autocast_enabled("cuda"):
            args = tuple(a.float() if torch.is_tensor(a) and a.dtype == torch.float16 else a for a in args)
            with torch.autocast("cuda", enabled=False):
                return fn(ctx, *args)
        return fn(ctx, *args)
    return forward


def _bwd32(fn):
    @functools.wraps(fn)
    def backward(ctx, *grads):
        with torch.autocast("cuda", enabled=False):
            return fn(ctx, *grads)
    return backward


class Propagate3(torch.autograd.Function):

    @staticmethod
    @_fwd32
    def forward(ctx, x, g: CSRGraph, fused: bool = False):
        ctx.g = g
        return spmm3(g, x, fused=fused)

    @staticmethod
    @_bwd32
    def backward(ctx, dZ):
        if not ctx.needs_input_grad[0]:
            return None, None, None
        return spmm3_t(ctx.g, dZ), None, None


class Propagate1(torch.autograd.Function):
    @staticmethod
    @_fwd32
    def forward(ctx, x, a: ShapedAdjacency):
        ctx.a = a
        return spmm1(a, x)

    @staticmethod
    @_bwd32
    def backward(ctx, dY):
        return spmm1(ctx.a, dY, transpose=True), None


_DENSE_KEYS = ("W_main_in", "W_main_out", "W_undirected", "W_shared", "b_main_in", "b_dir_shared_in",
# ... 235 lines not shown
```

Baseline: 79.11 billion edges/s.

## Fuse L2 row normalization into last dense layer epilogue and feed head from embeddings

The last DirectGCN layer's dense kernel now computes each row's L2 norm in its register epilogue through cross-wave LDS reduction, writes the normalized embedding plus a per-row norm vector, and a new head kernel variant reads that embedding and rescales the first linear layer by the stored norm. This removes the separate write of the unnormalized hidden state and its reread in the head's normalization pass. In exchange it adds an extra LDS reduction, a deferred store stage and adjusted vmcnt waits to the pipelined dense kernel. It also slightly changes rounding, since the head now computes s*(W1·emb)+b rather than W1·h+b.

```diff
diff --git a/include/pg_directgcn.h b/include/pg_directgcn.h
--- a/include/pg_directgcn.h
+++ b/include/pg_directgcn.h
@@ -300,6 +300,13 @@
                           const float* W1, const float* b1, const float* W2, const float* b2, float eps,
                           float* logp, int64_t ldp, float* emb, int64_t lde, void* stream);
 
+int pg_directgcn_dense_emb_f32(const pg_layer_args_t* args, const float* packed, float eps, float* s, uint32_t flags,
+                               void* stream);
+
+int pg_directgcn_head_emb_f32(int64_t M, int64_t F, int64_t H, int64_t C, const float* emb, int64_t lde,
+                              const float* s, const float* W1, const float* b1, const float* W2, const float* b2,
+                              float* logp, int64_t ldp, void* stream);
+
 #ifdef __cplusplus
 }
 #endif
diff --git a/protgram-directgcn_amd/_lib.py b/protgram-directgcn_amd/_lib.py
--- a/protgram-directgcn_amd/_lib.py
+++ b/protgram-directgcn_amd/_lib.py
@@ -159,6 +159,9 @@
     "pg_gemm_at_b_f32": (ctypes.c_int, [c_i64, c_i64, c_i64, c_vp, c_i64, c_vp, c_i64, c_vp, c_vp, c_i64, c_vp]),
     "pg_directgcn_head_f32": (ctypes.c_int, [c_i64, c_i64, c_i64, c_i64, c_vp, c_i64, c_vp, c_vp, c_vp, c_vp, c_f32,
                                              c_vp, c_i64, c_vp, c_i64, c_vp]),
+    "pg_directgcn_dense_emb_f32": (ctypes.c_int, [ctypes.POINTER(LayerArgs), c_vp, c_f32, c_vp, c_u32, c_vp]),
+    "pg_directgcn_head_emb_f32": (ctypes.c_int, [c_i64, c_i64, c_i64, c_i64, c_vp, c_i64, c_vp, c_vp, c_vp, c_vp, c_vp,
+                                                 c_vp, c_i64, c_vp]),
     "pg_head_train_workspace": (c_i64, [c_i64, c_i64, c_i64, c_i64]),
     "pg_head_train_f32": (ctypes.c_int, [c_i64, c_i64, c_i64, c_i64, c_vp, c_i64, c_vp, c_vp, c_vp, c_vp, c_vp, c_f32,
                                          c_f32, c_vp, c_vp, c_vp, c_i64, c_vp, c_vp, c_vp, c_i64, c_vp]),
diff --git a/protgram-directgcn_amd/csrc/pg_common.h b/protgram-directgcn_amd/csrc/pg_common.h
--- a/protgram-directgcn_amd/csrc/pg_common.h
+++ b/protgram-directgcn_amd/csrc/pg_common.h
@@ -14,6 +14,10 @@
 void clear_error();
 
 __device__ __forceinline__ float4 ld4(const float* p) { return *reinterpret_cast<const float4*>(p); }
+__device__ __forceinline__ float sumsq4(float x, float y, float z, float w) {
+#pragma clang fp contract(off)
+    return ((x * x + y * y) + z * z) + w * w;
+}
 __device__ __forceinline__ float fb(int v) { return __int_as_float(v); }
 
 __device__ __forceinline__ int64_t xcd_logical_block(int64_t b, int64_t nb, bool remap) {
diff --git a/protgram-directgcn_amd/csrc/pg_dense.hip b/protgram-directgcn_amd/csrc/pg_dense.hip
--- a/protgram-directgcn_amd/csrc/pg_dense.hip
+++ b/protgram-directgcn_amd/csrc/pg_dense.hip
@@ -42,6 +42,8 @@
     uint32_t drop_thr;
     float drop_s;
     const int64_t* drop_seed;
+    float eps;
+    float* S;
 };
 
 __device__ __forceinline__ float drop_apply(const DenseP& p, uint64_t seed, int64_t m, int j, float y) {
@@ -676,8 +678,9 @@
 
 __device__ __forceinline__ int a_unit16(int s, int r, int g) { return 64 * s + 4 * r + (g ^ ((-(r >> 2)) & 3)); }
 
-template <bool PRE, bool IL, bool DROP, bool LDSE>
+template <bool PRE, bool IL, bool DROP, bool LDSE, bool NORM = false>
 __global__ __launch_bounds__(512) void dense_x3p_kernel(DenseP p) {
+    static_assert(!NORM || (!DROP && !LDSE), "NORM: register epilogue, inference only");
     constexpr int F_IN = 128, K = 384;
     constexpr int CH = K / 4;
     constexpr int NU = K / 8;
@@ -697,6 +700,7 @@
     __shared__ __attribute__((aligned(16))) float Es[LDSE ? BM * ELD : 4];
     __shared__ __attribute__((aligned(16))) float Gi[4][8][BM];
     __shared__ __attribute__((aligned(16))) float Bs[4][128];
+    __shared__ __attribute__((aligned(16))) float Ns[NORM ? 2 * BM * 8 : 4];
 
     const int tid = threadIdx.x;
     const int wave = tid >> 6, lane = tid & 63;
@@ -887,6 +891,7 @@
         lds_barrier();
         split_tile(Af0, 0, 0);
     }
+    [[maybe_unused]] float yk[4] = {0.f, 0.f, 0.f, 0.f};
     float4 bq[4];
     if (ntl > 0) lds_ld4x4(&Bs[0][ec], &Bs[1][ec], &Bs[2][ec], &Bs[3][ec], bq);
     auto epilogue = [&](int64_t m0, float4 ov, float4 cq, float4 rq, const float (&c)[5]) {
@@ -904,8 +909,26 @@
             y[e] = (p.act && !(qv > 0.f)) ? qv * p.slope : qv;
             if (DROP) y[e] = drop_apply(p, dseed, m0 + er, ec + e, y[e]);
         }
-        const int64_t yr = p.map_y ? ngram_row(p, m0 + er) : m0 + er;
-        *reinterpret_cast<float4*>(p.Y + yr * p.ldy + ec) = make_float4(y[0], y[1], y[2], y[3]);
+        if constexpr (NORM) {
+#pragma unroll
+            for (int e = 0; e < 4; ++e) yk[e] = y[e];
+        } else {
+            const int64_t yr = p.map_y ? ngram_row(p, m0 + er) : m0 + er;
+            *reinterpret_cast<float4*>(p.Y + yr * p.ldy + ec) = make_float4(y[0], y[1], y[2], y[3]);
+        }
+    };
+    [[maybe_unused]] auto store_norm = [&](int64_t m0, int slot) {
+        float4 pa, pb;
+        lds_ld4x2(&Ns[(slot * BM + lc) * 8], &Ns[(slot * BM + lc) * 8 + 4], pa, pb);
+        const float ss = __fadd_rn(__fadd_rn(__fadd_rn(pa.x, pa.y), __fadd_rn(pa.z, pa.w)),
+                                   __fadd_rn(__fadd_rn(pb.x, pb.y), __fadd_rn(pb.z, pb.w)));
+        if (m0 + er < p.M) {
+            const float sn = sqrtf(ss) + p.eps;
+            const float inv = 1.0f / sn;
+            *reinterpret_cast<float4*>(p.Y + (m0 + er) * p.ldy + ec) =
+                make_float4(yk[0] * inv, yk[1] * inv, yk[2] * inv, yk[3] * inv);
+            if (wave == 0 && kg == 0) p.S[m0 + er] = sn;
+        }
     };
     if constexpr (!LDSE) {
         bool y_pending = false;
@@ -913,11 +936,20 @@
             const int ab = (int)(i & 1);
             [[maybe_unused]] const int si = (int)i;
             DSTAMP(si, 0);
-            if (y_pending) asm volatile("s_waitcnt vmcnt(1)" ::: "memory");
-            else asm volatile("s_waitcnt vmcnt(0)" ::: "memory");
+            if constexpr (NORM) {
+                if (y_pending && wave == 0) asm volatile("s_waitcnt vmcnt(2)" ::: "memory");
+                else if (y_pending) asm volatile("s_waitcnt vmcnt(1)" ::: "memory");
+                else asm volatile("s_waitcnt vmcnt(0)" ::: "memory");
+            } else {
+                if (y_pending) asm volatile("s_waitcnt vmcnt(1)" ::: "memory");
+                else asm volatile("s_waitcnt vmcnt(0)" ::: "memory");
+            }
             lds_barrier();
             DSTAMP(si, 1);
             const int64_t m0 = tile_of(i) * BM;
+            if constexpr (NORM) {
+                if (!mfma_first && i > 0) store_norm(tile_of(i - 1) * BM, ab ^ 1);
+            }
             load_CR(tile_of(i));
             __builtin_amdgcn_sched_barrier(0);
             const int64_t a_tile = tile_of(i + 2);
@@ -934,11 +966,20 @@
                 DSTAMP(si, pt);
                 wait_CR();
                 DSTAMP(si, pt + 1);
+                if constexpr (NORM) {
+                    if (mfma_first && i > 0) store_norm(tile_of(i - 1) * BM, ab ^ 1);
+                }
                 float c[5];
                 lds_gates5<BM * 4>(&Gi[(int)(i & 3)][0][er], c);
                 if (!DEXP(2) && m0 + er < p.M) {
                     epilogue(m0, make_float4(acc[0], acc[1], acc[2], acc[3]), make_float4(cv[0], cv[1], cv[2], cv[3]),
                              make_float4(rv[0], rv[1], rv[2], rv[3]), c);
+                }
+                if constexpr (NORM) {
+                    float ss = pg::sumsq4(yk[0], yk[1], yk[2], yk[3]);
+                    ss += __shfl_xor(ss, 16);
+                    ss += __shfl_xor(ss, 32);
+                    if (kg == 0) lds_stf(&Ns[(ab * BM + lc) * 8 + wave], ss);
                 }
                 DSTAMP(si, pt + 2);
             };
@@ -951,7 +992,14 @@
                 DSTAMP(si, 3);
                 mfma_epi(4);
             }
-            y_pending = !DEXP(2) && m0 + BM <= p.M;
+            if constexpr (NORM) y_pending = mfma_first && i > 0 && tile_of(i - 1) * BM + BM <= p.M;
+            else y_pending = !DEXP(2) && m0 + BM <= p.M;
+        }
+        if constexpr (NORM) {
+            if (ntl > 0) {
+                lds_barrier();
+                store_norm(tile_of(ntl - 1) * BM, (int)((ntl - 1) & 1));
+            }
         }
     } else {
         bool y_pending = false;
@@ -1067,7 +1115,7 @@
 }
 
 static int dense_launch(const pg_layer_args_t* a, const float* packed, uint32_t flags, const int64_t* ngmap,
-                        void* stream) {
+                        void* stream, float* S = nullptr, float eps = 0.f) {
     PG_REQUIRE(a != nullptr, "null args");
     PG_REQUIRE(a->M >= 0 && a->F_in > 0 && a->F_out > 0 && a->F_in < (1 << 20) && a->F_out < (1 << 20),
                "bad shape M=%lld F_in=%lld F_out=%lld", (long long)a->M, (long long)a->F_in, (long long)a->F_out);
@@ -1127,6 +1175,8 @@
     p.nt_a = (flags & PG_FLAG_DENSE_A_CACHED) ? 0 : 1;
     if (const int rc = pg::drop_params(a, p.drop_thr, p.drop_s)) return rc;
     p.drop_seed = a->drop_seed;
+    p.S = S;
+    p.eps = eps;
     PG_REQUIRE(p.drop_s == 0.f || a->M * a->F_out <= (int64_t(1) << 32), "fused dropout: M * F_out > 2^32");
 #ifdef PG_DENSE_EXP
     p.exp = (int)((flags >> 24) & 31u);
@@ -1163,6 +1213,8 @@
             const bool il = (flags & PG_FLAG_DENSE_NO_IL) == 0;
             const bool ldse = (flags & PG_FLAG_DENSE_LDS_EPILOGUE) != 0;
             const bool drop = p.drop_s != 0.f;
+            if (S && (ldse || drop || ngmap))
+                return pg::set_error(PG_ERR_UNSUPPORTED, "pg_directgcn_dense_emb_f32: register epilogue, no dropout");
             void (*kern)(DenseP);
 #define PG_X3P_PICK(LDSE)                                                                                  \
     kern = drop ? (p.pregated ? dense_x3p_kernel<true, true, true, LDSE> : dense_x3p_kernel<false, true, true, LDSE>) \
@@ -1171,8 +1223,15 @@
             if (ldse) PG_X3P_PICK(true);
             else PG_X3P_PICK(false);
 #undef PG_X3P_PICK
+            if (S)
+                kern = p.pregated ? (il ? dense_x3p_kernel<true, true, false, false, true>
+                                        : dense_x3p_kernel<true, false, false, false, true>)
+                                  : (il ? dense_x3p_kernel<false, true, false, false, true>
+                                        : dense_x3p_kernel<false, false, false, false, true>);
             hipLaunchKernelGGL(kern, dim3(g16), dim3(512), 0, s, p);
         } else {
+            if (S)
+                return pg::set_error(PG_ERR_UNSUPPORTED, "pg_directgcn_dense_emb_f32: F_in = F_out = 128 only");
             if (p.rawW)
                 return pg::set_error(PG_ERR_UNSUPPORTED, "pg_directgcn_dense_f32: unpacked weights need the pipelined "
                                                          "split-bf16 kernel (F_in = F_out = 128, no row map)");
@@ -1183,6 +1242,9 @@
         }
         return pg::check_launch("pg_directgcn_dense_f32");
     }
+    if (S)
+        return pg::set_error(PG_ERR_UNSUPPORTED, "pg_directgcn_dense_emb_f32: needs the pipelined split-bf16 kernel's "
+                                                 "shape (F_in = F_out = 128, no W_res, no row map, aligned)");
     if (ngmap)
         return pg::set_error(PG_ERR_UNSUPPORTED, "pg_directgcn_dense_ngram_rows_f32: needs the pipelined split-bf16 "
                                                  "kernel's shape (F_in = F_out = 128, no W_res, no row map, aligned)");
@@ -1201,6 +1263,12 @@
 
 int pg_directgcn_dense_f32(const pg_layer_args_t* a, const float* packed, uint32_t flags, void* stream) {
     return dense_launch(a, packed, flags, nullptr, stream);
+}
+
+int pg_directgcn_dense_emb_f32(const pg_layer_args_t* a, const float* packed, float eps, float* s, uint32_t flags,
+                               void* stream) {
+    PG_REQUIRE(s != nullptr && (reinterpret_cast<uintptr_t>(s) & 3) == 0, "s must be a 4-B aligned [M] vector");
+    return dense_launch(a, packed, flags, nullptr, stream, s, eps);
 }
 
 #ifdef PG_DENSE_EXP
diff --git a/protgram-directgcn_amd/csrc/pg_head.hip b/protgram-directgcn_amd/csrc/pg_head.hip
--- a/protgram-directgcn_amd/csrc/pg_head.hip
+++ b/protgram-directgcn_amd/csrc/pg_head.hip
@@ -20,6 +20,7 @@
     int64_t ldp;
     float* emb;
     int64_t lde;
+    const float* srow;
 };
 
 using pg::ld4;
@@ -304,12 +305,14 @@
     }
 }
 
+template <bool EMB_IN>
 __global__ __launch_bounds__(256) __attribute__((amdgpu_waves_per_eu(4, 8))) void head_x3_kernel(HeadP p) {
     constexpr int BM = 32, F = 128, H = 64, CP = 32;
     constexpr int ZLD = H + 8, LLD = CP + 1;
     constexpr int NU = F / 8;
     __shared__ __attribute__((aligned(16))) uint4 As[3][BM * NU];
     __shared__ __attribute__((aligned(16))) float Ls[BM * LLD];
+    __shared__ float Ss[EMB_IN ? 1 : BM];
     float* Zs = reinterpret_cast<float*>(&As[0][0]);
     static_assert(BM * ZLD * 4 <= 3 * BM * NU * 16, "Zs fits the split images");
     const int tid = threadIdx.x, wave = tid >> 6, lane = tid & 63;
@@ -322,7 +325,7 @@
         const int64_t m = m0 + (tid >> 5) + 8 * k;
         if (m >= p.M) {
             hv[k] = make_float4(0.f, 0.f, 0.f, 0.f);
-        } else if (p.hb) {
+        } else if (!EMB_IN && p.hb) {
             const uint2 w = *reinterpret_cast<const uint2*>(p.hb + m * p.ldh + 4 * c4);
             hv[k] = make_float4(__uint_as_float(w.x << 16), __uint_as_float(w.x & 0xffff0000u),
                                 __uint_as_float(w.y << 16), __uint_as_float(w.y & 0xffff0000u));
@@ -330,6 +333,13 @@
             hv[k] = ld4(p.h + m * p.ldh + 4 * c4);
         }
     }
+    [[maybe_unused]] float sv[2][4];
+    if constexpr (EMB_IN) {
+#pragma unroll
+        for (int rb = 0; rb < 2; ++rb)
+#pragma unroll
+            for (int i = 0; i < 4; ++i) sv[rb][i] = p.srow[min(m0 + 16 * rb + 4 * q + i, p.M - 1)];
+    }
     uint4 w0[4], w1[4], w2[4];
     {
         const float* w1row = p.W1 + (int64_t)(16 * wave + li) * F + 8 * q;
@@ -353,14 +363,17 @@
 #pragma unroll
     for (int k = 0; k < 4; ++k) {
         const int r = (tid >> 5) + 8 * k;
-        const float4 v = hv[k];
-        float ss = v.x * v.x + v.y * v.y + v.z * v.z + v.w * v.w;
-#pragma unroll
-        for (int o = 1; o < 32; o <<= 1) ss += __shfl_xor(ss, o, 32);
-        const int64_t m = m0 + r;
-        if (m < p.M) {
-            const float inv = 1.0f / (sqrtf(ss) + p.eps);
-            *reinterpret_cast<float4*>(p.emb + m * p.lde + 4 * c4) = make_float4(v.x * inv, v.y * inv, v.z * inv, v.w * inv);
+        float4 v = hv[k];
+        if constexpr (!EMB_IN) {
+            float ss = pg::sumsq4(v.x, v.y, v.z, v.w);
+#pragma unroll
+            for (int o = 1; o < 32; o <<= 1) ss += __shfl_xor(ss, o, 32);
+            const int64_t m = m0 + r;
+            const float sn = sqrtf(ss) + p.eps;
+            const float inv = 1.0f / sn;
+            v = make_float4(v.x * inv, v.y * inv, v.z * inv, v.w * inv);
+            if (m < p.M) *reinterpret_cast<float4*>(p.emb + m * p.lde + 4 * c4) = v;
+            if (c4 == 0) Ss[r] = sn;
         }
         uint32_t s0[2], s1[2], s2[2];
         {
@@ -398,7 +411,7 @@
     for (int rb = 0; rb < 2; ++rb)
 #pragma unroll
         for (int i = 0; i < 4; ++i) {
-            const float z = acc[rb][i] + b1v;
+            const float z = __fmaf_rn(EMB_IN ? sv[rb][i] : Ss[16 * rb + 4 * q + i], acc[rb][i], b1v);
             Zs[(16 * rb + 4 * q + i) * ZLD + 16 * wave + li] = z > 0.f ? z : 0.f;
         }
     __syncthreads();
@@ -486,7 +499,7 @@
     if (M == 0) return PG_OK;
     PG_REQUIRE((h || hb) && W1 && b1 && W2 && b2 && logp && emb, "null pointer");
     PG_REQUIRE(ldh >= F && lde >= F && ldp >= C, "bad leading dimension");
-    HeadP p{M, (int)F, (int)H, (int)C, h, hb, ldh, W1, b1, W2, b2, eps, logp, ldp, emb, lde};
+    HeadP p{M, (int)F, (int)H, (int)C, h, hb, ldh, W1, b1, W2, b2, eps, logp, ldp, emb, lde, nullptr};
     hipStream_t s = (hipStream_t)stream;
     const bool in_ok = hb ? ((reinterpret_cast<uintptr_t>(hb) & 7) == 0) : pg::aligned16(h);
     const bool vec = F % 4 == 0 && H % 4 == 0 && ldh % 4 == 0 && lde % 4 == 0 && in_ok &&
@@ -504,7 +517,7 @@
 #ifdef PG_HEAD_FP32
         hipLaunchKernelGGL(head_f128_kernel, dim3((unsigned)((M + 31) / 32)), dim3(256), 0, s, p);
 #else
-        hipLaunchKernelGGL(head_x3_kernel, dim3((unsigned)((M + 31) / 32)), dim3(256), 0, s, p);
+        hipLaunchKernelGGL(head_x3_kernel<false>, dim3((unsigned)((M + 31) / 32)), dim3(256), 0, s, p);
 #endif
     } else if (vec && F <= 128 && H <= 64 && C <= 32) {
         hipLaunchKernelGGL((head_kernel<128, 64, 32>), dim3(grid_of(2)), dim3(256), 0, s, p);
@@ -530,3 +543,20 @@
                                       float* logp, int64_t ldp, float* emb, int64_t lde, void* stream) {
     return head_launch(M, F, H, C, nullptr, h, ldh, W1, b1, W2, b2, eps, logp, ldp, emb, lde, stream);
 }
+
+extern "C" int pg_directgcn_head_emb_f32(int64_t M, int64_t F, int64_t H, int64_t C, const float* emb, int64_t lde,
+                                         const float* s, const float* W1, const float* b1, const float* W2,
+                                         const float* b2, float* logp, int64_t ldp, void* stream) {
+    PG_REQUIRE(M >= 0 && F > 0 && H > 0 && C > 0, "bad shape");
+    if (!(F == 128 && H == 64 && C <= 32))
+        return pg::set_error(PG_ERR_UNSUPPORTED, "pg_directgcn_head_emb_f32: needs F = 128, H = 64, C <= 32");
+    if (M == 0) return PG_OK;
+    PG_REQUIRE(emb && s && W1 && b1 && W2 && b2 && logp, "null pointer");
+    PG_REQUIRE(lde >= F && ldp >= C, "bad leading dimension");
+    if (!(lde % 4 == 0 && pg::aligned16(emb) && pg::aligned16(W1) && pg::aligned16(W2)))
+        return pg::set_error(PG_ERR_UNSUPPORTED, "pg_directgcn_head_emb_f32: emb, W1, W2 must be 16-B aligned, lde a "
+                                                 "multiple of 4");
+    HeadP p{M, (int)F, (int)H, (int)C, emb, nullptr, lde, W1, b1, W2, b2, 0.f, logp, ldp, nullptr, 0, s};
+    hipLaunchKernelGGL(head_x3_kernel<true>, dim3((unsigned)((M + 31) / 32)), dim3(256), 0, (hipStream_t)stream, p);
+    return pg::check_launch("pg_directgcn_head_emb_f32");
+}
diff --git a/protgram-directgcn_amd/layer.py b/protgram-directgcn_amd/layer.py
--- a/protgram-directgcn_amd/layer.py
+++ b/protgram-directgcn_amd/layer.py
@@ -143,6 +143,25 @@
         return ops.LayerDense.apply(Z, res_x, constant, W_res, b_res, rows, gate_mode, act, ops.LEAKY_SLOPE, drop,
                                     *params)
 
+    def fused_forward_emb(self, x, graph, eps: float, res_x=None, act=False, fused_norm: bool = False):
+        M = x.size(0)
+        if self.use_vector_coeffs and self.num_nodes != M:
+            raise RuntimeError(f"vector coefficients hold {self.num_nodes} nodes but x has {M} rows "
+                               "(pass original_indices for subgraphs)")
+        if graph.n_rows != M:
+            raise ValueError("graph rows != x rows")
+        constant = self.constant if self.use_vector_coeffs else None
+        gate_mode = 0 if self.use_vector_coeffs else 1
+        prm = dict(zip(ops._DENSE_KEYS, self._dense_params()))
+        Z = ops.spmm3_gated(graph, x, prm, gate_mode) if ops.PREGATED_INFERENCE and not fused_norm else None
+        pregated = Z is not None
+        if Z is None:
+            Z = ops.Propagate3.apply(x, graph, fused_norm)
+        out = ops.layer_dense_emb(Z, prm, gate_mode, eps, constant=constant, res_x=res_x, act=act, pregated=pregated)
+        if out is None:
+            out = ops.layer_dense(Z, prm, gate_mode, constant=constant, res_x=res_x, act=act, pregated=pregated)
+        return out
+
     def forward(self, x: torch.Tensor,
                 edge_index_in: torch.Tensor, edge_weight_in: Optional[torch.Tensor],
                 edge_index_out: torch.Tensor, edge_weight_out: Optional[torch.Tensor],
@@ -233,9 +252,28 @@
                             data.edge_index_undirected_norm, getattr(data, "edge_weight_undirected_norm", None))
 
     def forward(self, data) -> Tuple[torch.Tensor, torch.Tensor]:
+        if self._emb_path(data):
+            out = self._layers(data, last_emb=True)
+            if isinstance(out, tuple):
+                emb, s = out
+                dec = self.decoder_fc
+                return ops.head_from_emb(emb, s, dec[0].weight, dec[0].bias, dec[3].weight, dec[3].bias), emb
+            return self.head(out)
         return self.head(self.body(data))
 
+    def _emb_path(self, data) -> bool:
+        dec = self.decoder_fc
+        x = getattr(data, "x", None)
+        return (ops.FUSED_EMB and not self.training and not torch.is_grad_enabled()
+                and self.compute_dtype == torch.float32 and x is not None and x.is_cuda
+                and getattr(data, "original_indices", None) is None
+                and isinstance(self.res_projs[-1], nn.Identity) and self.convs[-1].out_channels == 128
+                and self.head_train_args() is not None and ops.head_emb_supported(128, dec[0].weight, dec[3].weight))
+
     def body(self, data) -> torch.Tensor:
+        return self._layers(data)
+
+    def _layers(self, data, last_emb: bool = False):
         x = getattr(data, "x", None)
         ei_in = getattr(data, "edge_index_in", None)
         ei_out = getattr(data, "edge_index_out", None)
@@ -259,6 +297,8 @@
             seeds = torch.randint(0, 1 << 62, (len(self.convs),), device=x.device, dtype=torch.int64)
         for i, (conv, res) in enumerate(zip(self.convs, self.res_projs)):
             drop = (p, seeds[i:i + 1]) if seeds is not None else None
+            if last_emb and i == len(self.convs) - 1:
+                return conv.fused_forward_emb(h, g, self.l2_eps, res_x=h, act=True, fused_norm=self.fused_norm)
             if isinstance(res, nn.Linear):
                 h = conv.fused_forward(h, g, original_indices, res_x=h, W_res=res.weight, b_res=res.bias, act=True,
                                        fused_norm=self.fused_norm, drop=drop)
diff --git a/protgram-directgcn_amd/ops.py b/protgram-directgcn_amd/ops.py
--- a/protgram-directgcn_amd/ops.py
+++ b/protgram-directgcn_amd/ops.py
@@ -19,6 +19,7 @@
 SPAN_BACKWARD = True
 BF16_BACKWARD = True
 PREGATED_INFERENCE = True
+FUSED_EMB = True
 
 SPMM_EVENTS: Optional[list] = None
 DENSE_EVENTS: Optional[list] = None
@@ -725,6 +726,61 @@
     return Y
 
 
+def layer_dense_emb(Z, prm: dict, gate_mode: int, eps: float, constant=None, res_x=None, W_res=None, rows=None,
+                    act: bool = False, slope: float = LEAKY_SLOPE, flags: Optional[int] = None,
+                    pregated: bool = False, packed: bool = False):
+    lib = load_library()
+    _require_gpu(Z)
+    if Z.dtype != torch.float32 or W_res is not None or rows is not None:
+        return None
+    M = Z.size(0)
+    F_out = prm["W_main_in"].size(0)
+    emb = torch.empty(M, F_out, device=Z.device, dtype=torch.float32)
+    s = torch.empty(M, device=Z.device, dtype=torch.float32)
+    a, keep = _layer_args(Z, prm, gate_mode, None, constant, res_x, None, act, slope)
+    a.Y, a.ldy = _p(emb), emb.stride(0)
+    fl = default_flags() if flags is None else flags
+    if pregated:
+        fl |= _lib.PG_FLAG_DENSE_PREGATED
+    if packed:
+        w = pack_weights(prm, None, None)
+    else:
+        raw = [_f32c(prm[k].detach()) for k in _PACK_KEYS]
+        (a.W_main_in, a.W_main_out, a.W_undirected, a.W_shared, a.b_main_in, a.b_dir_shared_in, a.b_main_out,
+         a.b_dir_shared_out, a.b_undirected, a.b_undirected_shared) = [_p(t) for t in raw]
+        w = None
+    ev = _ev_start(Z, "DENSE")
+    rc = lib.pg_directgcn_dense_emb_f32(ctypes.byref(a), _p(w) if w is not None else None, float(eps), _p(s), fl,
+                                        _stream(Z))
+    if rc == _lib.PG_ERR_UNSUPPORTED:
+        return None
+    check(rc, "pg_directgcn_dense_emb_f32")
+    _ev_end(Z, ev, "DENSE")
+    del keep
+    return emb, s
+
+
+def head_from_emb(emb: torch.Tensor, s: torch.Tensor, W1, b1, W2, b2):
+    lib = load_library()
+    _require_gpu(emb, s)
+    M, F = emb.shape
+    H, C = W1.size(0), W2.size(0)
+    if emb.dtype != torch.float32 or s.dtype != torch.float32 or s.numel() != M or not s.is_contiguous():
+        raise ValueError("head_from_emb: emb [M, F] and s [M] must be fp32, s contiguous")
+    W1, b1, W2, b2 = (_f32c(t.detach()) for t in (W1, b1, W2, b2))
+    emb = _f32c(emb.detach())
+    logp = torch.empty(M, C, device=emb.device, dtype=torch.float32)
+    ev = _ev_start(emb, "HEAD")
+    check(lib.pg_directgcn_head_emb_f32(M, F, H, C, _p(emb), emb.stride(0), _p(s), _p(W1), _p(b1), _p(W2), _p(b2),
+                                        _p(logp), logp.stride(0), _stream(emb)), "pg_directgcn_head_emb_f32")
+    _ev_end(emb, ev, "HEAD")
+    return logp
+
+
+def head_emb_supported(F: int, W1, W2) -> bool:
+    return F == 128 and tuple(W1.shape) == (64, 128) and W2.size(1) == 64 and W2.size(0) <= 32
+
+
 def layer_dense_ngram_rows(Z, prm: dict, gate_mode: int, Kn1: int, m0: int, constant=None, res_x=None,
                            map_res: bool = False, out: Optional[torch.Tensor] = None, map_out: bool = False,
                            act: bool = False, slope: float = LEAKY_SLOPE, flags: Optional[int] = None):
```

Result: no change. 79.56 billion edges/s (median of 6 runs) (+0.6%).
